# seobbro/TTA-depth-completion

Measured on AMD Instinct MI355X. Metric: TTA frames/sec (fwd+loss+bwd+Adam) at 352x1216, higher is better.
Workload: dtype mixed: real frames' forward (the scored depth) f32 storage + bf16x3 MFMA arithmetic; no_grad proxy pass and all data gradients bf16 storage + single bf16 MFMA; fp32 accumulate everywhere; loss / Adam / adapted parameters fp32 (include/ptta.h PTTA_DTYPE_MIXED)

## Files before the change

include/ptta.h:

```cpp
#ifndef PTTA_H
#define PTTA_H
#include <stdint.h>
#ifdef __cplusplus
extern "C" {
#endif

typedef struct ptta_ctx* ptta_handle;
typedef void* ptta_stream;

enum { PTTA_BACKBONE_MSG_CHN = 0, PTTA_BACKBONE_NLSPN = 1, PTTA_BACKBONE_COSTDCNET = 2 };
enum { PTTA_DTYPE_F32 = 0, PTTA_DTYPE_MIXED = 1,
       PTTA_MIXED_KEEP_PROXY = 0x100, PTTA_MIXED_KEEP_BACKWARD = 0x200, PTTA_MIXED_KEEP_HEADS = 0x400,
       PTTA_MIXED_BWD_ROUNDED_W = 0x800 };
enum { PTTA_META_1LAYER = 0, PTTA_META_2LAYERS = 1, PTTA_META_NONE = 2 };
enum { PTTA_NLSPN_LEGACY_OFFSET = 0x100,
       PTTA_NLSPN_SYNCBN_ADAPT = 0x200,
       PTTA_SYNCBN_ADAPT = 0x200,
       PTTA_ADAPT_META_ONLY = 0x400 };

typedef struct {
    float lr, beta1, beta2, eps, weight_decay;
    float w_sparse_depth, w_smoothness, w_cos;
    float max_input_depth;
    float max_predict_depth;
// ... 52 lines not shown
int ptta_eval_metrics(const float* depth, const float* ground_truth, int64_t numel, float min_evaluate_depth,
                      float max_evaluate_depth, void* scratch, float* metrics_out, ptta_stream s);

int ptta_mdconv_forward(const float* input, const float* weight, const float* bias, const float* offset, const float* mask,
                        float* output, int b, int c, int h, int w, int c_out, int kh, int kw, int sh, int sw, int ph, int pw,
                        int dh, int dw, int group, int deformable_group, ptta_stream s);
int ptta_mdconv_backward(const float* input, const float* weight, const float* bias, const float* offset, const float* mask,
                         const float* grad_output, float* grad_input, float* grad_offset, float* grad_mask, float* grad_weight,
                         float* grad_bias, int b, int c, int h, int w, int c_out, int kh, int kw, int sh, int sw, int ph, int pw,
                         int dh, int dw, int group, int deformable_group, ptta_stream s);

int ptta_set_image_norm(ptta_handle h, float divisor, const float* mean, const float* stdv);

int ptta_head_bind(ptta_handle h, const char* name, float* param, float* exp_avg, float* exp_avg_sq);
int ptta_head_set_hparams(ptta_handle h, float lr, float beta1, float beta2, float eps, float weight_decay, float tau,
                          int adam_step, ptta_stream s);
int ptta_head_reload(ptta_handle h, ptta_stream s);
int ptta_head_forward(ptta_handle h, const float* image, const float* sparse_depth, int reverse, float* emb_out, float* ref_out,
                      ptta_stream s);
int ptta_head_backward(ptta_handle h, float* loss_out, ptta_stream s);
int ptta_head_adam_step(ptta_handle h, ptta_stream s);
int ptta_head_step(ptta_handle h, const float* image, const float* sparse_depth, int reverse, float* loss_out, ptta_stream s);
int ptta_head_get_grad(ptta_handle h, const char* name, float* dst, int64_t capacity, int* has_grad_host, ptta_stream s);

enum { PTTA_HEAD_FORM_PLAIN = 0, PTTA_HEAD_FORM_SYNCBN = 1 };
int ptta_head_set_form(ptta_handle h, int form);

int ptta_crop_flip(const float* src, float* dst, int n, int channels, int height, int width, int crop_height, int crop_width,
                   const int32_t* start_y, const int32_t* start_x, const uint8_t* hflip, const uint8_t* vflip, ptta_stream s);

int ptta_rotate(const float* src, float* dst, int n, int channels, int height, int width, const uint8_t* do_rotate, const float* angle_deg,
                int bilinear, ptta_stream s);
int ptta_resize_crop(const float* src, float* dst, int n, int channels, int height, int width, const uint8_t* do_resize,
                     const int32_t* resize_height, const int32_t* resize_width, const int32_t* start_y, const int32_t* start_x,
                     int bilinear, int scale_depth, ptta_stream s);
int ptta_photometric(const float* src, float* dst, int n, int height, int width, const uint8_t* do_brightness, const float* f_brightness,
                     const uint8_t* do_contrast, const float* f_contrast, const uint8_t* do_saturation, const float* f_saturation,
                     double* scratch, ptta_stream s);

int ptta_photometric_full(const float* src, float* dst, int n, int height, int width, const uint8_t* do_brightness, const float* f_brightness,
                          const uint8_t* do_contrast, const float* f_contrast, const uint8_t* do_gamma, const float* f_gamma,
                          const uint8_t* do_hue, const float* f_hue, const uint8_t* do_saturation, const float* f_saturation,
                          double* scratch, ptta_stream s);
int ptta_add_noise(const float* src, const float* noise, float* dst, int n, int channels, int height, int width, const uint8_t* do_noise,
                   float spread, int uniform, ptta_stream s);
int ptta_remove_patches(const float* src, float* dst, int n, int channels, int height, int width, const uint8_t* do_remove,
                        const uint8_t* selected, const int32_t* patch_height, const int32_t* patch_width, ptta_stream s);
int ptta_crop_pad(const float* src, float* dst, int n, int channels, int height, int width, const uint8_t* do_crop_pad,
                  const int32_t* start_y, const int32_t* start_x, const int32_t* end_y, const int32_t* end_x,
                  const int32_t* pad_top, const int32_t* pad_left, int padding_mode, float fill, ptta_stream s);
int ptta_resize_pad(const float* src, float* dst, int n, int channels, int height, int width, const uint8_t* do_resize_pad,
                    const int32_t* resize_height, const int32_t* resize_width, const int32_t* pad_top, const int32_t* pad_left,
                    int bilinear, int padding_mode, float fill, ptta_stream s);

typedef int (*ptta_allreduce_fn)(void* user, double* exchange_buf, long long count, ptta_stream s);
int ptta_set_stat_sync(ptta_handle h, ptta_allreduce_fn fn, void* user, double* exchange_buf, int64_t capacity, int world_size);

int ptta_rccl_unique_id(void* id128_host);
int ptta_rccl_comm_create(const void* id128_host, int rank, int world_size, void** comm_out_host);
int ptta_rccl_comm_destroy(void* comm);
int ptta_rccl_allreduce_mean_f32(void* comm, float* buf, int64_t count, ptta_stream s);
const char* ptta_rccl_last_error(void);
int ptta_set_stat_sync_rccl(ptta_handle h, void* comm, double* exchange_buf, int64_t capacity, int world_size);
int ptta_set_grad_sync_rccl(ptta_handle h, void* comm);

int ptta_set_graph(ptta_handle h, int enable);

int ptta_set_option(ptta_handle h, const char* key, int value);
int ptta_get_option(ptta_handle h, const char* key, int* value_host);

int ptta_profile(ptta_handle h, int enable);
int ptta_profile_read(ptta_handle h, int klass, double* ms_total_host, double* alg_bytes_host, double* macs_host,
                      int64_t* launches_host, ptta_stream s);

int ptta_debug_tensor(ptta_handle h, const char* name, float* dst, int64_t capacity, int64_t* numel_host, ptta_stream s);
int ptta_op_conv32(const float* in_nhwc, const float* weight, const float* bias, float* out_nhwc,
                   int b, int hin, int win, int mode, int relu_in, int in_major, int flip, int dtype, int naive,
                   ptta_stream s);
int ptta_op_conv32_pair(const float* in_nhwc, const float* weight1, const float* bias1, const float* weight2, const float* bias2,
                        const float* up_nhwc, const float* add0_nhwc, const float* add1_nhwc, const float* add2_nhwc,
                        const uint32_t* mask1_bits, const uint32_t* mask2_bits, float* out_raw, float* out_sum, float* mid_raw,
                        float* mid_sum, uint32_t* mid_bits, int b, int in_nb, int hin, int win, int first_mode, int relu1, int relu2,
                        int in_major, int flip, int dtype, int w2, int fused, int* fused_host, ptta_stream s);
int ptta_op_gwgrad(const float* x_nhwc, const float* gy_nhwc, float* gw, float* gb, int b, int h, int w, int ci, int co, int impl,
                   int reps, float* us_per_call_host, ptta_stream s);
#define PTTA_GCONV_S1 0
#define PTTA_GCONV_S2 1
#define PTTA_GCONV_T2 2
#define PTTA_GCONV_VERT 1
#define PTTA_GCONV_X1_W2 2
#define PTTA_GCONV_DGRAD 4
#define PTTA_GCONV_AFF_ACT_FIRST 8
#define PTTA_GCONV_AFF_RES_PLAIN 16
int ptta_op_gconv(const float* x0, int c0, int ld0, const float* x1, int c1, int ld1, const float* weight, const float* bias, float* y,
                  int co, int ldy, int b, int hin, int win, int hout, int wout, int k, int geom, int act, int accumulate, int impl,
                  int flags, int six_b, int x1_from_b, int stat_npass, double* stat_host, int* form_host, ptta_stream s);
int ptta_op_gconv_affine(const float* x0, int c0, int ld0, const float* x1, int c1, int ld1, const float* weight, const float* bias, float* y,
                         int co, int ldy, int b, int hin, int win, int hout, int wout, int k, int geom, int act, int accumulate, int impl,
                         int flags, int six_b, int x1_from_b, int stat_npass, double* stat_host, int* form_host, const float* scale,
                         const float* shift, const float* res, int ld_res, ptta_stream s);
#define PTTA_GBN_TRAIN 0
#define PTTA_GBN_EVAL 1
#define PTTA_GBN_BACKWARD 2
typedef struct ptta_gbn_view { float* p; int c; int ld; } ptta_gbn_view;
typedef struct ptta_gbn_args {
    int mode, b, h, w, npass, act, act_first, res_relu, acc_gx, acc_gres, world, nblocks_in, repeats;
    float eps, momentum;
    ptta_gbn_view x, res, y, g, gx, gres;
    const float* gamma; const float* beta; const float* part_in;
    float* st; float* rm; float* rv; long long* nbt; float* st_eval; float* dgamma; float* dbeta;
} ptta_gbn_args;
int ptta_op_gbn(const ptta_gbn_args* a, ptta_stream s);
typedef struct ptta_cd_sparse ptta_cd_sparse;
int ptta_cd_sparse_create(ptta_cd_sparse** out, int n, int h, int w);
void ptta_cd_sparse_destroy(ptta_cd_sparse* q);
int ptta_cd_sparse_build(ptta_cd_sparse* q, const float* sparse, float z_step, ptta_stream s);
int ptta_cd_sparse_read(ptta_cd_sparse* q, int level, int* cnt_host, int* coords_host, long long coords_cap, int* vol_host, float* feat_in_host,
                        ptta_stream s);
int ptta_op_cd_sparse_conv(ptta_cd_sparse* q, const float* x, const float* wk, float* y, int lin, int lout, int ksize, int ci, int co, int backward,
                           int acc, ptta_stream s);
typedef struct ptta_cd_sbn_args {
    int mode, level, c, relu, repeats, world, acc_res;
    const float* f; const float* res; const float* y; const float* g; const float* gamma; const float* beta;
    float* rm; float* rv; long long* nbt; float* out; float* st; float* dgamma; float* dbeta; float* gx; float* gres;
} ptta_cd_sbn_args;
int ptta_op_cd_sbn(ptta_cd_sparse* q, const ptta_cd_sbn_args* a, ptta_stream s);
int ptta_op_cd_densify(ptta_cd_sparse* q, const float* in, float* out, int c, int backward, int ldv, int c0, ptta_stream s);
#define PTTA_CD_PAD_DUAL 0
#define PTTA_CD_CROP_AVG 1
#define PTTA_CD_SCATTER_DUAL_GRAD 2
#define PTTA_CD_STAGE 3
#define PTTA_CD_CLAMP 4
#define PTTA_CD_FUSION_FWD 5
#define PTTA_CD_FUSION_BWD 6
#define PTTA_CD_POOL_FWD 7
#define PTTA_CD_POOL_BWD 8
#define PTTA_CD_UP_FWD 9
#define PTTA_CD_UP_BWD 10
#define PTTA_CD_REGRESS_FWD 11
#define PTTA_CD_REGRESS_BWD 12
#define PTTA_CD_ROWS_FWD 13
#define PTTA_CD_ROWS_BWD 14
int ptta_op_cd_dense(int op, const float* a, const float* b, float* out, float* out2, const int* d, const float* f, ptta_stream s);
int ptta_op_conv32_chain(const float* in_nhwc, const float* weight, const float* bias, float* buf_a, float* buf_b, const float* aux,
                         int b, int h, int w, int relu_in, int epi_flags, int reps, int replays, float* us_per_launch_host, ptta_stream s);
#define PTTA_ABI_VERSION 2
int ptta_version(void);

#ifdef __cplusplus
}
#endif
#endif
```

tta-depth-completion_amd/csrc/msgchn_backward.hip:

```cpp
#include "msgchn_ctx.h"

using namespace msgchn;

namespace msgchn {

static int meta2_backward(ptta_ctx* c, hipStream_t s) {
    auto& m2 = c->m2;
    ptta_ctx::Adapted* A = c->adapted.data();
    const int H4 = c->H4, W4 = c->W4, Nn = c->Nn;
    const long P = (long)Nn * H4 * W4;
    if (m2.generic) {
        const int npass = 2;
        GView x; x.p = (float*)c->c2; x.B = Nn; x.H = H4; x.W = W4; x.C = 32; x.ld = 32;
        GView hv = x; hv.p = m2.gh; hv.C = 128; hv.ld = 128;
        GView av = hv; av.p = m2.ga1;
        GView tv = x; tv.p = m2.gt;
        GView gm = x; gm.p = c->nar_bwd ? c->dm_f32 : (float*)c->dm_total;
        GView dt = x; dt.p = m2.gdt;
        GView da1 = hv; da1.p = m2.gda1;
        GView dh = hv; dh.p = m2.gdh;
        RUN(ptta_launch_gbn_backward(tv, gm, tv, dt, GView(), npass, GACT_NONE, 0, 0, 0, A[5].p, m2.gst2, m2.gpart, m2.gbw, A[5].g, A[6].g, s, 0, &c->stat_sync));
        RUN(ptta_launch_gwgrad_mfma(av, dt, m2.wgp, A[3].g, A[4].g, s));
        GX3Args a;
        a.x0 = dt.p; a.C0 = 32; a.ld0 = 32; a.B = Nn; a.H = H4; a.W = W4;
// ... 30 lines not shown
                  (double)c->Rg * (16384.0 + 262144.0), 3);
    const Lin& l0 = c->fc["proj.0"]; const Lin& l3 = c->fc["proj.3"]; BNorm& bn = c->bn["proj.1"];
    const int R = (int)c->Rg;
    if (c->nar_heads && heads_v2_on(c)) {
        HnGemmArgs g; g.epi = 3; g.R = R; g.W = l3.Wtsl;
        if (c->cos_in_gemm) { g.pro = 4; g.A = c->emb_n; g.Bref = c->ref_n; g.rowstats = c->loss_ws + ptta_loss_ws_rows_off(c->N); g.coef = c->loss_ws; }
        else { g.pro = 5; g.Af = gref; }
        g.X = c->feat; g.x_bf16 = 0; g.W0 = l0.Whi; g.W0t = l0.Wthi; g.b0 = l0.bias;
        g.escale = bn.scale; g.eshift = bn.shift; g.emean = bn.mean; g.einv = bn.inv; g.part = c->bn_part; g.P = c->headP;
        RUN(ptta_launch_hn_gemm(g, s));
        const int nb = ptta_hn_row_blocks(R);
        RUN(ptta_stat_sync(&c->stat_sync, c->bn_part, nb, 512, 1, s));
        RUN(ptta_launch_bn_bwd_finalize(c->bn_part, nb, R * (c->stat_sync.world > 1 ? c->stat_sync.world : 1), 512, bn.gamma, bn.inv, c->bnb_gscale, c->bnb_c1, c->bnb_c2, s,
                                        nullptr, nullptr, c->head_k12, l0.bias, bn.mean));
        RUN(ptta_launch_head_bwd_finish(c->head_k12, l0.W, c->headP, (const float*)c->feat, R, c->g_feat, s, 1, c->nar_bwd ? 1 : 0));
        return 0;
    }
    if (heads_v2_on(c)) {
        GemmArgs g; g.A = gref; g.W = l3.Wt; g.R = R; g.K = 512; g.N = 512; g.epi = 3;
        if (c->cos_in_gemm) {
            g.A = c->emb; g.Bref = c->ref; g.rowstats = c->loss_ws + ptta_loss_ws_rows_off(c->N); g.coef = c->loss_ws; g.pro = 4;
        }
        g.escale = bn.scale; g.eshift = bn.shift; g.emean = bn.mean; g.einv = bn.inv; g.part = c->bn_part;
        g.x3 = 1; g.Whi = l3.Wthi; g.Wlo = l3.Wtlo; g.Wil = l3.Wtil;
        g.X = (const float*)c->feat; g.b0 = l0.bias; g.W0hi = l0.Whi; g.W0lo = l0.Wlo; g.W0thi = l0.Wthi; g.W0tlo = l0.Wtlo; g.P = c->headP;
        RUN(ptta_launch_gemm(g, s));
        RUN(ptta_stat_sync(&c->stat_sync, c->bn_part, ptta_gemm_part_blocks(g), 512, 1, s));
        RUN(ptta_launch_bn_bwd_finalize(c->bn_part, ptta_gemm_part_blocks(g), R * (c->stat_sync.world > 1 ? c->stat_sync.world : 1), 512, bn.gamma, bn.inv, c->bnb_gscale, c->bnb_c1, c->bnb_c2, s,
                                        nullptr, nullptr, c->head_k12, l0.bias, bn.mean));
        RUN(ptta_launch_head_bwd_finish(c->head_k12, l0.W, c->headP, (const float*)c->feat, R, c->nar_bwd ? c->g_feat_f32 : (float*)c->g_feat, s));
        if (c->nar_bwd) RUN(to_narrow(c, c->g_feat_f32, c->g_feat, c->Rg * 32, s));
        return 0;
    }
    GemmArgs g; g.A = gref; g.W = l3.Wt; g.C = c->gmask; g.R = R; g.K = 512; g.N = 512; g.epi = 2;
    g.eH = c->h1; g.escale = bn.scale; g.eshift = bn.shift; g.emean = bn.mean; g.einv = bn.inv; g.part = c->bn_part;
    g.x3 = c->x3; g.Whi = l3.Wthi; g.Wlo = l3.Wtlo; g.Wil = l3.Wtil;
    RUN(ptta_launch_gemm(g, s));
    RUN(ptta_stat_sync(&c->stat_sync, c->bn_part, ptta_gemm_part_blocks(g), 512, 1, s));
    RUN(ptta_launch_bn_bwd_finalize(c->bn_part, ptta_gemm_part_blocks(g), R * (c->stat_sync.world > 1 ? c->stat_sync.world : 1), 512, bn.gamma, bn.inv, c->bnb_gscale, c->bnb_c1, c->bnb_c2, s));
    GemmArgs g2; g2.A = c->gmask; g2.A2 = c->h1; g2.W = l0.Wt; g2.C = (c->bf16 || c->nar_bwd) ? c->g_feat_f32 : (float*)c->g_feat; g2.R = R; g2.K = 512; g2.N = 32; g2.pro = 2;
    g2.pscale = c->bnb_gscale; g2.pmean = bn.mean; g2.pinv = bn.inv; g2.pc1 = c->bnb_c1; g2.pc2 = c->bnb_c2;
    g2.x3 = c->x3; g2.Whi = l0.Wthi; g2.Wlo = l0.Wtlo;
    RUN(ptta_launch_gemm(g2, s));
    if (c->bf16 || c->nar_bwd) from_f32_launch(c->g_feat_f32, (bf16_t*)c->g_feat, c->Rg * 32, s);
    return 0;
}

int backbone_backward(ptta_ctx* c, const float* g_net, hipStream_t s, bool join_aux) {
    const int Nn = c->Nn, B2 = 2 * Nn;
    const int nbf = c->nar_bwd ? 1 : c->bf16;
    const int H1 = c->Hp, W1 = c->Wp, H2 = c->H2, W2 = c->W2, H4 = c->H4, W4 = c->W4, H8 = c->H8, W8 = c->W8;
    auto out1_args = [&](const std::string& layer, const float* g, const void* mask, void* out, int H, int W) {
        const LOut& lo = c->lout[layer];
        ConvInArgs a; a.cin = 1; a.pl[0].p = g; a.pl[0].nb = Nn; a.pl[0].bstride = (long)H * W;
        a.wfrag = lo.bfrag; a.wcanon = lo.bcanon; a.mask = mask; a.mask_nb = B2; a.out_raw = out;
        a.B = Nn; a.H = H; a.W = W; a.bf16 = c->nar_bwd ? 1 : c->bf16; a.naive = c->naive;
        return a;
    };
    auto dgrad_out1 = [&](const std::string& layer, const float* g, const void* mask, void* out, int H, int W) -> int {
        ConvInArgs a = out1_args(layer, g, mask, out, H, W);
        return conv_in_p(c, a, s);
    };
    auto head_bwd = [&](const std::string& l3, const std::string& l1, const float* g, const void* v, void* dv, int H, int W, const E& e) -> int {
        ConvInArgs a = out1_args(l3, g, v, dv, H, W);
        return conv32_first_bwd(c, s, l1, a, Nn, H, W, e);
    };
    auto dgrad_in_ch1 = [&](const std::string& layer, const void* g, const float* add, float* out, int H, int W) -> int {
        const LIn& li = c->lin_in[layer];
        ConvOut1Args a; a.in = g; a.in_nb = Nn; a.w = li.bw; a.add = add; a.add_nb = Nn; a.out = out;
        a.B = Nn; a.H = H; a.W = W; a.relu_in = 0; a.bf16 = c->nar_bwd ? 1 : c->bf16;
        return conv_out1_p(c, a, s);
    };
    auto em = [](void* raw, const void* mask, int mask_nb) { E e; e.raw = raw; e.mask = mask; e.mask_nb = mask_nb; return e; };
    RUN(head_bwd("depth_decoder3.prdct.3", "depth_decoder3.prdct.1", g_net, c->v3, c->dv3, H1, W1, em(c->ds0_3, c->s0_3, Nn)));
    CV("depth_decoder3.dec1.3", true, CONV_S1, c->ds0_3, Nn, Nn, H1, W1, false, em(c->du3, c->u3, Nn));
    CV("depth_decoder3.dec1.1", true, CONV_S2, c->du3, Nn, Nn, H1, W1, false, em(c->ds1_3, c->s1_3, Nn));
    CV("depth_decoder3.dec2.3", true, CONV_S1, c->ds1_3, Nn, Nn, H2, W2, false, em(c->dt3, c->t3, Nn));
    if (join_aux) HIPCHK(hipStreamWaitEvent(s, c->ev_join, 0));
    { E e; e.raw = c->dw2; e.mask = c->w2; e.mask_nb = B2; e.sum = c->dfeat_tot; e.add1 = c->g_feat; e.add1_nb = Nn;
      RUN(conv32_pair(c, s, true, "depth_decoder3.dec2.1", c->dt3, Nn, Nn, H2, W2, e, "depth_encoder3.enc2.3", Nn, em(c->de3_2a, c->e3_2a, B2))); }
    hipStream_t sd = join_aux ? c->aux(s) : nullptr;
    if (!sd) sd = s;
    { E e; e.sum = c->de3_1; e.mask = c->e3_1; e.mask_nb = B2; e.add1 = c->ds1_3; e.add1_nb = Nn;
      CV("depth_encoder3.enc2.1", true, CONV_T2, c->de3_2a, Nn, Nn, H4, W4, false, e); }
    CV("depth_encoder3.enc1.3", true, CONV_S1, c->de3_1, Nn, Nn, H2, W2, false, em(c->de3_1a, c->e3_1a, B2));
    { E e; e.sum = c->de3_0; e.mask = c->e3_0; e.mask_nb = B2; e.add1 = c->ds0_3; e.add1_nb = Nn;
      CV("depth_encoder3.enc1.1", true, CONV_T2, c->de3_1a, Nn, Nn, H2, W2, false, e); }
    if (sd != s) { HIPCHK(hipEventRecord(c->ev_side[0], s)); HIPCHK(hipStreamWaitEvent(sd, c->ev_side[0], 0)); }
    REST_(sd, ptta_launch_up2T_32(c->de3_0, nullptr, c->up4_t, Nn, H2, W2, nbf, sd));
    REST_(sd, ptta_launch_up2T_32(c->de3_1, nullptr, c->up3_t, Nn, H4, W4, nbf, sd));
    REST_(sd, ptta_launch_up2T_32(c->dfeat_tot, nullptr, c->dz2_up, Nn, H8, W8, nbf, sd));
    if (sd != s) HIPCHK(hipEventRecord(c->ev_side[3], sd));
    if (c->loss_report.on) {
        REST_(sd, ptta_launch_loss_depth_part(final_depth(c), c->loss_report.image, c->loss_report.sparse, c->loss_report.validity, c->hp.max_input_depth,
                                              c->N, c->H, c->W, c->loss_ws, sd));
        REST_(sd, ptta_launch_loss_finalize(c->loss_ws, c->N, c->H, c->W, c->Rg, 1, c->hyper + 5, c->loss_info_dst ? c->loss_info_dst : c->loss_info, sd));
        HIPCHK(hipEventRecord(c->ev_loss, sd));
    }
    CV("depth_encoder3.init.2", true, CONV_S1, c->de3_0, Nn, Nn, H1, W1, false, em(c->de3_0a, c->e3_0a, B2));
    RUN(dgrad_in_ch1("depth_encoder3.init.0", c->de3_0a, g_net, c->dp11, H1, W1));
    REST_(s, ptta_launch_up2T_1ch(c->dp11, c->dq, Nn, H2, W2, s));
    if (sd != s) HIPCHK(hipStreamWaitEvent(s, c->ev_side[3], 0));
    { E e = em(c->ds0_2, c->s0_2, B2); e.sum = c->dz4; e.add1 = c->up4_t; e.add1_nb = Nn;
      RUN(head_bwd("depth_decoder2.prdct.3", "depth_decoder2.prdct.1", c->dq, c->v2, c->dv2, H2, W2, e)); }
    CV("depth_decoder2.dec1.3", true, CONV_S1, c->dz4, Nn, Nn, H2, W2, false, em(c->du2, c->u2, B2));
    { E e = em(c->ds1_2, c->s1_2, B2); e.sum = c->dz3; e.add1 = c->up3_t; e.add1_nb = Nn;
      RUN(conv32_pair(c, s, true, "depth_decoder2.dec1.1", c->du2, Nn, Nn, H2, W2, e, "depth_decoder2.dec2.3", Nn, em(c->dt2, c->t2, B2))); }
    { E e; e.sum = c->dz2; e.mask = c->z2; e.mask_nb = B2; e.add1 = c->dz2_up; e.add1_nb = Nn;
      RUN(conv32_pair(c, s, true, "depth_decoder2.dec2.1", c->dt2, Nn, Nn, H4, W4, e, "depth_encoder2.enc2.3", Nn, em(c->de2_2a, c->e2_2a, B2))); }
    { E e; e.sum = c->de2_1; e.mask = c->e2_1; e.mask_nb = B2; e.add1 = c->ds1_2; e.add1_nb = Nn;
      CV("depth_encoder2.enc2.1", true, CONV_T2, c->de2_2a, Nn, Nn, H8, W8, false, e); }
    CV("depth_encoder2.enc1.3", true, CONV_S1, c->de2_1, Nn, Nn, H4, W4, false, em(c->de2_1a, c->e2_1a, B2));
    { E e; e.sum = c->de2_0; e.mask = c->e2_0; e.mask_nb = B2; e.add1 = c->ds0_2; e.add1_nb = Nn;
      CV("depth_encoder2.enc1.1", true, CONV_T2, c->de2_1a, Nn, Nn, H4, W4, false, e); }
    CV("depth_encoder2.init.2", true, CONV_S1, c->de2_0, Nn, Nn, H2, W2, false, em(c->de2_0a, c->e2_0a, B2));
    RUN(dgrad_in_ch1("depth_encoder2.init.0", c->de2_0a, c->dq, c->dp12, H2, W2));
    REST_(s, ptta_launch_up2T_1ch(c->dp12, c->dout1, Nn, H4, W4, s));
    RUN(dgrad_out1("depth_decoder1.prdct.3", c->dout1, c->v1, c->dv1, H4, W4));
    { E e; e.sum = c->dm_total; e.mask = c->s0_1; e.mask_nb = B2; e.add1 = c->dw2; e.add1_nb = Nn; e.add2 = c->ds1_2; e.add2_nb = Nn;
      CV("depth_decoder1.prdct.1", true, CONV_S1, c->dv1, Nn, Nn, H4, W4, false, e); }
    if (sd != s && c->loss_report.on) HIPCHK(hipStreamWaitEvent(s, c->ev_loss, 0));
    if (c->nar_bwd && c->meta_mode == PTTA_META_2LAYERS) RUN(to_wide(c, c->dm_total, c->dm_f32, (long)Nn * H4 * W4 * 32, s));
    if (c->meta_mode == PTTA_META_2LAYERS) return meta2_backward(c, s);
    if (!c->bf16 && c->x3 && !c->naive) {
        GView xv; xv.p = (float*)c->c2; xv.B = Nn; xv.H = H4; xv.W = W4; xv.C = 32; xv.ld = 32;
        GView gv; gv.p = (float*)c->dm_total; gv.B = Nn; gv.H = H4; gv.W = W4; gv.C = 32; gv.ld = 32;
        GwAdam ga;
        const bool fuse = c->adam_fuse_req && c->adam_in_wgrad && !c->grad_comm && c->adapted.size() == 2 && c->adapted[0].p && c->adapted[0].m && c->adapted[0].v &&
                          c->adapted[1].p && c->adapted[1].m && c->adapted[1].v && c->adapted[0].g == c->gW && c->adapted[1].g == c->gB;
        if (fuse) { ga.pw = c->adapted[0].p; ga.mw = c->adapted[0].m; ga.vw = c->adapted[0].v; ga.pb = c->adapted[1].p; ga.mb = c->adapted[1].m; ga.vb = c->adapted[1].v;
                    ga.hyper = c->hyper; ga.step = c->step_dev; ga.ticket = c->adam_ticket; }
        REST_(s, ptta_launch_gwgrad_mfma(xv, gv, c->wgrad_part, c->gW, c->gB, s, c->nar_bwd ? 1 : 0, fuse ? &ga : nullptr));
        c->adam_fused = fuse;
        return 0;
    }
    REST_(s, ptta_launch_wgrad32(c->c2, c->dm_total, c->bf16, Nn, H4, W4, c->wgrad_part, c->gW, c->gB, s));
    return 0;
}

}
```

tta-depth-completion_amd/csrc/msgchn_ctx.h:

```cpp
#pragma once
#include <cstdio>
#include <cstdlib>
#include <cstring>
#include <map>
#include <string>
#include <unordered_map>
#include <vector>

#include "../../include/ptta.h"
#include "ptta_common.h"
#include "ptta_kernels.h"
#include "nlspn.h"

#pragma GCC visibility push(hidden)

#define HIPCHK(x) do { hipError_t e_ = (x); if (e_ != hipSuccess) return c->fail(std::string(#x) + ": " + hipGetErrorString(e_), -100 - (int)e_); } while (0)
#define RUN(x) do { int r_ = (x); if (r_ != 0) return c->fail_chain(std::string(#x) + " failed", r_ < 0 ? r_ : -r_); } while (0)

#define NLFWD(call) do { if (c && c->nl) { c->err.clear(); return (call); } } while (0)

struct ImgNorm { int on; float div; float mean[3]; float stdv[3]; };

namespace msgchn {
hipError_t d2d_copy(void* dst, const void* src, size_t bytes, hipStream_t s);
void stamp_launch(float* out, unsigned long long* base, int i, hipStream_t s);
void transpose_launch(const float* src, float* dst, int rows, int cols, hipStream_t s);
void pad_dual_launch(const float* src, float* dst, int N, int C, int H, int W, int Hp, int Wp, int pt, int pr, hipStream_t s,
                     ImgNorm nm = ImgNorm{0, 1.f, {0.f, 0.f, 0.f}, {1.f, 1.f, 1.f}});
void crop_avg_launch(const float* net, float* out, int N, int H, int W, int Hp, int Wp, int pt, int pr, hipStream_t s);
void scatter_dual_grad_launch(const float* g, float* gnet, int N, int H, int W, int Hp, int Wp, int pt, int pr, hipStream_t s);
void to_f32_launch(const bf16_t* src, float* dst, long n, hipStream_t s);
void from_f32_launch(const float* src, bf16_t* dst, long n, hipStream_t s);
void fuse_linear_launch(const float* Wb, const float* bb, const float* Wa, const float* ba, float* W, float* bias, int N, int M, int K, hipStream_t s);
}

static constexpr unsigned kStepEvent = hipEventDisableTiming | hipEventDisableSystemFence;
struct L32 { ConvW f{}, b{}; float* bias = nullptr; int transposed = 0; };
struct LIn { float *wfrag = nullptr, *wcanon = nullptr, *bias = nullptr, *bw = nullptr; int cin = 1; };
struct LOut { float *w = nullptr, *bias = nullptr, *bfrag = nullptr, *bcanon = nullptr; };
struct Lin { float *W = nullptr, *Wt = nullptr, *bias = nullptr; bf16_t *Whi = nullptr, *Wlo = nullptr, *Wthi = nullptr, *Wtlo = nullptr, *Wil = nullptr, *Wtil = nullptr;
             bf16_t *Wsl = nullptr, *Wtsl = nullptr;
             int N = 0, K = 0; };
struct BNorm { float *gamma = nullptr, *beta = nullptr, *rm = nullptr, *rv = nullptr; long long* nbt = nullptr;
               float *mean = nullptr, *inv = nullptr, *scale = nullptr, *shift = nullptr; };
struct Dbg { const void* p; long numel; int is_act; };

struct PrefixBufs {
    void *c0 = nullptr, *c1 = nullptr, *c2 = nullptr, *c3 = nullptr, *c4 = nullptr, *e1_0a = nullptr, *e1_0 = nullptr, *e1_1a = nullptr;
    void *c0a = nullptr, *c1a = nullptr, *c2a = nullptr, *c3a = nullptr, *c4a = nullptr;
    void *e1_1 = nullptr, *y1 = nullptr, *e1_2a = nullptr, *y2 = nullptr, *t1 = nullptr, *y3 = nullptr, *s1_1 = nullptr, *u1 = nullptr;
    float *dclamp = nullptr, *d12 = nullptr, *d14 = nullptr, *in_image = nullptr, *in_loss_image = nullptr, *in_sparse = nullptr, *in_validity = nullptr;
    bool proxy_valid = false;
};

struct ptta_ctx : PrefixBufs {
    GNet* nl = nullptr;
    int N = 1, H = 0, W = 0, Hp = 0, Wp = 0, pt = 0, pr = 0, dual = 0, Nn = 1;
    int bf16 = 0, naive = 0, es = 4, x3 = 1;
    int mixed = 0;
    int nar_proxy = 0, nar_bwd = 0, nar_heads = 0;
    std::unordered_map<const void*, void*> ntwin;
    void* tw(const void* p) const { auto it = ntwin.find(p); return it == ntwin.end() ? nullptr : it->second; }
    void twin_alloc(const void* p, int nb, int h, int w) { if (nar_proxy && p) ntwin[p] = dalloc((size_t)nb * h * w * 32 * 2); }
    float *dm_f32 = nullptr;
    ptta_hparams hp{};
    std::string err;
    std::vector<void*> allocs;
    std::map<std::string, L32> l32;
    std::map<std::string, LIn> lin_in;
    std::map<std::string, LOut> lout;
    std::map<std::string, Lin> fc;
    std::map<std::string, BNorm> bn;
    std::map<std::string, Dbg> dbg;
    int meta_mode = 0;
    struct Adapted { std::string name; long n = 0; float *p = nullptr, *m = nullptr, *v = nullptr, *g = nullptr; };
    std::vector<Adapted> adapted;
    struct HeadT { bool ready = false; std::vector<Adapted> prm, tgt; bool has_grad[12] = {};
                   float *hyper = nullptr, *tau2 = nullptr, *loss = nullptr, *loss_part = nullptr, *wpart = nullptr, *bpart = nullptr, *dp = nullptr;
                   float *sv_mean = nullptr, *sv_inv = nullptr, *sv_scale = nullptr, *sv_shift = nullptr;
                   int* step = nullptr; unsigned* ticket = nullptr; PttaAdamEntry *tab = nullptr, *etab = nullptr;
                   std::vector<PttaAdamEntry> tab_host, etab_host; int tab_n = 0; long tab_total = 0, etab_total = 0; int tab_mode = -1; bool etab_dirty = true;
                   int reverse = 1; bool fwd_ok = false, bwd_ok = false;
                   float* garena = nullptr; long garena_n = 0;
                   int form = 0; bool stepped = false; } head;
    int skip_dec3 = 0;
    int head_swap = 0;
    float *meta_w = nullptr, *meta_b = nullptr;
    float *gW = nullptr, *gB = nullptr;
    struct Meta2 {
        ConvW w1f[4], w2f[4], w2b[4];
        void *h[4] = {}, *a1[4] = {}, *t = nullptr, *dt = nullptr, *da1 = nullptr, *dh = nullptr;
        float *st1 = nullptr, *st2 = nullptr;
        float *rm1 = nullptr, *rv1 = nullptr, *rm2 = nullptr, *rv2 = nullptr; long long *nbt1 = nullptr, *nbt2 = nullptr;
        float *cs_part = nullptr, *bw = nullptr;
        bool generic = false;
        float *gh = nullptr, *ga1 = nullptr, *gt = nullptr, *gdt = nullptr, *gda1 = nullptr, *gdh = nullptr;
        float *w1c = nullptr, *w2c = nullptr, *w2bc = nullptr;
        bf16_t *w1hi = nullptr, *w1lo = nullptr, *w2hi = nullptr, *w2lo = nullptr, *w2bhi = nullptr, *w2blo = nullptr;
        float *gst1 = nullptr, *gst2 = nullptr, *part1 = nullptr, *part2 = nullptr, *gbw = nullptr, *gpart = nullptr, *wgp = nullptr;
    } m2;
    float* hyper = nullptr;
    float* w3_tmp = nullptr;
    int* step_dev = nullptr; float* stamp_f = nullptr; unsigned long long* stamp_base = nullptr; int stamps = 0;
    void stamp(int i, hipStream_t s) { if (stamps) msgchn::stamp_launch(stamp_f, stamp_base, i, s); }
    PttaAdamEntry* adam_tab = nullptr; unsigned* adam_ticket = nullptr; bool adam_tab_dirty = true;
    std::vector<PttaAdamEntry> adam_host;
    bool fwd_valid = false;
    PttaStatSync stat_sync;
    Lin fused_pp; bool fused_pp_valid = false; int fuse_heads = 1;
    int heads_v2 = 1;
    int thru = 1; bool thru_active = false;
    int adam_in_wgrad = 1; bool adam_fuse_req = false, adam_fused = false;
    int bwd_w2 = 1;
    const float *cnt_sparse = nullptr, *cnt_validity = nullptr;
    struct { const float *image = nullptr, *sparse = nullptr, *validity = nullptr; bool on = false; } loss_report;
    hipEvent_t ev_loss = nullptr;
    hipEvent_t ev_dpart = nullptr;
    int fuse_first = 1, fuse_head_bwd = 1;
    int pair_fuse = 1;
    int pair_fuse_count = 0;
    int cos_grad_fused = 1;
    bool cos_in_gemm = false;
    void* w0frag = nullptr; float *hm_part = nullptr, *headP = nullptr; double* head_k12 = nullptr;
    struct ProfClass { std::vector<std::pair<hipEvent_t, hipEvent_t>> ev; size_t used = 0; double bytes = 0, macs = 0; long launches = 0; };
    bool prof_on = false;
    static constexpr int NPROF = 9;
    ProfClass prof[NPROF];
    std::vector<std::pair<int, size_t>> prof_seq;
    int use_graph = 0;
    void* grad_comm = nullptr;
    float* grad_arena = nullptr; long grad_arena_n = 0;
    int pre_sync_graph = -1, pre_sync_aux = -1;
    hipGraphExec_t gexec[4] = {nullptr, nullptr, nullptr, nullptr};
    hipGraph_t graph[4] = {nullptr, nullptr, nullptr, nullptr};
    hipStream_t cap_stream = nullptr;
    struct PreSet : PrefixBufs {
        bool prepared = false, rest_recorded = false;
        uint64_t prep_token = 0;
        uint64_t last_token = 0;
    };
    PreSet pset[2];
    int cur_set = 0, pipe_cur = 0, pipe_last = 0;
    bool pipe_ready = false, pipe_active = false, skip_prefix = false;
    const float *fb_image = nullptr, *fb_sparse = nullptr;
    hipStream_t pre_stream = nullptr;
    hipEvent_t ev_prefix[2] = {nullptr, nullptr}, ev_rest[2] = {nullptr, nullptr}, ev_entry = nullptr;
    hipStream_t pipe_stream = nullptr; bool pipe_stream_set = false;
    hipGraph_t pgraph[2] = {nullptr, nullptr}, rgraph[4][2] = {{nullptr, nullptr}, {nullptr, nullptr}, {nullptr, nullptr}, {nullptr, nullptr}};
    hipGraphExec_t pexec[2] = {nullptr, nullptr}, rexec[4][2] = {{nullptr, nullptr}, {nullptr, nullptr}, {nullptr, nullptr}, {nullptr, nullptr}};
    int use_aux = 1;
    hipStream_t aux_stream = nullptr;
    hipEvent_t ev_fork = nullptr, ev_join = nullptr, ev_real = nullptr;
    hipEvent_t ev_side[4] = {nullptr, nullptr, nullptr, nullptr};
    hipStream_t aux(hipStream_t caller) {
        if (!use_aux) return nullptr;
        if (!aux_stream) {
            if (hipStreamCreateWithFlags(&aux_stream, hipStreamNonBlocking) != hipSuccess) return nullptr;
            if (hipEventCreateWithFlags(&ev_fork, kStepEvent) != hipSuccess ||
                hipEventCreateWithFlags(&ev_join, kStepEvent) != hipSuccess ||
                hipEventCreateWithFlags(&ev_real, kStepEvent) != hipSuccess ||
                hipEventCreateWithFlags(&ev_side[0], kStepEvent) != hipSuccess || hipEventCreateWithFlags(&ev_side[1], kStepEvent) != hipSuccess ||
                hipEventCreateWithFlags(&ev_side[2], kStepEvent) != hipSuccess || hipEventCreateWithFlags(&ev_side[3], kStepEvent) != hipSuccess) { (void)hipStreamDestroy(aux_stream); aux_stream = nullptr; return nullptr; }
        }
        return prof_on ? caller : aux_stream;
    }
    hipEvent_t ev_replay = nullptr;
    void drop_graphs() {
        if (ev_replay) (void)hipEventSynchronize(ev_replay);
        if (pre_stream) (void)hipStreamSynchronize(pre_stream);
        for (int k = 0; k < 4; ++k) {
            if (gexec[k]) { (void)hipGraphExecDestroy(gexec[k]); gexec[k] = nullptr; }
            if (graph[k]) { (void)hipGraphDestroy(graph[k]); graph[k] = nullptr; }
            for (int p = 0; p < 2; ++p) {
                if (rexec[k][p]) { (void)hipGraphExecDestroy(rexec[k][p]); rexec[k][p] = nullptr; }
                if (rgraph[k][p]) { (void)hipGraphDestroy(rgraph[k][p]); rgraph[k][p] = nullptr; }
            }
        }
        for (int p = 0; p < 2; ++p) {
            if (pexec[p]) { (void)hipGraphExecDestroy(pexec[p]); pexec[p] = nullptr; }
            if (pgraph[p]) { (void)hipGraphDestroy(pgraph[p]); pgraph[p] = nullptr; }
            pset[p].prepared = false; pset[p].prep_token = pset[p].last_token = 0;
        }
        fb_image = fb_sparse = nullptr;
    }

    int err_code = 0;
    int fail(const std::string& m, int code) { err = m; err_code = code; return code; }
    int fail_chain(const std::string& m, int code) { err = (err_code == code && !err.empty() && err.size() < 600) ? m + " <- " + err : m; err_code = code; return code; }

    bool oom = false;
    void* dalloc(size_t bytes) {
        void* p = nullptr;
        if (hipMalloc(&p, bytes ? bytes : 16) != hipSuccess) { oom = true; return nullptr; }
        allocs.push_back(p);
        if (hipMemset(p, 0, bytes ? bytes : 16) != hipSuccess) { oom = true; return nullptr; }
        return p;
    }
    float* falloc(size_t n) { return (float*)dalloc(n * sizeof(float)); }
    void* act(const char* name, int nb, int h, int w) {
        void* p = dalloc((size_t)nb * h * w * 32 * es);
        dbg[name] = Dbg{p, (long)nb * h * w * 32, 1};
        if (nar_proxy && nb == 2 * Nn) twin_alloc(p, Nn, h, w);
        return p;
// ... 1 lines not shown
    void* gact(const char* name, int nb, int h, int w) {
        const int e = nar_bwd ? 2 : es;
        void* p = dalloc((size_t)nb * h * w * 32 * e);
        dbg[name] = Dbg{p, (long)nb * h * w * 32, nar_bwd ? 2 : 1};
        return p;
    }
    int mask_bits_on = 1;
    std::unordered_map<const void*, uint32_t*> mbits;
    void mask_plane(const void* map, int nb, int h, int w) {
        if (bf16 || naive) return;
        if (mbits.count(map)) return;
        mbits[map] = (uint32_t*)dalloc((size_t)nb * h * w * sizeof(uint32_t));
    }
    uint32_t* bits_of(const void* map) const {
        if (!map || !mask_bits_on) return nullptr;
        auto it = mbits.find(map);
        return it == mbits.end() ? nullptr : it->second;
    }
    float* map1(const char* name, int nb, int h, int w) {
        float* p = falloc((size_t)nb * h * w);
        dbg[name] = Dbg{p, (long)nb * h * w, 0};
        return p;
    }

    int H2, W2, H4, W4, H8, W8, H16, W16;
    long Rg = 0;
    float *img_pad = nullptr, *sp_pad = nullptr, *zero_plane = nullptr;
    ImgNorm img_norm = ImgNorm{0, 1.f, {0.f, 0.f, 0.f}, {1.f, 1.f, 1.f}};
    float *out1, *p12, *q, *p11, *depth_net, *depth_final, *validity_tmp;
    void *m, *y4, *s0_1, *v1;
    void *e2_0a, *e2_0, *e2_1a, *e2_1, *e2_2a, *z2, *t2, *z3, *s1_2, *u2, *z4, *s0_2, *v2;
    void *e3_0a, *e3_0, *e3_1a, *e3_1, *e3_2a, *feat, *w2, *t3, *s1_3, *u3, *s0_3, *v3;
    float *h1z, *pz, *h2, *emb, *h1, *ref, *gref_buf, *gmask, *bn_part;
    double* hn_msc = nullptr;
    float* hn_rs = nullptr;
    bool cos_rows_done = false;
    bf16_t *emb_n = nullptr, *ref_n = nullptr, *h2_n = nullptr;
    float *bnb_gscale, *bnb_c1, *bnb_c2;
    float *loss_ws, *loss_info, *g_final, *g_net;
    float* loss_info_dst = nullptr;
    void *dv3, *ds0_3, *du3, *ds1_3, *dt3, *dw2, *dfeat_tot, *dz2_up, *de3_2a, *de3_1, *de3_1a, *de3_0, *de3_0a;
    void *up4_t, *up3_t, *dv2, *ds0_2, *dz4, *du2, *ds1_2, *dz3, *dt2, *dz2, *de2_2a, *de2_1, *de2_1a, *de2_0, *de2_0a, *dv1, *dm_total, *g_feat;
    float *dp11, *dq, *dp12, *dout1, *g_feat_f32;
    float* wgrad_part;
};

struct ProfScope {
    ptta_ctx::ProfClass* pc = nullptr; hipStream_t s;
    ProfScope(ptta_ctx* c, int klass, hipStream_t s_, double bytes, double macs, int launches) : s(s_) {
        if (!c->prof_on) return;
        pc = &c->prof[klass];
        if (pc->used == pc->ev.size()) {
            hipEvent_t e0, e1;
            if (hipEventCreate(&e0) != hipSuccess || hipEventCreate(&e1) != hipSuccess) { pc = nullptr; return; }
            pc->ev.push_back({e0, e1});
        }
        pc->bytes += bytes; pc->macs += macs; pc->launches += launches;
        c->prof_seq.push_back({klass, pc->used});
        (void)hipEventRecord(pc->ev[pc->used].first, s);
    }
    ~ProfScope() { if (pc) { (void)hipEventRecord(pc->ev[pc->used].second, s); pc->used++; } }
};
#define REST_(s_, call) do { ProfScope ps_(c, 8, (s_), 0, 0, 1); RUN(call); } while (0)
#define CV(...) RUN(conv32(c, s, __VA_ARGS__))

struct E { const void* up = nullptr; int up_nb = 1; const void* mask = nullptr; int mask_nb = 1;
           const void* add1 = nullptr; int add1_nb = 1; const void* add2 = nullptr; int add2_nb = 1;
           void* raw = nullptr; void* sum = nullptr;
           bool nar = false; };

inline float* st_ptr(float* base, int C, int pass, int kind) { return base + ((size_t)pass * 4 + kind) * C; }

namespace msgchn {
int pad16(int n);
void build_registry(ptta_ctx* c);
void build_workspace(ptta_ctx* c);
int load_weight(ptta_ctx* c, const std::string& name, const void* tensor, const int64_t* shape, int ndim, hipStream_t s);
int conv_in_p(ptta_ctx* c, const ConvInArgs& a_, hipStream_t s);
int conv_out1_p(ptta_ctx* c, const ConvOut1Args& a, hipStream_t s);
int conv32(ptta_ctx* c, hipStream_t s, const std::string& layer, bool bwd, int mode, const void* in, int in_nb,
           int B, int Hin, int Win, bool relu, const E& e);
int conv32_pair(ptta_ctx* c, hipStream_t s, bool bwd, const std::string& first, const void* in, int in_nb, int B, int Hin, int Win, const E& fe,
                const std::string& second, int mid_nb, const E& se);
int conv32w(ptta_ctx* c, hipStream_t s, const ConvW* w, const float* bias, const void* in, int in_nb, int B, int H, int W, const E& e);
int conv32_first_bwd(ptta_ctx* c, hipStream_t s, const std::string& layer, ConvInArgs& f, int B, int H, int W, const E& e);
int to_narrow(ptta_ctx* c, const void* src_f32, void* dst, long n, hipStream_t s);
int to_wide(ptta_ctx* c, const void* src_nar, float* dst, long n, hipStream_t s);
int rgb_encoder(ptta_ctx* c, const float* image, int nb, int boff, int zero_from_b, hipStream_t s);
int ensure_fused_heads(ptta_ctx* c, hipStream_t s);
int ensure_proxy_rgb(ptta_ctx* c, const float* any_image, hipStream_t s);
int enc1_head_fn(ptta_ctx* c, hipStream_t st);
int stage1_independent(ptta_ctx* c, int B2, hipStream_t s);
bool heads_v2_on(const ptta_ctx* c);
int heads_forward(ptta_ctx* c, hipStream_t s, int part = 0);
int push_hparams(ptta_ctx* c, hipStream_t s);
int forward_common(ptta_ctx* c, const float* image, const float* sparse, bool train, hipStream_t s);
const float* final_depth(ptta_ctx* c);
int heads_backward(ptta_ctx* c, const float* gref, hipStream_t s);
int backbone_backward(ptta_ctx* c, const float* g_net, hipStream_t s, bool join_aux);
void pipe_use(ptta_ctx* c, int p);
void pipe_overwritten(ptta_ctx* c, int p);
int pipe_quiesce(ptta_ctx* c);
int ensure_adam_table(ptta_ctx* c, hipStream_t s);
}
#pragma GCC visibility pop
```

tta-depth-completion_amd/csrc/msgchn_forward.hip:

```cpp
#include "msgchn_ctx.h"

using namespace msgchn;

namespace msgchn {

int conv_in_p(ptta_ctx* c, const ConvInArgs& a_, hipStream_t s) {
    ConvInArgs a = a_;
    const double px = (double)a.B * a.H * a.W;
    ProfScope ps(c, 7, s, px * (a.cin * 4 + 32 * (a.bf16 ? 2 : c->es)) + 9.0 * a.cin * 32 * 4, px * 9.0 * a.cin * 32, 1);
    if (!c->mbits.empty()) {
        if (!a.mask_bits) a.mask_bits = c->bits_of(a.mask);
        if (!a.bf16 && !a.a_bits) { a.a_bits = c->bits_of(a.out_raw); a.a_bits_nb = c->Nn; }
    }
    return ptta_launch_conv_in(a, s);
}
int conv_out1_p(ptta_ctx* c, const ConvOut1Args& a, hipStream_t s) {
    const double px = (double)a.B * a.H * a.W;
    ProfScope ps(c, 7, s, px * (32 * (a.bf16 ? 2 : c->es) + 4) + 288 * 4, px * 288.0, 1);
    return ptta_launch_conv_out1(a, s);
}

static int conv32_args(ptta_ctx* c, Conv32Args& a, const std::string& layer, bool bwd, int mode, const void* in, int in_nb,
                       int B, int Hin, int Win, bool relu, const E& e) {
    auto it = c->l32.find(layer);
    if (it == c->l32.end()) return c->fail("unknown 32->32 layer " + layer, -2);
    a.in = in; a.in_nb = in_nb; a.w = bwd ? &it->second.b : &it->second.f;
    a.bias = bwd ? nullptr : (layer == "conv1_rgb_meta" ? c->meta_b : it->second.bias);
    a.up = e.up; a.up_nb = e.up_nb; a.mask = e.mask; a.mask_nb = e.mask_nb;
    a.add1 = e.add1; a.add1_nb = e.add1_nb; a.add2 = e.add2; a.add2_nb = e.add2_nb;
    a.out_raw = e.raw; a.out_sum = e.sum;
    const bool nar = e.nar || (bwd && c->nar_bwd);
    a.B = B; a.Hin = Hin; a.Win = Win; a.mode = mode; a.relu_in = relu ? 1 : 0; a.bf16 = nar ? 1 : c->bf16; a.naive = c->naive; a.x3 = c->x3;
    a.w2 = (bwd && c->nar_bwd && c->bwd_w2) ? 1 : 0;
    if (!c->mbits.empty()) {
        a.mask_bits = c->bits_of(e.mask);
        if (!bwd && !nar) {
            uint32_t* bs = c->bits_of(e.sum); uint32_t* br = c->bits_of(e.raw);
            if (bs && br) return c->fail("conv32: both outputs of " + layer + " are registered masks", -22);
            if (bs || br) { a.bits_out = bs ? bs : br; a.bits_sum = bs ? 1 : 0; a.bits_nb = c->Nn; }
        }
    }
    return 0;
}

static void conv32_cost(int mode, int B, int Hin, int Win, int es_l, double& bytes, double& macs) {
    const long pin = (long)B * Hin * Win;
    const long pout = mode == CONV_S1 ? pin : (mode == CONV_S2 ? pin / 4 : pin * 4);
    bytes = (double)((pin + pout) * 32 + 9216) * es_l;
    macs = (double)(mode == CONV_T2 ? pin : pout) * 9.0 * 32.0 * 32.0;
}

int conv32(ptta_ctx* c, hipStream_t s, const std::string& layer, bool bwd, int mode, const void* in, int in_nb,
           int B, int Hin, int Win, bool relu, const E& e) {
    Conv32Args a;
    { const int rc = conv32_args(c, a, layer, bwd, mode, in, in_nb, B, Hin, Win, relu, e); if (rc) return rc; }
    const bool nar = e.nar || (bwd && c->nar_bwd);
    const int es_l = nar ? 2 : c->es;
    const long pin = (long)B * Hin * Win;
    const long pout = mode == CONV_S1 ? pin : (mode == CONV_S2 ? pin / 4 : pin * 4);
    const bool small = (long)Hin * Win <= (long)c->H4 * c->W4 * (mode == CONV_S2 ? 4 : 1);
#ifdef PTTA_EXP_SKIP_PAIRED_S1
    if (mode == CONV_S1 && small && layer.size() > 2 && layer.compare(layer.size() - 2, 2, ".3") == 0 && layer.find("prdct") == std::string::npos) return 0;
#endif
    ProfScope ps(c, (mode == CONV_S1 ? (relu ? 0 : 2) : 4) + (small ? 1 : 0), s, (double)((pin + pout) * 32 + 9216) * es_l,
                 (double)(mode == CONV_T2 ? pin : pout) * 9.0 * 32.0 * 32.0, 1);
    return ptta_launch_conv32(a, s);
}

int conv32_pair(ptta_ctx* c, hipStream_t s, bool bwd, const std::string& first, const void* in, int in_nb, int B, int Hin, int Win, const E& fe,
                const std::string& second, int mid_nb, const E& se) {
    const int Hm = Hin / 2, Wm = Win / 2;
    const bool relu = !bwd;
    void* const mid = fe.sum ? fe.sum : fe.raw;
    const bool nar = fe.nar || (bwd && c->nar_bwd);
    if (c->pair_fuse && !c->naive && (c->x3 || c->bf16 || nar) && fe.nar == se.nar && mid) {
        Conv32Args f, g;
        { const int rc = conv32_args(c, f, first, bwd, CONV_S2, in, in_nb, B, Hin, Win, relu, fe); if (rc) return rc; }
        { const int rc = conv32_args(c, g, second, bwd, CONV_S1, mid, mid_nb, B, Hm, Wm, relu, se); if (rc) return rc; }
        if (mid_nb == B && ptta_conv32_pair_applies(f, g)) {
            const int es_l = nar ? 2 : c->es;
            double b1, m1, b2, m2;
            conv32_cost(CONV_S2, B, Hin, Win, es_l, b1, m1); conv32_cost(CONV_S1, B, Hm, Wm, es_l, b2, m2);
            ProfScope ps(c, 5, s, b1 + b2, m1 + m2, 1);
            const int rc = ptta_launch_conv32_pair(f, g, s);
            if (rc == 1) return c->fail("conv32_pair: fused form refused a case its own test accepted", -22);
            if (rc == 0) c->pair_fuse_count++;
            return rc;
        }
    }
    { const int rc = conv32(c, s, first, bwd, CONV_S2, in, in_nb, B, Hin, Win, relu, fe); if (rc) return rc; }
    return conv32(c, s, second, bwd, CONV_S1, mid, mid_nb, B, Hm, Wm, relu, se);
}

int conv32w(ptta_ctx* c, hipStream_t s, const ConvW* w, const float* bias, const void* in, int in_nb, int B, int H, int W, const E& e) {
    Conv32Args a;
    a.in = in; a.in_nb = in_nb; a.w = w; a.bias = bias;
    a.add1 = e.add1; a.add1_nb = e.add1_nb; a.out_raw = e.raw; a.out_sum = e.sum;
    a.B = B; a.Hin = H; a.Win = W; a.mode = CONV_S1; a.relu_in = 0; a.bf16 = c->bf16; a.naive = c->naive; a.x3 = c->x3;
    return ptta_launch_conv32(a, s);
}

static int conv32_first(ptta_ctx* c, hipStream_t s, const std::string& layer, ConvInArgs& f, int a_nb, int B, int H, int W, const E& e) {
    auto it = c->l32.find(layer);
    if (it == c->l32.end()) return c->fail("unknown 32->32 layer " + layer, -2);
    const long tiles = (long)B * ((W + 31) / 32) * ((H + 7) / 8);
    const bool nar = e.nar;
    f.bf16 = nar ? 1 : c->bf16;
    if (c->fuse_first >= (f.cin == 3 ? 2 : 1) && !c->bf16 && !c->naive && c->x3 && tiles > 256 && !e.mask && !e.add1 && !e.add2 && !e.sum) {
        Conv32Args a;
        a.in = nullptr; a.in_nb = B; a.w = &it->second.f; a.bias = it->second.bias;
        a.up = e.up; a.up_nb = e.up_nb; a.out_raw = e.raw;
        a.B = B; a.Hin = H; a.Win = W; a.mode = CONV_S1; a.relu_in = 1; a.bf16 = nar ? 1 : 0; a.naive = 0; a.x3 = 1;
        const double px = (double)B * H * W;
        const int es_l = nar ? 2 : c->es;
        ProfScope ps(c, 0, s, (px * f.cin + 9.0 * f.cin * 32) * 4 + (px * 96 + 9216) * es_l, px * 9.0 * (f.cin * 32 + 1024), 1);
        f.a_bits = (a_nb > 0 && !nar) ? c->bits_of(f.out_raw) : nullptr;
        if (!c->mbits.empty() && !nar) { uint32_t* br = c->bits_of(e.raw); if (br) { a.bits_out = br; a.bits_nb = c->Nn; } }
        const int rc = ptta_launch_conv32_first(a, f, (a_nb > 0 && !nar && !f.a_bits) ? f.out_raw : nullptr, a_nb, s);
        return rc == 1 ? c->fail("conv32_first: fused form refused a case its caller accepted", -22) : rc;
    }
    RUN(conv_in_p(c, f, s));
    return conv32(c, s, layer, false, CONV_S1, f.out_raw, B, B, H, W, true, e);
}

int conv32_first_bwd(ptta_ctx* c, hipStream_t s, const std::string& layer, ConvInArgs& f, int B, int H, int W, const E& e) {
    auto it = c->l32.find(layer);
    if (it == c->l32.end()) return c->fail("unknown 32->32 layer " + layer, -2);
    const long tiles = (long)B * ((W + 31) / 32) * ((H + 7) / 8);
    const bool nar = c->nar_bwd != 0;
    f.bf16 = nar ? 1 : c->bf16;
    if (c->fuse_head_bwd && c->bits_of(f.mask) && c->bits_of(e.mask) && c->fuse_first >= 1 && !c->bf16 && !c->naive && c->x3 && tiles > 256 && e.mask && e.raw && (e.add1 != nullptr) == (e.sum != nullptr) && !e.add2 && !e.up) {
        Conv32Args a;
        a.in = nullptr; a.in_nb = B; a.w = &it->second.b; a.bias = nullptr;
        a.mask = e.mask; a.mask_nb = e.mask_nb; a.out_raw = e.raw; a.add1 = e.add1; a.add1_nb = e.add1_nb; a.out_sum = e.sum;
        a.mask_bits = c->bits_of(e.mask); f.mask_bits = c->bits_of(f.mask);
        a.B = B; a.Hin = H; a.Win = W; a.mode = CONV_S1; a.relu_in = 0; a.bf16 = nar ? 1 : 0; a.naive = 0; a.x3 = 1;
        a.w2 = (nar && c->bwd_w2) ? 1 : 0;
        const double px = (double)B * H * W;
        const int es_l = nar ? 2 : c->es;
        ProfScope ps(c, 2, s, (px + 9.0 * 32) * 4 + (px * 96 + 9216) * es_l, px * 9.0 * (32 + 1024), 1);
        const int rc = ptta_launch_conv32_first(a, f, nullptr, 0, s);
        return rc == 1 ? c->fail("conv32_first_bwd: fused form refused a case its caller accepted", -22) : rc;
    }
    RUN(conv_in_p(c, f, s));
    return conv32(c, s, layer, true, CONV_S1, f.out_raw, B, B, H, W, false, e);
}


static int meta_forward(ptta_ctx* c, bool train, int B, hipStream_t s) {
    const int H4 = c->H4, W4 = c->W4, Nn = c->Nn;
    if (c->meta_mode == PTTA_META_1LAYER) {
        E e; e.raw = c->m;
        if (c->nar_proxy && train && B == 2 * Nn) {
            return conv32(c, s, "conv1_rgb_meta", false, CONV_S1, c->c2, Nn, Nn, H4, W4, false, e);
        }
        return conv32(c, s, "conv1_rgb_meta", false, CONV_S1, c->c2, B, B, H4, W4, false, e);
    }
    auto& m2 = c->m2;
    const ptta_ctx::Adapted* A = c->adapted.data();
    const long P = (long)Nn * H4 * W4;
    const int npass = train ? B / Nn : 1;
    if (m2.generic) {
        if (!train && (!m2.rm1 || !m2.rv1 || !m2.rm2 || !m2.rv2)) return c->fail("meta BatchNorm running statistics not loaded", -3);
        GView x; x.p = (float*)c->c2; x.B = B; x.H = H4; x.W = W4; x.C = 32; x.ld = 32;
        GView hv = x; hv.p = m2.gh; hv.C = 128; hv.ld = 128;
        GView av = hv; av.p = m2.ga1;
        GView tv = x; tv.p = m2.gt;
        GView mv = x; mv.p = (float*)c->m;
        const int tiles_pp = ptta_gconv_x3_tiles(B / npass, H4, W4);
        auto finalize = [&](float* part, int C, const float* gamma, const float* beta, float* rm, float* rv, long long* nbt, float* st) -> int {
            if (!train) return ptta_launch_bn_eval_affine(gamma, beta, rm, rv, 1e-5f, st + 2 * C, st + 3 * C, C, s);
            if (ptta_stat_sync(&c->stat_sync, part, tiles_pp, C, npass, s)) return -5;
            const int wmul = c->stat_sync.world > 1 ? c->stat_sync.world : 1;
// ... 135 lines not shown
    return 0;
}

int enc1_head_fn(ptta_ctx* c, hipStream_t st) {
    const int Nn = c->Nn, H4 = c->H4, W4 = c->W4;
    const LIn& li = c->lin_in["depth_encoder1.init.0"];
    ConvInArgs a; a.cin = 1; a.pl[0].p = c->d14; a.pl[0].nb = Nn; a.pl[0].bstride = (long)H4 * W4;
    a.wfrag = li.wfrag; a.wcanon = li.wcanon; a.bias = li.bias; a.out_raw = c->e1_0a;
    a.B = Nn; a.H = H4; a.W = W4; a.bf16 = c->bf16; a.naive = c->naive;
    RUN(conv_in_p(c, a, st));
    { E e; e.raw = c->e1_0; RUN(conv32(c, st, "depth_encoder1.init.2", false, CONV_S1, c->e1_0a, Nn, Nn, H4, W4, true, e)); }
    { E e; e.raw = c->e1_1a; RUN(conv32(c, st, "depth_encoder1.enc1.1", false, CONV_S2, c->e1_0, Nn, Nn, H4, W4, true, e)); }
    return 0;
}

int stage1_independent(ptta_ctx* c, int B2, hipStream_t s) {
    const int Nn = c->Nn, H4 = c->H4, W4 = c->W4, H8 = c->H8, W8 = c->W8, H16 = c->H16, W16 = c->W16;
    const bool two = c->nar_proxy && B2 == 2 * Nn;
    const int Bf = two ? Nn : B2;
    { E e; e.raw = c->e1_1; e.sum = c->y1; e.add1 = c->c3; e.add1_nb = B2;
      RUN(conv32(c, s, "depth_encoder1.enc1.3", false, CONV_S1, c->e1_1a, Nn, Bf, H8, W8, true, e)); }
    { E e; e.raw = c->e1_2a; RUN(conv32(c, s, "depth_encoder1.enc2.1", false, CONV_S2, c->e1_1, B2, Nn, H8, W8, true, e)); }
    { E e; e.sum = c->y2; e.add1 = c->c4; e.add1_nb = B2;
      RUN(conv32(c, s, "depth_encoder1.enc2.3", false, CONV_S1, c->e1_2a, Nn, Bf, H16, W16, true, e)); }
    { E e; e.raw = c->t1; RUN(conv32(c, s, "depth_decoder1.dec2.1", false, CONV_T2, c->y2, B2, Bf, H16, W16, true, e)); }
    { E e; e.raw = c->y3; e.sum = c->s1_1; e.add1 = c->y1; e.add1_nb = B2;
      RUN(conv32(c, s, "depth_decoder1.dec2.3", false, CONV_S1, c->t1, B2, Bf, H8, W8, true, e)); }
    { E e; e.raw = c->u1; RUN(conv32(c, s, "depth_decoder1.dec1.1", false, CONV_T2, c->s1_1, B2, Bf, H8, W8, true, e)); }
    if (!two) return 0;
    RUN(to_narrow(c, c->e1_0, c->tw(c->e1_0), (long)Nn * H4 * W4 * 32, s));
    RUN(to_narrow(c, c->e1_1a, c->tw(c->e1_1a), (long)Nn * H8 * W8 * 32, s));
    RUN(to_narrow(c, c->e1_2a, c->tw(c->e1_2a), (long)Nn * H16 * W16 * 32, s));
    { E e; e.nar = true; e.sum = c->tw(c->y1); e.add1 = c->tw(c->c3); e.add1_nb = Nn;
      RUN(conv32(c, s, "depth_encoder1.enc1.3", false, CONV_S1, c->tw(c->e1_1a), Nn, Nn, H8, W8, true, e)); }
    { E e; e.nar = true; e.sum = c->tw(c->y2); e.add1 = c->tw(c->c4); e.add1_nb = Nn;
      RUN(conv32(c, s, "depth_encoder1.enc2.3", false, CONV_S1, c->tw(c->e1_2a), Nn, Nn, H16, W16, true, e)); }
    { E e; e.nar = true; e.raw = c->tw(c->t1); RUN(conv32(c, s, "depth_decoder1.dec2.1", false, CONV_T2, c->tw(c->y2), Nn, Nn, H16, W16, true, e)); }
    { E e; e.nar = true; e.raw = c->tw(c->y3); e.sum = c->tw(c->s1_1); e.add1 = c->tw(c->y1); e.add1_nb = Nn;
      RUN(conv32(c, s, "depth_decoder1.dec2.3", false, CONV_S1, c->tw(c->t1), Nn, Nn, H8, W8, true, e)); }
    { E e; e.nar = true; e.raw = c->tw(c->u1); RUN(conv32(c, s, "depth_decoder1.dec1.1", false, CONV_T2, c->tw(c->s1_1), Nn, Nn, H8, W8, true, e)); }
    return 0;
}

static int backbone(ptta_ctx* c, const float* image, bool train, hipStream_t s) {
    hipStream_t s2 = train ? c->aux(s) : nullptr;
    const int Nn = c->Nn, B2 = train ? 2 * Nn : Nn;
    const bool two = train && c->nar_proxy;
    const int H1 = c->Hp, W1 = c->Wp, H2 = c->H2, W2 = c->W2, H4 = c->H4, W4 = c->W4, H8 = c->H8, W8 = c->W8, H16 = c->H16, W16 = c->W16;
    auto e_raw = [](void* raw) { E e; e.raw = raw; return e; };
    if (!c->skip_prefix) RUN(rgb_encoder(c, image, Nn, 0, Nn, s));
    RUN(meta_forward(c, train, B2, s));
    if (!c->skip_prefix) { RUN(enc1_head_fn(c, s)); RUN(stage1_independent(c, B2, s)); }

    auto region = [&](hipStream_t st, int b0, int Bl, bool nar) -> int {
        auto A = [&](void* p_, int h, int w) -> void* { return nar ? c->tw(p_) : (void*)((char*)p_ + (size_t)b0 * h * w * 32 * c->es); };
        auto P1 = [&](float* p_, int h, int w) { return p_ + (size_t)b0 * h * w; };
        auto raw = [&](void* r) { E e; e.raw = r; e.nar = nar; return e; };
        const void* e1_0 = nar ? c->tw(c->e1_0) : c->e1_0;
#define CR(...) RUN(conv32(c, st, __VA_ARGS__))
        { E e; e.nar = nar; e.raw = A(c->y4, H4, W4); e.sum = A(c->s0_1, H4, W4); e.add1 = e1_0; e.add1_nb = Nn; e.add2 = A(c->m, H4, W4); e.add2_nb = Bl;
          CR("depth_decoder1.dec1.3", false, CONV_S1, A(c->u1, H4, W4), Bl, Bl, H4, W4, true, e); }
        CR("depth_decoder1.prdct.1", false, CONV_S1, A(c->s0_1, H4, W4), Bl, Bl, H4, W4, true, raw(A(c->v1, H4, W4)));
        {
            const LOut& lo = c->lout["depth_decoder1.prdct.3"];
            ConvOut1Args a; a.in = A(c->v1, H4, W4); a.in_nb = Bl; a.w = lo.w; a.bias = lo.bias; a.out = P1(c->out1, H4, W4);
            a.B = Bl; a.H = H4; a.W = W4; a.relu_in = 1; a.bf16 = nar ? 1 : c->bf16;
            RUN(conv_out1_p(c, a, st));
        }
        REST_(st, ptta_launch_up2_1ch(P1(c->out1, H4, W4), P1(c->p12, H2, W2), Bl, H4, W4, st));
        {
            const LIn& li = c->lin_in["depth_encoder2.init.0"];
            ConvInArgs a; a.cin = 2;
            a.pl[0].p = c->d12; a.pl[0].nb = Nn; a.pl[0].bstride = (long)H2 * W2;
            a.pl[1].p = P1(c->p12, H2, W2); a.pl[1].nb = Bl; a.pl[1].bstride = (long)H2 * W2;
            a.wfrag = li.wfrag; a.wcanon = li.wcanon; a.bias = li.bias; a.out_raw = A(c->e2_0a, H2, W2);
            a.B = Bl; a.H = H2; a.W = W2; a.bf16 = c->bf16; a.naive = c->naive;
            E e; e.nar = nar; e.raw = A(c->e2_0, H2, W2); e.up = A(c->y4, H4, W4); e.up_nb = Bl;
            RUN(conv32_first(c, st, "depth_encoder2.init.2", a, (b0 == 0 && !nar) ? Nn : 0, Bl, H2, W2, e));
        }
        { E e; e.nar = nar; e.raw = A(c->e2_1, H4, W4); e.up = A(c->y3, H8, W8); e.up_nb = Bl;
          RUN(conv32_pair(c, st, false, "depth_encoder2.enc1.1", A(c->e2_0, H2, W2), Bl, Bl, H2, W2, raw(A(c->e2_1a, H4, W4)), "depth_encoder2.enc1.3", Bl, e)); }
        { E e; e.nar = nar; e.sum = A(c->z2, H8, W8); e.up = A(c->y2, H16, W16); e.up_nb = Bl; e.add1 = A(c->c3, H8, W8); e.add1_nb = Bl;
          RUN(conv32_pair(c, st, false, "depth_encoder2.enc2.1", A(c->e2_1, H4, W4), Bl, Bl, H4, W4, raw(A(c->e2_2a, H8, W8)), "depth_encoder2.enc2.3", Bl, e)); }
        CR("depth_decoder2.dec2.1", false, CONV_T2, A(c->z2, H8, W8), Bl, Bl, H8, W8, true, raw(A(c->t2, H4, W4)));
        { E e; e.nar = nar; e.raw = A(c->z3, H4, W4); e.sum = A(c->s1_2, H4, W4); e.add1 = A(c->e2_1, H4, W4); e.add1_nb = Bl; e.add2 = A(c->m, H4, W4); e.add2_nb = Bl;
          CR("depth_decoder2.dec2.3", false, CONV_S1, A(c->t2, H4, W4), Bl, Bl, H4, W4, true, e); }
        CR("depth_decoder2.dec1.1", false, CONV_T2, A(c->s1_2, H4, W4), Bl, Bl, H4, W4, true, raw(A(c->u2, H2, W2)));
        { E e; e.nar = nar; e.raw = A(c->z4, H2, W2); e.sum = A(c->s0_2, H2, W2); e.add1 = A(c->e2_0, H2, W2); e.add1_nb = Bl; e.add2 = A(c->c1, H2, W2); e.add2_nb = Bl;
          CR("depth_decoder2.dec1.3", false, CONV_S1, A(c->u2, H2, W2), Bl, Bl, H2, W2, true, e); }
        CR("depth_decoder2.prdct.1", false, CONV_S1, A(c->s0_2, H2, W2), Bl, Bl, H2, W2, true, raw(A(c->v2, H2, W2)));
        {
            const LOut& lo = c->lout["depth_decoder2.prdct.3"];
            ConvOut1Args a; a.in = A(c->v2, H2, W2); a.in_nb = Bl; a.w = lo.w; a.bias = lo.bias; a.add = P1(c->p12, H2, W2); a.add_nb = Bl; a.out = P1(c->q, H2, W2);
            a.B = Bl; a.H = H2; a.W = W2; a.relu_in = 1; a.bf16 = nar ? 1 : c->bf16;
            RUN(conv_out1_p(c, a, st));
        }
        REST_(st, ptta_launch_up2_1ch(P1(c->q, H2, W2), P1(c->p11, H1, W1), Bl, H2, W2, st));
        {
            const LIn& li = c->lin_in["depth_encoder3.init.0"];
            ConvInArgs a; a.cin = 2;
            a.pl[0].p = c->dclamp; a.pl[0].nb = Nn; a.pl[0].bstride = (long)H1 * W1;
            a.pl[1].p = P1(c->p11, H1, W1); a.pl[1].nb = Bl; a.pl[1].bstride = (long)H1 * W1;
            a.wfrag = li.wfrag; a.wcanon = li.wcanon; a.bias = li.bias; a.out_raw = A(c->e3_0a, H1, W1);
            a.B = Bl; a.H = H1; a.W = W1; a.bf16 = c->bf16; a.naive = c->naive;
            E e; e.nar = nar; e.raw = A(c->e3_0, H1, W1); e.up = A(c->z4, H2, W2); e.up_nb = Bl;
            RUN(conv32_first(c, st, "depth_encoder3.init.2", a, (b0 == 0 && !nar) ? Nn : 0, Bl, H1, W1, e));
        }
        CR("depth_encoder3.enc1.1", false, CONV_S2, A(c->e3_0, H1, W1), Bl, Bl, H1, W1, true, raw(A(c->e3_1a, H2, W2)));
        { E e; e.nar = nar; e.raw = A(c->e3_1, H2, W2); e.up = A(c->z3, H4, W4); e.up_nb = Bl; CR("depth_encoder3.enc1.3", false, CONV_S1, A(c->e3_1a, H2, W2), Bl, Bl, H2, W2, true, e); }
        { E e; e.nar = nar; e.raw = A(c->feat, H4, W4); e.up = A(c->z2, H8, W8); e.up_nb = Bl; e.add1 = A(c->m, H4, W4); e.add1_nb = Bl;
          if (!nar) e.sum = A(c->w2, H4, W4); else e.add1 = nullptr;
          RUN(conv32_pair(c, st, false, "depth_encoder3.enc2.1", A(c->e3_1, H2, W2), Bl, Bl, H2, W2, raw(A(c->e3_2a, H4, W4)), "depth_encoder3.enc2.3", Bl, e)); }
#undef CR
        return 0;
    };
    if (two) {
        hipStream_t sp = s2 ? s2 : s;
        if (s2) { HIPCHK(hipEventRecord(c->ev_fork, s)); HIPCHK(hipStreamWaitEvent(s2, c->ev_fork, 0)); }
        c->stamp(3, sp);
        if (s2 && c->thru_active && c->cnt_sparse) REST_(s2, ptta_launch_loss_valid_count(c->cnt_sparse, c->cnt_validity, c->N, c->H, c->W, c->loss_ws, s2));
        RUN(meta_forward_proxy(c, sp));
        c->stamp(1, s);
        RUN(region(s, 0, Nn, false));
        c->stamp(2, s);
        RUN(region(sp, Nn, Nn, true));
        c->stamp(4, sp);
        const bool hn = c->nar_heads && heads_v2_on(c);
        if (!hn) RUN(to_wide(c, c->tw(c->feat), (float*)c->feat + (size_t)c->Rg * 32, c->Rg * 32, sp));
        if (s2) {
            if (hn) RUN(heads_forward(c, s2, 1));
            c->stamp(5, s2);
            HIPCHK(hipEventRecord(c->ev_real, s)); HIPCHK(hipStreamWaitEvent(s2, c->ev_real, 0));
            RUN(heads_forward(c, s2, hn ? 2 : 0));
            c->stamp(6, s2);
            HIPCHK(hipEventRecord(c->ev_join, s2));
        }
    } else {
        RUN(region(s, 0, B2, false));
        if (train && s2) {
            HIPCHK(hipEventRecord(c->ev_fork, s)); HIPCHK(hipStreamWaitEvent(s2, c->ev_fork, 0));
            if (c->thru_active && c->cnt_sparse) REST_(s2, ptta_launch_loss_valid_count(c->cnt_sparse, c->cnt_validity, c->N, c->H, c->W, c->loss_ws, s2));
            RUN(heads_forward(c, s2));
            HIPCHK(hipEventRecord(c->ev_join, s2));
        }
    }
    if (!c->skip_dec3) {
    CV("depth_decoder3.dec2.1", false, CONV_T2, c->w2, B2, Nn, H4, W4, true, e_raw(c->t3));
    { E e; e.sum = c->s1_3; e.add1 = c->e3_1; e.add1_nb = B2; e.add2 = c->c1; e.add2_nb = B2;
      CV("depth_decoder3.dec2.3", false, CONV_S1, c->t3, Nn, Nn, H2, W2, true, e); }
    CV("depth_decoder3.dec1.1", false, CONV_T2, c->s1_3, Nn, Nn, H2, W2, true, e_raw(c->u3));
    { E e; e.sum = c->s0_3; e.add1 = c->e3_0; e.add1_nb = B2; e.add2 = c->c0; e.add2_nb = B2;
      CV("depth_decoder3.dec1.3", false, CONV_S1, c->u3, Nn, Nn, H1, W1, true, e); }
    CV("depth_decoder3.prdct.1", false, CONV_S1, c->s0_3, Nn, Nn, H1, W1, true, e_raw(c->v3));
    {
        const LOut& lo = c->lout["depth_decoder3.prdct.3"];
        ConvOut1Args a; a.in = c->v3; a.in_nb = Nn; a.w = lo.w; a.bias = lo.bias; a.add = c->p11; a.add_nb = B2; a.out = c->depth_net;
        a.B = Nn; a.H = H1; a.W = W1; a.relu_in = 1; a.bf16 = c->bf16;
        RUN(conv_out1_p(c, a, s));
    }
    }
    c->stamp(7, s);
    if (train) {
        if (s2) { if (!c->thru_active) HIPCHK(hipStreamWaitEvent(s, c->ev_join, 0)); }
        else RUN(heads_forward(c, s));
    }
    return 0;
}

bool heads_v2_on(const ptta_ctx* c) {
    return c->heads_v2 && c->fuse_heads && c->fused_pp_valid && c->x3 && !c->bf16 && !c->naive && !c->skip_dec3 && !c->head_swap;
}

static int mlp_forward(ptta_ctx* c, const std::string& name, const void* A, int a_bf16, int K, float* hidden, float* out, hipStream_t s) {
    const Lin& l0 = c->fc[name + ".0"]; const Lin& l3 = c->fc[name + ".3"]; BNorm& bn = c->bn[name + ".1"];
    const int R = (int)c->Rg;
    GemmArgs g; g.A = A; g.a_bf16 = a_bf16; g.W = l0.W; g.bias = l0.bias; g.C = hidden; g.R = R; g.K = K; g.N = 512; g.epi = 1; g.part = c->bn_part;
    g.x3 = c->x3; g.Whi = l0.Whi; g.Wlo = l0.Wlo; g.Wil = l0.Wil;
    RUN(ptta_launch_gemm(g, s));
    RUN(ptta_stat_sync(&c->stat_sync, c->bn_part, ptta_gemm_part_blocks(g), 512, 1, s));
    RUN(ptta_launch_bn_finalize(c->bn_part, ptta_gemm_part_blocks(g), R * (c->stat_sync.world > 1 ? c->stat_sync.world : 1), 512, bn.gamma, bn.beta, 1e-5f, 0.1f, bn.rm, bn.rv, bn.nbt,
                                bn.mean, bn.inv, bn.scale, bn.shift, s));
    GemmArgs g2; g2.A = hidden; g2.W = l3.W; g2.bias = l3.bias; g2.C = out; g2.R = R; g2.K = 512; g2.N = 512; g2.pro = 1;
    g2.pscale = bn.scale; g2.pshift = bn.shift;
    g2.x3 = c->x3; g2.Whi = l3.Whi; g2.Wlo = l3.Wlo; g2.Wil = l3.Wil;
    RUN(ptta_launch_gemm(g2, s));
    return 0;
}

int heads_forward(ptta_ctx* c, hipStream_t s, int part) {
    if (part != 1) c->cos_rows_done = false;
    const double esh = (c->nar_heads && heads_v2_on(c)) ? 2.0 : 4.0;
    ProfScope ps_(c, 6, s, (double)c->Rg * 2 * 32 * 4 + ((double)c->Rg * (2 * 512 + 4 * 1024) + 2 * 16384.0 + 4 * 262144.0) * esh,
                  (double)c->Rg * (2 * 16384.0 + 4 * 262144.0), heads_v2_on(c) ? 7 : 8);
    const size_t half = (size_t)c->Rg * 32 * c->es;
    const void* feat_zero = (const char*)c->feat + half;
    if (c->nar_heads && heads_v2_on(c)) {
        const Lin& l0 = c->fc["proj.0"]; const Lin& lf = c->fused_pp; const Lin& lp3 = c->fc["pred.3"]; const Lin& l3 = c->fc["proj.3"];
        BNorm& b1 = c->bn["proj.1"]; BNorm& b2 = c->bn["pred.1"];
        const long R = c->Rg; const int Rw = (int)R * (c->stat_sync.world > 1 ? c->stat_sync.world : 1);
        const int nbh = 2, nb = ptta_hn_row_blocks(R);
        float* part_real = c->hm_part; float* part_zero = c->hm_part + (size_t)nbh * 2 * 512;
        double* msc_real = c->hn_msc; double* msc_zero = c->hn_msc + (size_t)ptta_hn_moment_scratch(R);
        HnBnOut bo1; bo1.gamma = b1.gamma; bo1.beta = b1.beta; bo1.rm = b1.rm; bo1.rv = b1.rv; bo1.nbt = b1.nbt;
        bo1.mean = b1.mean; bo1.inv = b1.inv; bo1.scale = b1.scale; bo1.shift = b1.shift;
        auto gemm_h = [&](const void* x, int x_bf16, const Lin& w, bf16_t* out, int epi) {
            HnGemmArgs g; g.pro = 3; g.epi = epi; g.X = x; g.x_bf16 = x_bf16; g.W0 = l0.Whi; g.b0 = l0.bias; g.pscale = b1.scale; g.pshift = b1.shift;
            g.W = w.Wsl; g.bias = w.bias; g.C = out; g.part = c->bn_part; g.R = R;
            return g;
        };
        if (part != 2) {
            const void* xz = c->nar_proxy ? (const void*)c->tw(c->feat) : (const void*)((const float*)c->feat + (size_t)R * 32);
            if (!c->stat_sync.on()) RUN(ptta_launch_hn_moments(xz, c->nar_proxy ? 1 : 0, R, 1, l0.W, l0.bias, msc_zero, nullptr, &bo1, s));
            else {
            RUN(ptta_launch_hn_moments(xz, c->nar_proxy ? 1 : 0, R, 1, l0.W, l0.bias, msc_zero, part_zero, nullptr, s));
            RUN(ptta_stat_sync(&c->stat_sync, part_zero, nbh, 512, 1, s));
            RUN(ptta_launch_bn_finalize(part_zero, nbh, Rw, 512, b1.gamma, b1.beta, 1e-5f, 0.1f, b1.rm, b1.rv, b1.nbt, b1.mean, b1.inv, b1.scale, b1.shift, s));
            }
            if (c->nar_proxy) RUN(ptta_launch_hn_gemm(gemm_h(c->tw(c->feat), 1, lf, c->h2_n, 1), s));
            else RUN(ptta_launch_hn_gemm(gemm_h((const float*)c->feat + (size_t)R * 32, 0, lf, c->h2_n, 1), s));
            RUN(ptta_stat_sync(&c->stat_sync, c->bn_part, nb, 512, 1, s));
            RUN(ptta_launch_bn_finalize(c->bn_part, nb, Rw, 512, b2.gamma, b2.beta, 1e-5f, 0.1f, b2.rm, b2.rv, b2.nbt, b2.mean, b2.inv, b2.scale, b2.shift, s));
            HnGemmArgs g3; g3.pro = 1; g3.epi = 2; g3.A = c->h2_n; g3.pscale = b2.scale; g3.pshift = b2.shift; g3.W = lp3.Wsl; g3.bias = lp3.bias; g3.C = c->emb_n; g3.R = R;
            g3.rs = c->hn_rs;
            RUN(ptta_launch_hn_gemm(g3, s));
        }
        if (part != 1) {
            if (!c->stat_sync.on()) RUN(ptta_launch_hn_moments(c->feat, 0, R, 1, l0.W, l0.bias, msc_real, nullptr, &bo1, s));
            else {
            RUN(ptta_launch_hn_moments(c->feat, 0, R, 1, l0.W, l0.bias, msc_real, part_real, nullptr, s));
            RUN(ptta_stat_sync(&c->stat_sync, part_real, nbh, 512, 1, s));
            RUN(ptta_launch_bn_finalize(part_real, nbh, Rw, 512, b1.gamma, b1.beta, 1e-5f, 0.1f, b1.rm, b1.rv, b1.nbt, b1.mean, b1.inv, b1.scale, b1.shift, s));
            }
            HnGemmArgs gr = gemm_h(c->feat, 0, l3, c->ref_n, 5);
            gr.E = c->emb_n; gr.rs = c->hn_rs; gr.rowstats_out = c->loss_ws + ptta_loss_ws_rows_off(c->N);
            gr.cpart = c->loss_ws + ptta_loss_ws_cos_off(c->N, c->Rg); gr.cpart_n = ptta_loss_cos_blocks(c->Rg);
// ... 131 lines not shown
```

tta-depth-completion_amd/csrc/msgchn_step.hip:

```cpp
#include "msgchn_ctx.h"

using namespace msgchn;

namespace msgchn {

void pipe_overwritten(ptta_ctx* c, int p) {
    ptta_ctx::PreSet& P = c->pset[p];
    if (c->pipe_cur == p) { P.prepared = false; P.prep_token = 0; }
    P.last_token = 0;
}

static void pipe_save(ptta_ctx* c, ptta_ctx::PreSet& P) { static_cast<PrefixBufs&>(P) = *c; }
void pipe_use(ptta_ctx* c, int p) {
    if (p == c->cur_set) return;
    pipe_save(c, c->pset[c->cur_set]);
    static_cast<PrefixBufs&>(*c) = c->pset[p];
    c->cur_set = p;
}
static int pipe_init(ptta_ctx* c) {
    if (c->pipe_ready) return 0;
    const int Nn = c->Nn, B2 = 2 * Nn, H1 = c->Hp, W1 = c->Wp;
    const size_t es = c->es;
    auto A = [&](int nb, int h, int w) { return c->dalloc((size_t)nb * h * w * 32 * es); };
    pipe_save(c, c->pset[c->cur_set]);
// ... 43 lines not shown
    RUN(enc1_head_fn(c, s));
    RUN(stage1_independent(c, 2 * c->Nn, s));
    c->stamp(13, s);
    return 0;
}
template <class F>
static int pipe_capture(ptta_ctx* c, hipGraph_t* g_out, hipGraphExec_t* e_out, F body) {
    if (!c->cap_stream) HIPCHK(hipStreamCreateWithFlags(&c->cap_stream, hipStreamNonBlocking));
    HIPCHK(hipStreamBeginCapture(c->cap_stream, hipStreamCaptureModeThreadLocal));
    const int rc = body(c->cap_stream);
    hipGraph_t g = nullptr;
    const hipError_t e = hipStreamEndCapture(c->cap_stream, &g);
    if (rc != 0) { if (g) (void)hipGraphDestroy(g); return rc; }
    if (e != hipSuccess || !g) return c->fail(std::string("hipStreamEndCapture: ") + hipGetErrorString(e), -100 - (int)e);
    *g_out = g;
    HIPCHK(hipGraphInstantiate(e_out, g, nullptr, nullptr, 0));
    return 0;
}

}

static int step_tail(ptta_handle c, const float* loss_image, const float* sparse, const float* validity, ptta_stream s_) {
    hipStream_t s = (hipStream_t)s_;
    auto sync_and_adam = [&](bool stamp9) -> int {
        if (c->grad_comm && ptta_rccl_allreduce_mean_f32(c->grad_comm, c->grad_arena, c->grad_arena_n, s_)) return c->fail(std::string("gradient all-reduce: ") + ptta_rccl_last_error(), -5);
        if (stamp9) c->stamp(9, s);
        if (!c->adam_fused) RUN(ptta_adam_step(c, nullptr, nullptr, s_));
        return 0;
    };
    if (c->thru_active) {
        hipStream_t s2 = c->aux(s);
        if (!c->ev_dpart) HIPCHK(hipEventCreateWithFlags(&c->ev_dpart, kStepEvent));
        if (!(c->nar_heads && heads_v2_on(c) && c->cos_rows_done)) REST_(s2, ptta_launch_loss_cos_part(c->emb, c->ref, c->Rg, 512, c->N, c->loss_ws, s2));
        HIPCHK(hipEventRecord(c->ev_dpart, s2));
        REST_(s2, ptta_launch_loss_cos_coef(c->loss_ws, c->N, c->Rg, c->hyper + 5, s2));
        HIPCHK(hipStreamWaitEvent(s, c->ev_dpart, 0));
        if (!c->ev_loss) HIPCHK(hipEventCreateWithFlags(&c->ev_loss, kStepEvent));
        c->loss_report.image = loss_image; c->loss_report.sparse = sparse; c->loss_report.validity = validity; c->loss_report.on = true;
        REST_(s, ptta_launch_loss_backward(final_depth(c), loss_image, sparse, validity, c->hp.max_input_depth, nullptr, nullptr, c->Rg, 512,
                                           c->N, c->H, c->W, c->loss_ws, c->g_final, nullptr, s, c->hyper + 5, nullptr, 1, 1));
        c->cos_in_gemm = true;
        const int rc_h = heads_backward(c, c->gref_buf, s2);
        c->cos_in_gemm = false;
        if (rc_h) return rc_h;
        c->stamp(8, s2);
        HIPCHK(hipEventRecord(c->ev_join, s2));
        const float* g_net = c->g_final;
        if (c->dual) {
            scatter_dual_grad_launch(c->g_final, c->g_net, c->N, c->H, c->W, c->Hp, c->Wp, c->pt, c->pr, s);
            g_net = c->g_net;
        }
        c->adam_fuse_req = true; c->adam_fused = false;
        const int rc_bb = backbone_backward(c, g_net, s, true);
        c->adam_fuse_req = false;
        if (rc_bb) return rc_bb;
        const int rc_a = sync_and_adam(true);
        if (rc_a) return rc_a;
        c->stamp(10, s);
        return 0;
    }
    if (c->nar_heads && heads_v2_on(c)) {
        RUN(ptta_launch_hn_untile(c->emb_n, c->emb, c->Rg, s));
        RUN(ptta_launch_hn_untile(c->ref_n, c->ref, c->Rg, s));
    }
    REST_(s, ptta_launch_loss_forward(final_depth(c), loss_image, sparse, validity, c->hp.max_input_depth, c->emb, c->ref, c->Rg, 512,
                                      c->hyper + 5, c->N, c->H, c->W, c->loss_ws, c->loss_info_dst ? c->loss_info_dst : c->loss_info, s, 1));
    const bool cig = c->cos_grad_fused && heads_v2_on(c) && c->N <= 16;
    REST_(s, ptta_launch_loss_backward(final_depth(c), loss_image, sparse, validity, c->hp.max_input_depth, c->emb, c->ref, c->Rg, 512,
                                       c->N, c->H, c->W, c->loss_ws, c->g_final, cig ? nullptr : c->gref_buf, s, c->hyper + 5, c->loss_info_dst ? c->loss_info_dst : c->loss_info));
    c->cos_in_gemm = cig;
    c->adam_fuse_req = true; c->adam_fused = false;
    const int rc_b = ptta_backward(c, c->g_final, c->gref_buf, nullptr, nullptr, s_);
    c->cos_in_gemm = false; c->adam_fuse_req = false;
    if (rc_b) return rc_b;
    return sync_and_adam(false);
}

static bool thru_ok(ptta_ctx* c, hipStream_t s) {
    return c->thru && c->cos_grad_fused && heads_v2_on(c) && c->N <= 16 && c->aux(s) != nullptr;
}
static int step_body(ptta_handle c, const float* image, const float* loss_image, const float* sparse, const float* validity,
                     ptta_stream s_) {
    c->pair_fuse_count = 0;
    RUN(ensure_fused_heads(c, (hipStream_t)s_));
    c->thru_active = thru_ok(c, (hipStream_t)s_);
    c->cnt_sparse = c->thru_active ? sparse : nullptr; c->cnt_validity = validity;
    const int rc = ptta_forward_train(c, image, sparse, nullptr, nullptr, nullptr, s_);
    if (rc) { c->thru_active = false; c->cnt_sparse = nullptr; return rc; }
    const int rc2 = step_tail(c, loss_image, sparse, validity, s_);
    c->thru_active = false; c->cnt_sparse = nullptr; c->loss_report.on = false;
    return rc2;
}

extern "C" {

int ptta_step(ptta_handle c, const float* image, const float* loss_image, const float* sparse, const float* validity,
              float* depth_out, float* loss_info_out, ptta_stream s_) {
    if (c) c->err_code = 0;
    if (!c || !image || !sparse) return -1;
    if (c->nl) return c->nl->step(image, loss_image, sparse, validity, depth_out, loss_info_out, (hipStream_t)s_);
    RUN(pipe_quiesce(c));
    hipStream_t s = (hipStream_t)s_;
    if (!loss_image) loss_image = image;
    const size_t ibytes = (size_t)c->N * 3 * c->H * c->W * 4, pbytes = (size_t)c->N * c->H * c->W * 4;
    if (c->use_graph && !c->prof_on) {
        const int key = (validity ? 2 : 0) | (loss_image != image ? 1 : 0);
        HIPCHK(d2d_copy(c->in_image, image, ibytes, s));
        HIPCHK(d2d_copy(c->in_sparse, sparse, pbytes, s));
        if (key & 1) HIPCHK(d2d_copy(c->in_loss_image, loss_image, ibytes, s));
        if (key & 2) HIPCHK(d2d_copy(c->in_validity, validity, pbytes, s));
        RUN(ensure_fused_heads(c, s));
        if (!c->gexec[key]) {
            RUN(ensure_proxy_rgb(c, c->in_image, s));
            RUN(ensure_adam_table(c, s));
            const int rc = pipe_capture(c, &c->graph[key], &c->gexec[key], [&](hipStream_t cs) {
                return step_body(c, c->in_image, (key & 1) ? c->in_loss_image : c->in_image, c->in_sparse, (key & 2) ? c->in_validity : nullptr, (ptta_stream)cs);
            });
            if (rc) return rc;
        }
        HIPCHK(hipGraphLaunch(c->gexec[key], s));
        if (!c->ev_replay) HIPCHK(hipEventCreateWithFlags(&c->ev_replay, hipEventDisableTiming));
        HIPCHK(hipEventRecord(c->ev_replay, s));
        c->fwd_valid = true;
    } else {
        c->loss_info_dst = loss_info_out;
        const int rc = step_body(c, image, loss_image, sparse, validity, s_);
        c->loss_info_dst = nullptr;
        if (rc) return rc;
        if (depth_out) HIPCHK(d2d_copy(depth_out, final_depth(c), pbytes, s));
        return 0;
    }
    if (depth_out) HIPCHK(d2d_copy(depth_out, final_depth(c), pbytes, s));
    if (loss_info_out) HIPCHK(d2d_copy(loss_info_out, c->loss_info, 16, s));
    return 0;
}

int ptta_pipeline_stream(ptta_handle c, ptta_stream* out) {
    if (!c || !out) return -1;
    if (c->nl) return c->fail("frame pipelining is built for MSG_CHN handles", -38);
    RUN(pipe_init(c));
    *out = (ptta_stream)c->pre_stream;
    return 0;
}

int ptta_step_pipelined(ptta_handle c, const float* image, const float* loss_image, const float* sparse, const float* validity, uint64_t frame_token,
                        const float* next_image, const float* next_sparse, uint64_t next_token, float* depth_out, float* loss_info_out, ptta_stream s_) {
    if (c) c->err_code = 0;
    if (!c || !image || !sparse) return -1;
    if (c->nl || c->prof_on || c->dual || c->stat_sync.on() || c->grad_comm || c->naive || c->bf16) {
        const int rc = ptta_step(c, image, loss_image, sparse, validity, depth_out, loss_info_out, s_);
        if (!c->nl) { c->fb_image = rc ? nullptr : image; c->fb_sparse = rc ? nullptr : sparse; }
        return rc;
    }
    hipStream_t s = (hipStream_t)s_;
    if (!loss_image) loss_image = image;
    RUN(pipe_init(c));
    c->pipe_active = true;
    const size_t ibytes = (size_t)c->N * 3 * c->H * c->W * 4, pbytes = (size_t)c->N * c->H * c->W * 4;
    const int p = c->pipe_cur, q = 1 - p;
    const int key = (validity ? 2 : 0) | (loss_image != image ? 1 : 0);
    if (c->pipe_stream_set && c->pipe_stream != s) { HIPCHK(hipEventRecord(c->ev_rest[0], c->pipe_stream)); HIPCHK(hipStreamWaitEvent(s, c->ev_rest[0], 0)); }
    c->pipe_stream = s; c->pipe_stream_set = true;
    HIPCHK(hipEventRecord(c->ev_entry, s));
    pipe_use(c, p);
    RUN(ensure_fused_heads(c, s));
    if (!c->proxy_valid) RUN(ensure_proxy_rgb(c, c->in_image, s));
// ... 67 lines not shown
```

tta-depth-completion_amd/csrc/ptta_api.hip:

```cpp
#include "msgchn_ctx.h"

using namespace msgchn;

int msgchn::ensure_adam_table(ptta_ctx* c, hipStream_t s) {
    if (!c->adam_tab_dirty) return 0;
    for (auto& ad : c->adapted) if (!ad.p || !ad.m || !ad.v) return 0;
    c->adam_host.resize(c->adapted.size());
    long off = 0;
    for (size_t k = 0; k < c->adapted.size(); ++k) { auto& ad = c->adapted[k]; c->adam_host[k] = PttaAdamEntry{ad.p, ad.m, ad.v, ad.g, ad.n, off}; off += ad.n; }
    HIPCHK(hipMemcpyAsync(c->adam_tab, c->adam_host.data(), c->adam_host.size() * sizeof(PttaAdamEntry), hipMemcpyHostToDevice, s));
    c->adam_tab_dirty = false;
    return 0;
}

extern "C" {

int ptta_version(void) { return PTTA_ABI_VERSION; }

static thread_local std::string g_create_err;
static int create_refused(const std::string& why) { g_create_err = why; return -38; }

const char* ptta_last_error(ptta_handle h) {
    if (!h) return g_create_err.empty() ? "null handle" : g_create_err.c_str();
    return h->nl && h->err.empty() ? h->nl->err.c_str() : h->err.c_str();
// ... 303 lines not shown
    if ((gw || gb) && c->meta_mode != PTTA_META_1LAYER) return c->fail("explicit gradients are a 1layer convenience; use the internal ones", -22);
    hipStream_t s = (hipStream_t)s_;
    if (!gw && !gb) {
        RUN(ensure_adam_table(c, s));
        long total = 0; for (auto& ad : c->adapted) total += ad.n;
        REST_(s, ptta_launch_adam_multi(c->adam_tab, (int)c->adapted.size(), total, c->hyper, c->step_dev, c->adam_ticket, s));
        return 0;
    }
    RUN(ptta_launch_step_inc(c->step_dev, s));
    for (size_t k = 0; k < c->adapted.size(); ++k) {
        auto& ad = c->adapted[k];
        const float* g = ad.g;
        if (c->meta_mode == PTTA_META_1LAYER) { if (k == 0 && gw) g = gw; if (k == 1 && gb) g = gb; }
        RUN(ptta_launch_adam(ad.p, ad.m, ad.v, g, ad.n, c->hyper, c->step_dev, s));
    }
    return 0;
}

int ptta_set_image_norm(ptta_handle c, float divisor, const float* mean, const float* stdv) {
    NLFWD(c->nl->set_image_norm(divisor, mean, stdv));

    if (!c) return -1;
    if (!(divisor > 0.f)) return c->fail("ptta_set_image_norm: divisor must be positive", -22);
    ImgNorm nm = ImgNorm{0, divisor, {0.f, 0.f, 0.f}, {1.f, 1.f, 1.f}};
    for (int k = 0; k < 3; ++k) {
        if (mean) nm.mean[k] = mean[k];
        if (stdv) { if (!(stdv[k] > 0.f)) return c->fail("ptta_set_image_norm: std must be positive", -22); nm.stdv[k] = stdv[k]; }
    }
    nm.on = !(divisor == 1.f && nm.mean[0] == 0.f && nm.mean[1] == 0.f && nm.mean[2] == 0.f && nm.stdv[0] == 1.f &&
              nm.stdv[1] == 1.f && nm.stdv[2] == 1.f);
    c->img_norm = nm;
    c->drop_graphs();
    return 0;
}

static int set_stat_sync(ptta_ctx* c, const PttaStatSync& sy, bool on, bool keeps_graph) {
    if (c->nl && !c->nl->one_rank_why.empty()) { c->err.clear(); return c->nl->fail(c->nl->one_rank_why, -38); }
    if (c->nl && c->nl->meta_only) { c->err.clear(); return c->nl->fail("the SyncBatchNorm form of the meta-only adaptation mode is not offered (PTTA_ADAPT_META_ONLY)", -38); }
    if (c->nl) { c->err.clear(); c->nl->drop_graphs(); c->nl->stat_sync = sy; return 0; }
    if (on && c->meta_mode == PTTA_META_2LAYERS && !c->m2.generic) return c->fail("SyncBatchNorm needs the default arithmetic for the 2layers meta layer", -38);
    c->stat_sync = sy;
    c->drop_graphs();
    if (on) {
        if (c->pre_sync_graph < 0) { c->pre_sync_graph = c->use_graph; c->pre_sync_aux = c->use_aux; }
        else if (keeps_graph) c->use_graph = c->pre_sync_graph;
        if (!keeps_graph) c->use_graph = 0;
        c->use_aux = 0;
    } else if (c->pre_sync_graph >= 0) {
        c->use_graph = c->pre_sync_graph; c->use_aux = c->pre_sync_aux; c->pre_sync_graph = c->pre_sync_aux = -1;
    }
    return 0;
}

int ptta_set_stat_sync(ptta_handle c, ptta_allreduce_fn fn, void* user, double* exchange_buf, int64_t capacity, int world_size) {
    if (!c || world_size < 1 || (world_size > 1 && (!fn || !exchange_buf || capacity < 2 * 1024))) return -22;
    PttaStatSync sy; sy.fn = (ptta_allreduce_cb)fn; sy.user = user; sy.buf = exchange_buf; sy.cap = (long)capacity; sy.world = world_size;
    return set_stat_sync(c, sy, world_size > 1, false);
}

int ptta_set_stat_sync_rccl(ptta_handle c, void* comm, double* exchange_buf, int64_t capacity, int world_size) {
    if (!c || world_size < 1 || (comm && (!exchange_buf || capacity < 2 * 1024))) return -22;
    PttaStatSync sy; sy.comm = comm; sy.buf = exchange_buf; sy.cap = (long)capacity; sy.world = world_size;
    return set_stat_sync(c, sy, comm != nullptr, true);
}

int ptta_set_grad_sync_rccl(ptta_handle c, void* comm) {
    if (!c) return -1;
    if (c->nl && !c->nl->one_rank_why.empty()) { c->err.clear(); return c->nl->fail(c->nl->one_rank_why, -38); }
    if (c->nl && c->nl->meta_only) { c->err.clear(); return c->nl->fail("no gradient exchange in the meta-only adaptation mode: more than one rank is not offered (PTTA_ADAPT_META_ONLY)", -38); }
    if (c->nl) { c->nl->drop_graphs(); c->nl->grad_comm = comm; return 0; }
    c->grad_comm = comm;
    c->drop_graphs();
    return 0;
}

struct Option { const char* key; int ptta_ctx::*member; int hi; bool mixed_free; };
static const Option kOptions[] = {
    {"aux_stream", &ptta_ctx::use_aux, 1, true},        {"thru", &ptta_ctx::thru, 1, true},
    {"adam_in_wgrad", &ptta_ctx::adam_in_wgrad, 1, true}, {"bwd_w2", &ptta_ctx::bwd_w2, 1, true},
    {"fuse_first", &ptta_ctx::fuse_first, 2, false},    {"fuse_head_bwd", &ptta_ctx::fuse_head_bwd, 1, false},
    {"fuse_heads", &ptta_ctx::fuse_heads, 1, false},    {"heads_v2", &ptta_ctx::heads_v2, 1, false},
    {"cos_in_gemm", &ptta_ctx::cos_grad_fused, 1, false}, {"mask_bits", &ptta_ctx::mask_bits_on, 1, false},
    {"stamps", &ptta_ctx::stamps, 1, true},             {"pair_fuse", &ptta_ctx::pair_fuse, 1, true},
};
static const Option* find_option(const std::string& k) {
    for (const Option& o : kOptions) if (k == o.key) return &o;
    return nullptr;
}
int ptta_set_option(ptta_handle c, const char* key, int value) {
    if (!c || !key) return -1;
    const std::string k(key);
    if (k == "graph") return ptta_set_graph(c, value);
    if (k == "eval_bn_fused") {
        if (!c->nl || !c->nl->meta_only) return c->nl ? (c->err.clear(), c->nl->fail("ptta_set_option: 'eval_bn_fused' belongs to PTTA_ADAPT_META_ONLY handles", -38))
                                                      : c->fail("ptta_set_option: 'eval_bn_fused' belongs to PTTA_ADAPT_META_ONLY handles", -38);
        c->err.clear();
        if (value < 0 || value > 1) return c->nl->fail("ptta_set_option: value out of range for 'eval_bn_fused'", -22);
        if (c->nl->eval_bn_fused != value) { c->nl->drop_graphs(); c->nl->eval_bn_fused = value; }
        return 0;
    }
    if (k == "head_bn_fused" || k == "head_bn_fused_count") {
        if (!c->nl) return c->fail("ptta_set_option: '" + k + "' belongs to the generic engine's handles (MSG_CHN has no BatchNorm2d)", -38);
        c->err.clear();
        if (k == "head_bn_fused_count") return c->nl->fail("ptta_set_option: 'head_bn_fused_count' is read-only", -22);
        if (value < 0 || value > 1) return c->nl->fail("ptta_set_option: value out of range for 'head_bn_fused'", -22);
        if (c->nl->head_bn_fused != value) { c->nl->drop_graphs(); c->nl->head_bn_fused = value; }
        return 0;
    }
    if (c->nl) return -38;
    if (k == "pair_fuse_count") return c->fail("ptta_set_option: 'pair_fuse_count' is read-only", -22);
    const Option* o = find_option(k);
    if (!o) return c->fail("ptta_set_option: unknown key '" + k + "'", -22);
    int* f = &(c->*(o->member));
    if (value < 0 || value > o->hi) return c->fail("ptta_set_option: value out of range for '" + k + "'", -22);
    if (c->mixed && !o->mixed_free && value != 1)
        return c->fail("ptta_set_option: the mixed mode is defined on the default kernels ('" + k + "' stays 1)", -38);
    if (k == "aux_stream" && c->pre_sync_graph >= 0) { c->pre_sync_aux = value; return 0; }
    if (*f == value) return 0;
    RUN(pipe_quiesce(c));
    c->drop_graphs();
    *f = value;
    return 0;
}

int ptta_get_option(ptta_handle c, const char* key, int* value) {
    if (!c || !key || !value) return -1;
    const std::string k(key);
    if (k == "pipelined_active") { *value = !(c->nl || c->prof_on || c->dual || c->stat_sync.on() || c->grad_comm || c->naive || c->bf16); return 0; }
    if (k == "thru_active") { *value = c->nl ? 0 : (c->thru && c->cos_grad_fused && heads_v2_on(c) && c->use_aux); return 0; }
    if (k == "eval_bn_fused") { if (!c->nl || !c->nl->meta_only) return -38; *value = c->nl->eval_bn_fused; return 0; }
    if (k == "head_bn_fused" || k == "head_bn_fused_count") {
        if (!c->nl) return -38;
        *value = k == "head_bn_fused" ? c->nl->head_bn_fused : c->nl->head_bn_fused_count();
        return 0;
    }
    if (c->nl) { if (k != "graph") return -38; *value = c->nl->use_graph; return 0; }
    if (k == "graph") { *value = c->use_graph; return 0; }
    if (k == "pair_fuse_count") { *value = c->pair_fuse_count; return 0; }
    const Option* o = find_option(k);
    if (!o) return -22;
    *value = c->*(o->member);
    return 0;
}

int ptta_set_graph(ptta_handle c, int enable) {
    if (c && c->nl) { c->nl->use_graph = enable ? 1 : 0; if (!enable) c->nl->drop_graphs(); return 0; }

    if (!c) return -1;
    if (enable && c->stat_sync.on() && !c->stat_sync.comm) return c->fail("graph replay is not available with SyncBatchNorm exchange (ptta_set_stat_sync)", -38);
    c->use_graph = enable ? 1 : 0;
    if (!enable) c->drop_graphs();
    return 0;
}

int ptta_profile(ptta_handle c, int enable) {
    if (c && c->nl) return c->fail("not available for the NLSPN / CostDCNet backbones: use ptta_step / ptta_forward_*", -38);

    if (!c) return -1;
    c->prof_on = enable != 0;
    for (auto& pc : c->prof) { pc.used = 0; pc.bytes = 0; pc.macs = 0; pc.launches = 0; }
    c->prof_seq.clear();
    return 0;
}

int ptta_profile_read(ptta_handle c, int klass, double* ms_total, double* alg_bytes, double* macs, int64_t* launches, ptta_stream s_) {
    if (c && c->nl) return c->fail("not available for the NLSPN / CostDCNet backbones: use ptta_step / ptta_forward_*", -38);

    if (!c || klass < 0 || klass >= ptta_ctx::NPROF) return -1;
    HIPCHK(hipStreamSynchronize((hipStream_t)s_));
    ptta_ctx::ProfClass& pc = c->prof[klass];
    double ms = 0;
    for (size_t k = 0; k < pc.used; ++k) {
        float t = 0.f;
        HIPCHK(hipEventElapsedTime(&t, pc.ev[k].first, pc.ev[k].second));
        ms += t;
    }
    if (ms_total) *ms_total = ms;
    if (alg_bytes) *alg_bytes = pc.bytes;
    if (macs) *macs = pc.macs;
    if (launches) *launches = (int64_t)pc.launches;
    return 0;
}

int ptta_debug_tensor(ptta_handle c, const char* name, float* dst, int64_t capacity, int64_t* numel_host, ptta_stream s_) {
    NLFWD(c->nl->debug_tensor(name, dst, capacity, numel_host, (hipStream_t)s_));

    if (!c || !name) return -1;
    if (std::string(name) == "prof_seq") {
        HIPCHK(hipStreamSynchronize((hipStream_t)s_));
        const int64_t n = 2 * (int64_t)c->prof_seq.size();
        if (numel_host) *numel_host = n;
        if (!dst) return 0;
        if (capacity < n) return c->fail("capacity too small", -22);
        std::vector<float> h((size_t)n);
        for (size_t k = 0; k < c->prof_seq.size(); ++k) {
            const auto& q = c->prof_seq[k];
            float t = 0.f;
            HIPCHK(hipEventElapsedTime(&t, c->prof[q.first].ev[q.second].first, c->prof[q.first].ev[q.second].second));
            h[2 * k] = (float)q.first; h[2 * k + 1] = 1e3f * t;
        }
        HIPCHK(hipMemcpy(dst, h.data(), (size_t)n * 4, hipMemcpyHostToDevice));
        return 0;
    }
    auto it = c->dbg.find(name);
    if (it == c->dbg.end()) return c->fail(std::string("no debug tensor ") + name, -2);
    if (numel_host) *numel_host = it->second.numel;
    if (!dst) return 0;
    if (capacity < it->second.numel) return c->fail("capacity too small", -22);
    hipStream_t s = (hipStream_t)s_;
    const long n = it->second.numel;
    if (it->second.is_act == 3) RUN(ptta_launch_hn_untile(it->second.p, dst, n / 512, s));
    else if ((it->second.is_act == 1 && c->bf16) || it->second.is_act == 2) to_f32_launch((const bf16_t*)it->second.p, dst, n, s);
    else HIPCHK(hipMemcpyAsync(dst, it->second.p, (size_t)n * 4, hipMemcpyDeviceToDevice, s));
    return 0;
}

}
```

tta-depth-completion_amd/csrc/ptta_kernels.h:

```cpp
#pragma once
#include <hip/hip_runtime.h>
#include <cstdlib>
#include <cstring>
#include "ptta_common.h"

struct PttaCreateEnv { int naive = 0, exact = 0, graph = -1; };
inline PttaCreateEnv ptta_create_env() {
    PttaCreateEnv e;
    const char* v = getenv("PTTA_CONV_IMPL"); e.naive = (v && strcmp(v, "naive") == 0) ? 1 : 0;
    v = getenv("PTTA_ARITH"); e.exact = (v && strcmp(v, "exact") == 0) ? 1 : 0;
    v = getenv("PTTA_GRAPH"); e.graph = (v && (strcmp(v, "0") == 0 || strcmp(v, "1") == 0)) ? (v[0] - '0') : -1;
    return e;
}

struct ConvW {
    float* mf32;
    bf16_t* mbf16;
    bf16_t* mlo;
    float* canon;
};
struct Conv32Args {
    const void* in = nullptr; int in_nb = 1;
    const ConvW* w = nullptr;
    const float* bias = nullptr;
    const void* up = nullptr; int up_nb = 1;
    const void* mask = nullptr; int mask_nb = 1;
    const void* add1 = nullptr; int add1_nb = 1;
    const void* add2 = nullptr; int add2_nb = 1;
    void* out_raw = nullptr; void* out_sum = nullptr;
    int B = 1, Hin = 0, Win = 0;
    int mode = CONV_S1; int relu_in = 0; int bf16 = 0; int naive = 0;
    int x3 = 0;
    int w2 = 0;
    const uint32_t* mask_bits = nullptr;
    uint32_t* bits_out = nullptr; int bits_nb = 0; int bits_sum = 0;
};
void ptta_pack_conv32(const float* src, const ConvW& w, int in_major, int flip, hipStream_t s, int row_stride = 32, int col_off = 0);
int ptta_launch_conv32(const Conv32Args& a, hipStream_t s);
bool ptta_conv32_pair_applies(const Conv32Args& first, const Conv32Args& second);
int ptta_launch_conv32_pair(const Conv32Args& first, const Conv32Args& second, hipStream_t s);
int ptta_launch_conv32_loop(const Conv32Args& a, void* buf_a, void* buf_b, int reps, unsigned* ctr, unsigned* base_io, int* err, int variant, hipStream_t s);

struct Plane { const float* p = nullptr; int nb = 1; long bstride = 0;
               int norm = 0; float div = 1.f, mean = 0.f, stdv = 1.f; };
struct ConvInArgs {
    Plane pl[3]; int cin = 1; int zero_from_b = 1 << 30;
    const float* wfrag = nullptr;
    const float* wcanon = nullptr;
    const float* bias = nullptr;
    const void* up = nullptr; int up_nb = 1;
    const void* mask = nullptr; int mask_nb = 1;
    const void* add1 = nullptr; int add1_nb = 1;
    void* out_raw = nullptr; void* out_sum = nullptr;
    int B = 1, H = 0, W = 0; int bf16 = 0; int naive = 0;
    const uint32_t* mask_bits = nullptr; uint32_t* a_bits = nullptr;
    int a_bits_nb = 0;
};
void ptta_pack_conv_in(const float* src, int cin_total, int cin_first, int cin, int transpose_flip,
                       float* wfrag, float* wcanon, hipStream_t s);
int ptta_launch_conv_in(const ConvInArgs& a, hipStream_t s);
int ptta_launch_conv32_first(const Conv32Args& a, const ConvInArgs& f, void* a_out, int a_nb, hipStream_t s);

struct ConvOut1Args {
    const void* in = nullptr; int in_nb = 1;
    const float* w = nullptr;
    const float* bias = nullptr;
    const float* add = nullptr; int add_nb = 1;
    float* out = nullptr;
    int B = 1, H = 0, W = 0; int relu_in = 0; int bf16 = 0;
};
void ptta_pack_conv_out1(const float* src, int src_cin_total, int src_cin_index, int from_conv_in, float* w, hipStream_t s);
int ptta_launch_conv_out1(const ConvOut1Args& a, hipStream_t s);

int ptta_launch_prep(const float* sparse, float max_input_depth, float* dclamp, float* d12, float* d14,
                     int N, int H, int W, hipStream_t s);
int ptta_launch_up2_1ch(const float* in, float* out, int B, int Hin, int Win, hipStream_t s);
int ptta_launch_up2T_1ch(const float* gout, float* gin, int B, int Hin, int Win, hipStream_t s);
int ptta_launch_up2T_32(const void* gout, const void* add, void* gin, int B, int Hin, int Win, int bf16, hipStream_t s);

int ptta_launch_outlier_removal(const float* sparse, const float* validity, float* sparse_out, float* validity_out,
                                int N, int H, int W, int ksize, float threshold, float* scratch, hipStream_t s);

typedef int (*ptta_allreduce_cb)(void* user, double* dev_buf, long long count, void* stream);
int ptta_rccl_sum_f64(void* comm, double* buf, long long count, hipStream_t s);
struct PttaStatSync {
    ptta_allreduce_cb fn = nullptr; void* user = nullptr;
    void* comm = nullptr;
    double* buf = nullptr; long cap = 0; int world = 1;
    bool on() const { return (fn || comm) && (world > 1 || comm); }
    int exchange(long long count, hipStream_t s) const {
        if (comm) return ptta_rccl_sum_f64(comm, buf, count, s);
        const int rc = fn(user, buf, count, (void*)s);
        return rc ? (rc < 0 ? rc : -rc) : 0;
    }
};
int ptta_stat_sync(const PttaStatSync* sy, float* part, int nblocks, int C, int npass, hipStream_t s);
int ptta_grad_mean_sync(const PttaStatSync* sy, float* g, long n, hipStream_t s);

struct GemmArgs {
    const void* A = nullptr; int a_bf16 = 0;
    const float* A2 = nullptr;
    const float* W = nullptr;
    const float* bias = nullptr;
    float* C = nullptr;
    int R = 0, K = 0, N = 0;
    int pro = 0;
    const float* pscale = nullptr; const float* pshift = nullptr;
    const float* pmean = nullptr; const float* pinv = nullptr;
    const float* pc1 = nullptr; const float* pc2 = nullptr;
    int epi = 0;
    const float* eH = nullptr;
    const float* escale = nullptr; const float* eshift = nullptr; const float* emean = nullptr; const float* einv = nullptr;
    float* part = nullptr;
    int x3 = 0; const bf16_t* Whi = nullptr; const bf16_t* Wlo = nullptr;
    const bf16_t* Wil = nullptr;
    const float* X = nullptr;
    const void* W0frag = nullptr;
    const float* b0 = nullptr;
    const bf16_t* W0hi = nullptr; const bf16_t* W0lo = nullptr;
    const bf16_t* W0thi = nullptr; const bf16_t* W0tlo = nullptr;
    float* P = nullptr;
    const float* Bref = nullptr; const float* rowstats = nullptr; const float* coef = nullptr;
};
// ... 206 lines not shown
```

tta-depth-completion_amd/csrc/ptta_ops.hip:

```cpp
#include "msgchn_ctx.h"
#include "gnet.h"
#include "costdc.h"

using namespace msgchn;

namespace {
struct ScratchConvW {
    ConvW w{};
    bool ok;
    ScratchConvW() {
        ok = hipMalloc((void**)&w.mf32, 9 * 4 * 64 * 4 * 4) == hipSuccess && hipMalloc((void**)&w.mbf16, 9 * 2 * 64 * 8 * 2) == hipSuccess &&
             hipMalloc((void**)&w.canon, 9216 * 4) == hipSuccess && hipMalloc((void**)&w.mlo, 9 * 2 * 64 * 8 * 2) == hipSuccess;
    }
    ~ScratchConvW() { (void)hipFree(w.mf32); (void)hipFree(w.mbf16); (void)hipFree(w.mlo); (void)hipFree(w.canon); }
    ScratchConvW(const ScratchConvW&) = delete;
    ScratchConvW& operator=(const ScratchConvW&) = delete;
};

__global__ void op_scale_f64_kernel(double* buf, long long n, double f) {
    for (long long i = (long long)blockIdx.x * blockDim.x + threadIdx.x; i < n; i += (long long)gridDim.x * blockDim.x) buf[i] *= f;
}
int op_gbn_exchange(void* user, double* buf, long long count, void* stream) {
    long long blocks = (count + 255) / 256; if (blocks > 1024) blocks = 1024; if (blocks < 1) blocks = 1;
    hipLaunchKernelGGL(op_scale_f64_kernel, dim3((int)blocks), dim3(256), 0, (hipStream_t)stream, buf, count, (double)*(const int*)user);
    return hipGetLastError() == hipSuccess ? 0 : -5;
}
}

extern "C" {

int ptta_outlier_removal(const float* sparse, const float* validity, float* sparse_out, float* validity_out, int n, int height,
                         int width, int kernel_size, float threshold, float* scratch, ptta_stream s) {
    if (!sparse || !validity || !sparse_out || !validity_out || !scratch || n < 1 || height < 1 || width < 1 || kernel_size < 1 ||
        (kernel_size & 1) == 0) return -22;
    return ptta_launch_outlier_removal(sparse, validity, sparse_out, validity_out, n, height, width, kernel_size, threshold, scratch,
                                       (hipStream_t)s);
}

int ptta_eval_metrics(const float* depth, const float* ground_truth, int64_t numel, float min_evaluate_depth, float max_evaluate_depth,
                      void* scratch, float* metrics_out, ptta_stream s) {
    if (!depth || !ground_truth || !scratch || !metrics_out || numel < 1) return -22;
    return ptta_launch_eval_metrics(depth, ground_truth, numel, min_evaluate_depth, max_evaluate_depth, (double*)scratch, metrics_out,
                                    (hipStream_t)s);
}

static void dcn_args(DcnArgs& a, const float* input, const float* weight, const float* bias, const float* offset, const float* mask,
                     int b, int c, int h, int w, int c_out, int kh, int kw, int sh, int sw, int ph, int pw, int dh, int dw, int group, int dg) {
    a.in = input; a.weight = weight; a.bias = bias; a.offset = offset; a.mask = mask;
    a.B = b; a.C = c; a.H = h; a.W = w; a.Co = c_out; a.kh = kh; a.kw = kw; a.sh = sh; a.sw = sw; a.ph = ph; a.pw = pw;
    a.dh = dh; a.dw = dw; a.group = group; a.dg = dg;
}

int ptta_mdconv_forward(const float* input, const float* weight, const float* bias, const float* offset, const float* mask, float* output,
                        int b, int c, int h, int w, int c_out, int kh, int kw, int sh, int sw, int ph, int pw, int dh, int dw,
                        int group, int deformable_group, ptta_stream s) {
    if (!input || !weight || !offset || !mask || !output) return -22;
    DcnArgs a; dcn_args(a, input, weight, bias, offset, mask, b, c, h, w, c_out, kh, kw, sh, sw, ph, pw, dh, dw, group, deformable_group);
    a.out = output;
    return ptta_launch_dcn_forward(a, (hipStream_t)s);
}

int ptta_mdconv_backward(const float* input, const float* weight, const float* bias, const float* offset, const float* mask,
                         const float* grad_output, float* grad_input, float* grad_offset, float* grad_mask, float* grad_weight,
                         float* grad_bias, int b, int c, int h, int w, int c_out, int kh, int kw, int sh, int sw, int ph, int pw,
                         int dh, int dw, int group, int deformable_group, ptta_stream s) {
    if (!input || !weight || !offset || !mask || !grad_output) return -22;
    DcnArgs a; dcn_args(a, input, weight, bias, offset, mask, b, c, h, w, c_out, kh, kw, sh, sw, ph, pw, dh, dw, group, deformable_group);
    a.gout = grad_output; a.gin = grad_input; a.goff = grad_offset; a.gmask = grad_mask; a.gweight = grad_weight; a.gbias = grad_bias;
    return ptta_launch_dcn_backward(a, (hipStream_t)s);
}

int ptta_op_conv32(const float* in, const float* weight, const float* bias, float* out, int b, int hin, int win, int mode,
                   int relu_in, int in_major, int flip, int dtype, int naive, ptta_stream s_) {
    hipStream_t s = (hipStream_t)s_;
    ScratchConvW sw; ConvW& w = sw.w;
    void *tin = nullptr, *tout = nullptr;
    const int ho = mode == CONV_S1 ? hin : (mode == CONV_S2 ? hin / 2 : hin * 2), wo = mode == CONV_S1 ? win : (mode == CONV_S2 ? win / 2 : win * 2);
    const long nin = (long)b * hin * win * 32, nout = (long)b * ho * wo * 32;
    int rc = 0;
    if (!sw.ok || hipMalloc(&tin, nin * 2) != hipSuccess || hipMalloc(&tout, nout * 2) != hipSuccess) rc = -12;
    if (rc == 0) {
        ptta_pack_conv32(weight, w, in_major, flip, s);
        Conv32Args a; a.w = &w; a.bias = bias; a.B = b; a.Hin = hin; a.Win = win; a.mode = mode; a.relu_in = relu_in; a.naive = naive & 1; a.x3 = (naive >> 1) & 1;
        if (dtype != PTTA_DTYPE_F32) {
            from_f32_launch(in, (bf16_t*)tin, nin, s);
            a.in = tin; a.in_nb = b; a.out_raw = tout; a.bf16 = 1;
            rc = ptta_launch_conv32(a, s);
            to_f32_launch((const bf16_t*)tout, out, nout, s);
        } else {
            a.in = in; a.in_nb = b; a.out_raw = out; a.bf16 = 0;
            rc = ptta_launch_conv32(a, s);
        }
        (void)hipStreamSynchronize(s);
    }
    (void)hipFree(tin); (void)hipFree(tout);
    return rc;
}

int ptta_op_conv32_pair(const float* in, const float* weight1, const float* bias1, const float* weight2, const float* bias2, const float* up,
                        const float* add0, const float* add1, const float* add2, const uint32_t* mask1_bits, const uint32_t* mask2_bits,
                        float* out_raw, float* out_sum, float* mid_raw, float* mid_sum, uint32_t* mid_bits, int b, int in_nb,
                        int hin, int win, int first_mode, int relu1, int relu2, int in_major, int flip, int dtype, int w2, int fused,
                        int* fused_host, ptta_stream s_) {
    hipStream_t s = (hipStream_t)s_;
    if (!in || !weight1 || !weight2 || (!out_raw && !out_sum) || b < 1 || in_nb < 1 || in_nb > b || hin < 1 || win < 1 ||
        (first_mode != CONV_S2 && first_mode != CONV_T2) || (add2 && !add1) || (add1 && !out_sum)) return -22;
    const bool nar = dtype != PTTA_DTYPE_F32;
    if (w2 && (!nar || relu1 || relu2 || up)) return -22;
    const int hm = first_mode == CONV_S2 ? hin / 2 : hin * 2, wm = first_mode == CONV_S2 ? win / 2 : win * 2;
    if (hm < 1 || wm < 1) return -22;
    const long nin = (long)in_nb * hin * win * 32, nm = (long)b * hm * wm * 32, nu = (long)b * (hm / 2) * (wm / 2) * 32;
    ScratchConvW sw1, sw2;
    void* t[9] = {nullptr, nullptr, nullptr, nullptr, nullptr, nullptr, nullptr, nullptr, nullptr};
    const long cnt[9] = {nin, up ? nu : 0, add0 ? nm : 0, add1 ? nm : 0, add2 ? nm : 0, nm, add0 ? nm : 0, out_raw ? nm : 0, out_sum ? nm : 0};
    const float* src[5] = {in, up, add0, add1, add2};
    const int es = nar ? 2 : 4;
    int rc = (sw1.ok && sw2.ok) ? 0 : -12;
    for (int k = 0; k < 9 && !rc; ++k) if (cnt[k] > 0 && hipMalloc(&t[k], (size_t)cnt[k] * es) != hipSuccess) rc = -12;
    if (!rc) {
        ptta_pack_conv32(weight1, sw1.w, in_major, flip, s);
        ptta_pack_conv32(weight2, sw2.w, 0, 0, s);
        for (int k = 0; k < 5; ++k) {
            if (cnt[k] <= 0) continue;
            if (nar) from_f32_launch(src[k], (bf16_t*)t[k], cnt[k], s);
            else if (hipMemcpyAsync(t[k], src[k], (size_t)cnt[k] * 4, hipMemcpyDeviceToDevice, s) != hipSuccess) rc = -5;
        }
        (void)hipMemsetAsync(t[5], 0xff, (size_t)nm * es, s);
        if (t[6]) (void)hipMemsetAsync(t[6], 0xff, (size_t)nm * es, s);
    }
    if (!rc) {
        Conv32Args f, g;
        f.in = t[0]; f.in_nb = in_nb; f.w = &sw1.w; f.bias = bias1; f.out_raw = t[5]; f.B = b; f.Hin = hin; f.Win = win; f.mode = first_mode;
        f.relu_in = relu1; f.bf16 = nar ? 1 : 0; f.x3 = 1; f.w2 = w2;
        if (add0) { f.add1 = t[2]; f.add1_nb = b; f.out_sum = t[6]; }
        if (mask1_bits) { f.mask = mask1_bits; f.mask_nb = b; f.mask_bits = mask1_bits; }
        if (!nar && mid_bits) { f.bits_out = mid_bits; f.bits_nb = b; }
        g.in = add0 ? t[6] : t[5]; g.in_nb = b; g.w = &sw2.w; g.bias = bias2; g.up = t[1]; g.up_nb = b;
        g.add1 = t[3]; g.add1_nb = b; g.add2 = t[4]; g.add2_nb = b;
        if (mask2_bits) { g.mask = mask2_bits; g.mask_nb = b; g.mask_bits = mask2_bits; }
        g.out_raw = t[7]; g.out_sum = t[8]; g.B = b; g.Hin = hm; g.Win = wm; g.mode = CONV_S1; g.relu_in = relu2; g.bf16 = nar ? 1 : 0; g.x3 = 1; g.w2 = w2;
        int did = 0;
        rc = fused ? ptta_launch_conv32_pair(f, g, s) : 1;
        if (rc == 0) did = 1;
        if (rc == 1) { rc = ptta_launch_conv32(f, s); if (!rc) rc = ptta_launch_conv32(g, s); }
        if (fused_host) *fused_host = did;
    }
    if (!rc) {
        float* dst[4] = {mid_raw, mid_sum, out_raw, out_sum};
        for (int k = 0; k < 4; ++k) {
            if (!dst[k] || !t[5 + k]) continue;
            if (nar) to_f32_launch((const bf16_t*)t[5 + k], dst[k], nm, s);
            else if (hipMemcpyAsync(dst[k], t[5 + k], (size_t)nm * 4, hipMemcpyDeviceToDevice, s) != hipSuccess) rc = -5;
        }
    }
    if (hipStreamSynchronize(s) != hipSuccess && !rc) rc = -5;
    for (int k = 0; k < 9; ++k) (void)hipFree(t[k]);
    return rc;
}

int ptta_op_gwgrad(const float* x, const float* gy, float* gw, float* gb, int b, int h, int w, int ci, int co, int impl, int reps,
                   float* us_per_call_host, ptta_stream s_) {
    hipStream_t s = (hipStream_t)s_;
    if (!x || !gy || !gw || b < 1 || h < 1 || w < 1 || ci < 1 || co < 1 || ci > 256 || co > 256 || impl < 0 || impl > 2 || reps < 0 ||
        (reps > 0 && !us_per_call_host)) return -22;
    GView xv, gv;
    xv.p = (float*)x; xv.B = b; xv.H = h; xv.W = w; xv.C = ci; xv.ld = ci;
    gv.p = (float*)gy; gv.B = b; gv.H = h; gv.W = w; gv.C = co; gv.ld = co;
    const long P = (long)b * h * w;
    const size_t nm = (size_t)ptta_gwgrad_mfma_part_floats(P, ci, co), nn = (size_t)ptta_gwgrad_slabs(P) * (9 * ci * co + co);
    float* part = nullptr;
    if (hipMalloc((void**)&part, (impl == 2 ? nn : nm) * 4) != hipSuccess) return -12;
    auto run = [&]() {
        return impl == 0 ? ptta_launch_gwgrad_mfma(xv, gv, part, gw, gb, s)
                         : (impl == 1 ? ptta_launch_gwgrad_f32mfma(xv, gv, part, gw, gb, s) : ptta_launch_gwgrad(xv, gv, part, gw, gb, s));
    };
    int rc = run();
    if (!rc && reps > 0) {
        hipEvent_t e0 = nullptr, e1 = nullptr;
        if (hipEventCreate(&e0) != hipSuccess || hipEventCreate(&e1) != hipSuccess) rc = -5;
        if (!rc) {
            (void)hipEventRecord(e0, s);
            for (int r = 0; r < reps && !rc; ++r) rc = run();
            (void)hipEventRecord(e1, s);
            (void)hipEventSynchronize(e1);
            float ms = 0.f; (void)hipEventElapsedTime(&ms, e0, e1);
            *us_per_call_host = 1e3f * ms / (float)reps;
        }
        if (e0) (void)hipEventDestroy(e0);
        if (e1) (void)hipEventDestroy(e1);
    }
    if (hipStreamSynchronize(s) != hipSuccess && !rc) rc = -5;
    (void)hipFree(part);
    return rc;
}

static int op_gconv(const float* x0, int c0, int ld0, const float* x1, int c1, int ld1, const float* weight, const float* bias, float* y, int co,
                    int ldy, int b, int hin, int win, int hout, int wout, int k, int geom, int act, int accumulate, int impl, int flags,
                    int six_b, int x1_from_b, int stat_npass, double* stat_host, int* form_host, bool affine, const float* scale, const float* shift,
                    const float* res, int ld_res, ptta_stream s_) {
    hipStream_t s = (hipStream_t)s_;
    if (affine) {
        const int cm = geom == PTTA_GCONV_S1 ? 7 : 15;
        if (!scale || !shift || (((size_t)scale | (size_t)shift) & 15) || (res != nullptr) != (ld_res != 0) || (res && ld_res < co) ||
            impl != 0 || accumulate || stat_npass || six_b < 0 || six_b > b || (flags & PTTA_GCONV_DGRAD) || (act != GACT_NONE && act != GACT_RELU && act != GACT_LRELU) ||
            c0 < 1 || c1 < 0 || (c0 & cm) || (c1 & cm)) return -22;
        const bool af = flags & PTTA_GCONV_AFF_ACT_FIRST, rp = flags & PTTA_GCONV_AFF_RES_PLAIN;
        if ((af && rp) || (af && (!res || act != GACT_RELU || (flags & PTTA_GCONV_VERT))) || (rp && (!res || act != GACT_NONE))) return -22;
        if (geom == PTTA_GCONV_T2 && (af || six_b > 0)) return -22;
    } else if (flags & (PTTA_GCONV_AFF_ACT_FIRST | PTTA_GCONV_AFF_RES_PLAIN)) return -22;
    const bool vert = flags & PTTA_GCONV_VERT, dgrad = flags & PTTA_GCONV_DGRAD;
    if (!x0 || !weight || !y || b < 1 || hin < 1 || win < 1 || hout < 1 || wout < 1 || c0 < 1 || c1 < 0 || co < 1 || ld0 < c0 || ldy < co ||
        (c1 > 0) != (x1 != nullptr) || (c1 > 0 && ld1 < c1) || (k != 1 && k != 3) || geom < PTTA_GCONV_S1 || geom > PTTA_GCONV_T2 ||
        act < GACT_NONE || act > GACT_SIGMOID || impl < 0 || impl > 1 || (flags & ~31) || six_b < 0 || six_b > b || x1_from_b < 0 ||
        stat_npass < 0 || stat_npass > 2 || (accumulate & ~1)) return -22;
    if (vert && (k != 3 || geom != PTTA_GCONV_S1)) return -22;
    if (dgrad && (c1 > 0 || six_b > 0)) return -22;
    if (stat_npass > 0 && (!stat_host || geom != PTTA_GCONV_S1 || impl != 0 || dgrad || (b % stat_npass))) return -22;
    const int run = !dgrad ? geom : (geom == PTTA_GCONV_S2 ? PTTA_GCONV_T2 : (geom == PTTA_GCONV_T2 ? PTTA_GCONV_S2 : PTTA_GCONV_S1));
    const bool size_ok = run == PTTA_GCONV_S1 ? (hout == hin && wout == win)
                       : run == PTTA_GCONV_S2 ? (hout == (hin + 1) / 2 && wout == (win + 1) / 2)
                       : ((hout == 2 * hin || (dgrad && hout == 2 * hin - 1)) && (wout == 2 * win || (dgrad && wout == 2 * win - 1)));
    if (!size_ok) return -22;
    if (impl == 0 && ((((size_t)x0 | (size_t)x1) & 15) || (ld0 & 3) || (ld1 & 3))) return -22;
    if (form_host) *form_host = -1;

    gnet::GConvW cw;
    cw.k = k; cw.stride = geom == PTTA_GCONV_S1 ? 1 : 2; cw.transposed = geom == PTTA_GCONV_T2 ? 1 : 0; cw.vcol = vert ? 1 : 0;
    if (!dgrad) { cw.Ci = c0 + c1; cw.Co = co; cw.C0 = c0; cw.C1 = c1; }
    else { cw.Ci = co; cw.Co = c0; cw.C0 = co; cw.C1 = 0; }
    cw.mf = impl == 0 && !dgrad; cw.mb = impl == 0 && dgrad;
    const int KK = k * k;
    const size_t nw = (size_t)KK * cw.Ci * cw.Co;
    const size_t nfrag = cw.mf ? (size_t)ptta_gfrag_elems(KK, cw.C0, cw.C1, cw.Co) : (cw.mb ? (size_t)ptta_gfrag_elems(KK, cw.Co, 0, cw.Ci) : 0);
    const int tiles_pp = stat_npass ? ptta_gconv_x3_tiles(b / stat_npass, hout, wout) : 0;
    const size_t nstat = (size_t)stat_npass * tiles_pp * 2 * co;
    float* wbuf = nullptr; bf16_t* fbuf = nullptr; float* stat = nullptr;
    int rc = 0;
    if (hipMalloc((void**)&wbuf, 2 * nw * sizeof(float)) != hipSuccess || (nfrag && hipMalloc((void**)&fbuf, 3 * nfrag * sizeof(bf16_t)) != hipSuccess) ||
        (nstat && hipMalloc((void**)&stat, nstat * sizeof(float)) != hipSuccess)) rc = -12;
    if (!rc && (hipMemsetAsync(wbuf, 0, 2 * nw * sizeof(float), s) != hipSuccess || (nstat && hipMemsetAsync(stat, 0, nstat * sizeof(float), s) != hipSuccess))) rc = -5;
// ... 389 lines not shown
```

tta-depth-completion_amd/proxytta/_lib.py:

```python
import ctypes
import os
from ctypes import POINTER, byref, c_char_p, c_float, c_int, c_int64, c_uint64, c_void_p


_HERE = os.path.dirname(os.path.abspath(__file__))
LIB_PATH = os.path.join(_HERE, 'libptta_hip.so')

PTTA_BACKBONE_MSG_CHN = 0
PTTA_BACKBONE_NLSPN = 1
PTTA_BACKBONE_COSTDCNET = 2
PTTA_NLSPN_LEGACY_OFFSET = 0x100
PTTA_NLSPN_SYNCBN_ADAPT = 0x200
PTTA_SYNCBN_ADAPT = 0x200
PTTA_ADAPT_META_ONLY = 0x400
PTTA_META_1LAYER = 0
PTTA_META_2LAYERS = 1
PTTA_META_NONE = 2
PTTA_DTYPE_F32 = 0
PTTA_DTYPE_MIXED = 1
PTTA_HEAD_FORM_PLAIN = 0
PTTA_HEAD_FORM_SYNCBN = 1
PTTA_GCONV_VERT = 1
PTTA_GCONV_X1_W2 = 2
PTTA_GCONV_DGRAD = 4
# ... 15 lines not shown

class GbnArgs(ctypes.Structure):
    _fields_ = ([(n, c_int) for n in ('mode', 'b', 'h', 'w', 'npass', 'act', 'act_first', 'res_relu', 'acc_gx', 'acc_gres', 'world',
                                      'nblocks_in', 'repeats')] + [('eps', c_float), ('momentum', c_float)] +
                [(n, GbnView) for n in ('x', 'res', 'y', 'g', 'gx', 'gres')] +
                [(n, c_void_p) for n in ('gamma', 'beta', 'part_in', 'st', 'rm', 'rv', 'nbt', 'st_eval', 'dgamma', 'dbeta')])


class CdSbnArgs(ctypes.Structure):
    _fields_ = ([(n, c_int) for n in ('mode', 'level', 'c', 'relu', 'repeats', 'world', 'acc_res')] +
                [(n, c_void_p) for n in ('f', 'res', 'y', 'g', 'gamma', 'beta', 'rm', 'rv', 'nbt', 'out', 'st', 'dgamma', 'dbeta', 'gx', 'gres')])


CD_OPS = {'pad_dual': 0, 'crop_avg': 1, 'scatter_dual_grad': 2, 'stage': 3, 'clamp': 4, 'fusion_fwd': 5, 'fusion_bwd': 6, 'pool_fwd': 7,
          'pool_bwd': 8, 'up_fwd': 9, 'up_bwd': 10, 'regress_fwd': 11, 'regress_bwd': 12, 'rows_fwd': 13, 'rows_bwd': 14}

_P = c_void_p
SIGNATURES = [
    ('ptta_create', c_int, [POINTER(c_void_p), c_int, c_int, c_int, c_int, c_int, c_int, POINTER(Hparams)]),
    ('ptta_destroy', None, [_P]),
    ('ptta_last_error', c_char_p, [_P]),
    ('ptta_set_hparams', c_int, [_P, POINTER(Hparams), _P]),
    ('ptta_load_weights', c_int, [_P, c_char_p, _P, POINTER(c_int64), c_int, _P]),
    ('ptta_bind_adapted', c_int, [_P, c_char_p, _P, _P, _P]),
    ('ptta_set_adam_step', c_int, [_P, c_int, _P]),
    ('ptta_get_adam_step', c_int, [_P, POINTER(c_int), _P]),
    ('ptta_forward_train', c_int, [_P, _P, _P, _P, _P, _P, _P]),
    ('ptta_embedding_rows', c_int64, [_P]),
    ('ptta_forward_eval', c_int, [_P, _P, _P, _P, _P]),
    ('ptta_loss_forward', c_int, [_P, _P, _P, _P, _P, _P, _P, c_int64, c_float, c_float, c_float, _P, _P]),
    ('ptta_loss_backward', c_int, [_P, _P, _P, _P, _P, _P, _P, c_int64, _P, _P, _P]),
    ('ptta_backward', c_int, [_P, _P, _P, _P, _P, _P]),
    ('ptta_set_grad', c_int, [_P, c_char_p, _P, c_int64, _P]),
    ('ptta_get_grad', c_int, [_P, c_char_p, _P, c_int64, _P]),
    ('ptta_adapted_count', c_int, [_P]),
    ('ptta_adapted_name', c_char_p, [_P, c_int, POINTER(c_int64)]),
    ('ptta_adapted_repeat', c_int, [_P, c_int]),
    ('ptta_adam_step', c_int, [_P, _P, _P, _P]),
    ('ptta_step', c_int, [_P, _P, _P, _P, _P, _P, _P, _P]),
    ('ptta_step_pipelined', c_int, [_P] * 5 + [c_uint64] + [_P] * 2 + [c_uint64] + [_P] * 3),
    ('ptta_pipeline_stream', c_int, [_P, POINTER(c_void_p)]),
    ('ptta_forward_eval_last', c_int, [_P, _P, _P]),
    ('ptta_outlier_removal', c_int, [_P, _P, _P, _P, c_int, c_int, c_int, c_int, c_float, _P, _P]),
    ('ptta_eval_metrics', c_int, [_P, _P, c_int64, c_float, c_float, _P, _P, _P]),
    ('ptta_mdconv_forward', c_int, [_P] * 6 + [c_int] * 15 + [_P]),
    ('ptta_mdconv_backward', c_int, [_P] * 11 + [c_int] * 15 + [_P]),
    ('ptta_set_image_norm', c_int, [_P, c_float, POINTER(c_float), POINTER(c_float)]),
    ('ptta_head_bind', c_int, [_P, c_char_p, _P, _P, _P]),
    ('ptta_head_set_hparams', c_int, [_P, c_float, c_float, c_float, c_float, c_float, c_float, c_int, _P]),
    ('ptta_head_reload', c_int, [_P, _P]),
    ('ptta_head_forward', c_int, [_P, _P, _P, c_int, _P, _P, _P]),
    ('ptta_head_backward', c_int, [_P, _P, _P]),
    ('ptta_head_adam_step', c_int, [_P, _P]),
    ('ptta_head_step', c_int, [_P, _P, _P, c_int, _P, _P]),
    ('ptta_head_get_grad', c_int, [_P, c_char_p, _P, c_int64, POINTER(c_int), _P]),
    ('ptta_head_set_form', c_int, [_P, c_int]),
    ('ptta_crop_flip', c_int, [_P, _P] + [c_int] * 6 + [_P] * 5),
    ('ptta_rotate', c_int, [_P, _P, c_int, c_int, c_int, c_int, _P, _P, c_int, _P]),
    ('ptta_resize_crop', c_int, [_P, _P, c_int, c_int, c_int, c_int, _P, _P, _P, _P, _P, c_int, c_int, _P]),
    ('ptta_photometric', c_int, [_P, _P, c_int, c_int, c_int, _P, _P, _P, _P, _P, _P, _P, _P]),
    ('ptta_photometric_full', c_int, [_P, _P, c_int, c_int, c_int] + [_P] * 12),
    ('ptta_add_noise', c_int, [_P, _P, _P, c_int, c_int, c_int, c_int, _P, c_float, c_int, _P]),
    ('ptta_remove_patches', c_int, [_P, _P, c_int, c_int, c_int, c_int, _P, _P, _P, _P, _P]),
    ('ptta_crop_pad', c_int, [_P, _P, c_int, c_int, c_int, c_int] + [_P] * 7 + [c_int, c_float, _P]),
    ('ptta_resize_pad', c_int, [_P, _P, c_int, c_int, c_int, c_int] + [_P] * 5 + [c_int, c_int, c_float, _P]),
    ('ptta_set_stat_sync', c_int, [_P, _P, _P, _P, c_int64, c_int]),
    ('ptta_rccl_unique_id', c_int, [_P]),
    ('ptta_rccl_comm_create', c_int, [_P, c_int, c_int, POINTER(c_void_p)]),
    ('ptta_rccl_comm_destroy', c_int, [_P]),
    ('ptta_rccl_allreduce_mean_f32', c_int, [_P, _P, c_int64, _P]),
    ('ptta_rccl_last_error', c_char_p, []),
    ('ptta_set_stat_sync_rccl', c_int, [_P, _P, _P, c_int64, c_int]),
    ('ptta_set_grad_sync_rccl', c_int, [_P, _P]),
    ('ptta_set_graph', c_int, [_P, c_int]),
    ('ptta_set_option', c_int, [_P, c_char_p, c_int]),
    ('ptta_get_option', c_int, [_P, c_char_p, POINTER(c_int)]),
    ('ptta_profile', c_int, [_P, c_int]),
    ('ptta_profile_read', c_int, [_P, c_int, POINTER(ctypes.c_double), POINTER(ctypes.c_double), POINTER(ctypes.c_double),
                                  POINTER(c_int64), _P]),
    ('ptta_debug_tensor', c_int, [_P, c_char_p, _P, c_int64, POINTER(c_int64), _P]),
    ('ptta_op_conv32', c_int, [_P, _P, _P, _P, c_int, c_int, c_int, c_int, c_int, c_int, c_int, c_int, c_int, _P]),
    ('ptta_op_conv32_chain', c_int, [_P] * 6 + [c_int] * 7 + [POINTER(c_float), _P]),
    ('ptta_op_conv32_pair', c_int, [_P] * 16 + [c_int] * 12 + [POINTER(c_int), _P]),
    ('ptta_op_gwgrad', c_int, [_P, _P, _P, _P] + [c_int] * 7 + [POINTER(c_float), _P]),
    ('ptta_op_gconv', c_int, [_P, c_int, c_int, _P, c_int, c_int, _P, _P, _P] + [c_int] * 16 + [POINTER(ctypes.c_double), POINTER(c_int), _P]),
    ('ptta_op_gconv_affine', c_int, [_P, c_int, c_int, _P, c_int, c_int, _P, _P, _P] + [c_int] * 16 + [POINTER(ctypes.c_double), POINTER(c_int),
                                     _P, _P, _P, c_int, _P]),
    ('ptta_op_gbn', c_int, [POINTER(GbnArgs), _P]),
    ('ptta_cd_sparse_create', c_int, [POINTER(c_void_p), c_int, c_int, c_int]),
    ('ptta_cd_sparse_destroy', None, [_P]),
    ('ptta_cd_sparse_build', c_int, [_P, _P, c_float, _P]),
    ('ptta_cd_sparse_read', c_int, [_P, c_int, POINTER(c_int), _P, ctypes.c_longlong, _P, _P, _P]),
    ('ptta_op_cd_sparse_conv', c_int, [_P, _P, _P, _P] + [c_int] * 7 + [_P]),
    ('ptta_op_cd_sbn', c_int, [_P, POINTER(CdSbnArgs), _P]),
    ('ptta_op_cd_densify', c_int, [_P, _P, _P, c_int, c_int, c_int, c_int, _P]),
    ('ptta_op_cd_dense', c_int, [c_int, _P, _P, _P, _P, POINTER(c_int), POINTER(c_float), _P]),
    ('ptta_version', c_int, []),
]

_lib = None


def load():
    global _lib
    if _lib is not None:
        return _lib
    import torch
    if not os.path.exists(LIB_PATH):
        raise RuntimeError('libptta_hip.so not found at %s: build it with `python -c "import '
                           '__graft_entry__ as g; g.build()"` — there is no CPU fallback' % LIB_PATH)
    lib = ctypes.CDLL(LIB_PATH)
    for name, res, args in SIGNATURES:
        fn = getattr(lib, name)
        fn.restype = res
        fn.argtypes = args
    have = lib.ptta_version()
    if have != PTTA_ABI_VERSION:
        raise RuntimeError('%s has ABI version %d, this binding is written against %d (include/ptta.h PTTA_ABI_VERSION): rebuild it with '
                           '`make -C tta-depth-completion_amd/csrc`' % (LIB_PATH, have, PTTA_ABI_VERSION))
    _lib = lib
    return lib


def check(lib, handle, rc, what):
    if rc != 0:
        msg = lib.ptta_last_error(handle).decode() if handle else ''
        raise RuntimeError('%s failed (%d): %s' % (what, rc, msg))


def ptr(t):
    if t is None:
        return None
    assert t.is_contiguous()
    return c_void_p(t.data_ptr())


__all__ = ['load', 'check', 'ptr', 'Hparams', 'GbnArgs', 'GbnView', 'CdSbnArgs', 'CD_OPS', 'SIGNATURES', 'LIB_PATH', 'byref']
```

Measured before the change: 857.9.

## Fuse transposed-conv and following stride-1 conv into one tiled kernel

Adds a conv32_tpair kernel that computes a stride-2 transposed 3x3 conv into LDS per tile, including its halo, and immediately feeds it to the following stride-1 3x3 conv. The intermediate activation then stays on chip instead of being written to and reread from global memory, and one launch replaces two. The cost is recomputing the halo rows, higher LDS and register use per block, and intermediates that are no longer materialized, so debug reads of them are blocked. An option toggle, a 'pays' heuristic and a test entry point are added.

```diff
diff --git a/include/ptta.h b/include/ptta.h
--- a/include/ptta.h
+++ b/include/ptta.h
@@ -158,6 +158,11 @@
                         const uint32_t* mask1_bits, const uint32_t* mask2_bits, float* out_raw, float* out_sum, float* mid_raw,
                         float* mid_sum, uint32_t* mid_bits, int b, int in_nb, int hin, int win, int first_mode, int relu1, int relu2,
                         int in_major, int flip, int dtype, int w2, int fused, int* fused_host, ptta_stream s);
+int ptta_op_conv32_tpair(const float* in_nhwc, const float* weight1, const float* bias1, const float* weight2, const float* bias2,
+                         const float* up_nhwc, const float* add0_nhwc, const float* add1_nhwc, const float* add2_nhwc,
+                         const uint32_t* mask1_bits, const uint32_t* mask2_bits, float* out_raw, float* out_sum, float* mid_raw,
+                         float* mid_sum, uint32_t* mid_bits, int b, int in_nb, int hin, int win, int first_mode, int relu1, int relu2,
+                         int in_major, int flip, int dtype, int w2, int fused, int form, int max_blocks, int* fused_host, ptta_stream s);
 int ptta_op_gwgrad(const float* x_nhwc, const float* gy_nhwc, float* gw, float* gb, int b, int h, int w, int ci, int co, int impl,
                    int reps, float* us_per_call_host, ptta_stream s);
 #define PTTA_GCONV_S1 0
diff --git a/tta-depth-completion_amd/csrc/conv_tpair.hip b/tta-depth-completion_amd/csrc/conv_tpair.hip
--- /dev/null
+++ b/tta-depth-completion_amd/csrc/conv_tpair.hip
@@ -0,0 +1,354 @@
+#include <type_traits>
+#include "ptta_common.h"
+#include "ptta_kernels.h"
+
+template <typename T, int TH, bool ADD, bool DG = false>
+__global__ __launch_bounds__(256, 2) void conv32_tpair_kernel(Conv32P<T> p1, Conv32P<T> p2) {
+    static_assert(TH == 4 || TH == 8, "tile heights of the two stride-1 kernels");
+    constexpr bool F32 = sizeof(T) == 4, LO = F32 || DG, RELU = !DG;
+    static_assert(!DG || (!F32 && !ADD), "the masked / summed first half exists for the narrow data gradients");
+    constexpr int STR = Geo<T>::STR, WL = LO ? 18 * 64 * 16 : 0;
+    constexpr int PH = TH + 2;
+    constexpr int NR = TH / 2 + 1, NC = X3_PW / 2;
+    constexpr int NQ = NR * NC, NGC = (NQ + 31) / 32;
+    constexpr int WH = TH / 2 + 2, WW = X3_PW / 2 + 1, NWP = WH * WW;
+    constexpr int NIT = (((NWP + 7) / 8) * 32 + 255) / 256;
+    constexpr int WFR = 18 * 64;
+    constexpr int NPC = (LO ? 2 : 1) * 18;
+    constexpr int HALO_B = PH * X3_PW * STR, WIN_B = NWP * STR, W1_B = NPC * 1024;
+    constexpr bool W1T = LO;
+    constexpr int R_B = W1T ? (HALO_B > WIN_B + W1_B ? HALO_B : WIN_B + W1_B) : (HALO_B > WIN_B ? HALO_B : WIN_B);
+    static_assert(WIN_B % 16 == 0 && R_B % 16 == 0, "16-byte LDS pieces");
+    __shared__ __attribute__((aligned(16))) unsigned char lds[R_B + WL + (W1T ? 0 : W1_B)];
+    unsigned char* const win = lds;
+    unsigned char* const w1_lds = W1T ? lds + WIN_B : lds + R_B;
+    unsigned char* const wl_lds = lds + R_B;
+    const int tid = threadIdx.x, lane = tid & 63;
+    const int i = lane & 31, h = lane >> 5;
+    const float bias1 = epi_bias(p1.epi, i), bias2 = epi_bias(p2.epi, i);
+    const int wave = __builtin_amdgcn_readfirstlane(tid >> 6);
+    const int Hin = p1.Hin, Win = p1.Win, H = p2.Hout, W = p2.Wout;
+    const int ntx = (W + 31) >> 5, nty = (H + TH - 1) / TH;
+    const long ntiles = (long)p2.B * ntx * nty;
+    const float sy = up_scale(H >> 1, H), sx = up_scale(W >> 1, W);
+    const unsigned sched = TH == 8 ? (wave == 0 ? 0x04Cu : wave == 1 ? 0x18Du : wave == 2 ? 0x25Eu : 0x6A9u)
+                                   : (wave == 0 ? 0x0Cu : wave == 1 ? 0x1Du : wave == 2 ? 0x54u : 0x98u);
+
+    auto tile_coords = [&](long tile, int& b, int& y0, int& x0) {
+        long t_ = tile;
+        const int ty = (int)(t_ % nty); t_ /= nty;
+        const int tx = (int)(t_ % ntx);
+        b = (int)(t_ / ntx); y0 = ty * TH; x0 = tx << 5;
+    };
+    Px<T> v[NIT];
+    unsigned vok = 0;
+    auto issue_loads = [&](long tile) {
+        int b, y0, x0;
+        tile_coords(tile, b, y0, x0);
+        const T* inb = p1.in + (size_t)(b % p1.in_nb) * Hin * Win * 32;
+        vok = 0;
+#pragma unroll
+        for (int it = 0; it < NIT; ++it) {
+            const int idx = tid + 256 * it;
+            const int g = idx & 3, pix = x3_stage_pix(idx);
+            const int py = pix / WW, px = pix - py * WW;
+            const int gy = (y0 >> 1) - 1 + py, gx = (x0 >> 1) - 1 + px;
+            if (pix < NWP && gy >= 0 && gy < Hin && gx >= 0 && gx < Win) vok |= 1u << it;
+            v[it] = px_load(inb + ((size_t)min(max(gy, 0), Hin - 1) * Win + min(max(gx, 0), Win - 1)) * 32 + 8 * g);
+        }
+    };
+    if (blockIdx.x < ntiles) issue_loads(blockIdx.x);
+    uint4 wh[9][2];
+    {
+        const uint4* ph = (const uint4*)p2.wpack;
+#pragma unroll
+        for (int t = 0; t < 9; ++t)
+#pragma unroll
+            for (int k = 0; k < 2; ++k) wh[t][k] = ph[(t * 2 + k) * 64 + lane];
+        if constexpr (LO) {
+            const uint4* pl = (const uint4*)p2.wpack2;
+            for (int idx = tid; idx < WFR; idx += 256) *(uint4*)(wl_lds + idx * 16) = pl[idx];
+        } else {
+            const uint4* p1h = (const uint4*)p1.wpack;
+            for (int idx = tid; idx < WFR; idx += 256) *(uint4*)(w1_lds + idx * 16) = p1h[idx];
+        }
+    }
+
+    for (long tile = blockIdx.x; tile < ntiles; tile += gridDim.x) {
+        int b, y0, x0;
+        tile_coords(tile, b, y0, x0);
+        if constexpr (W1T) {
+#pragma unroll
+            for (int k = 0; k < (NPC + 3) / 4; ++k) {
+                const int piece = wave + 4 * k;
+                if (piece < NPC) {
+                    const unsigned char* src = (const unsigned char*)(piece < 18 ? p1.wpack : p1.wpack2) + ((size_t)(piece < 18 ? piece : piece - 18) * 64 + lane) * 16;
+                    __builtin_amdgcn_global_load_lds((const __attribute__((address_space(1))) void*)src,
+                                                     (__attribute__((address_space(3))) void*)(w1_lds + piece * 1024), 16, 0, 0);
+                }
+            }
+        }
+#pragma unroll
+        for (int it = 0; it < NIT; ++it) {
+            const int idx = tid + 256 * it;
+            const int pix = x3_stage_pix(idx);
+            Px<T> x = v[it];
+            if (!((vok >> it) & 1u)) x = px_zero<T>();
+            if (pix < NWP) px_stage<RELU>(x, win + pix * STR + 16 * (idx & 3), Geo<T>::LO);
+        }
+        uint32_t mw1[DG ? NGC : 1][4];
+        uint2 a1v[DG ? NGC : 1][4];
+        if constexpr (DG) {
+            const int tq_ = (i & 3) + 4 * h;
+#pragma unroll
+            for (int s_ = 0; s_ < NGC; ++s_) {
+                const int code = (int)((sched >> (4 * s_)) & 15u);
+#pragma unroll
+                for (int j = 0; j < 4; ++j) {
+                    const int qc = min(32 * (code & 3) + 8 * j + tq_, NQ - 1);
+                    const int rr = qc / NC, jj = qc - rr * NC;
+                    const int row = 2 * rr + ((code & 8) ? 0 : 1), col = 2 * jj + ((code & 4) ? 0 : 1);
+                    const size_t cpix = (size_t)min(max(y0 - 1 + row, 0), H - 1) * W + min(max(x0 - 1 + col, 0), W - 1);
+                    mw1[s_][j] = p1.epi.mask_bits[(size_t)(b % p1.epi.mask_nb) * H * W + cpix];
+                    a1v[s_][j] = *(const uint2*)((const bf16_t*)p1.epi.add1 + ((size_t)(b % p1.epi.add1_nb) * H * W + cpix) * 32 + 4 * (i >> 2));
+                }
+            }
+        }
+        if constexpr (W1T) asm volatile("s_waitcnt vmcnt(0)" ::: "memory");
+        lds_barrier();
+
+        const bool wbits = F32 && p1.epi.bits_out != nullptr && b < p1.epi.bits_nb;
+        const bool wmap = p1.epi.out_raw != nullptr;
+        uint2 keep_hi[NGC][4], keep_lo[F32 ? NGC : 1][4];
+#pragma unroll
+        for (int s_ = 0; s_ < NGC; ++s_) {
+            const int code = (int)((sched >> (4 * s_)) & 15u);
+            const bool yo = code & 8, xo = code & 4;
+            const int gi = code & 3;
+            f32x16 acc;
+#pragma unroll
+            for (int r = 0; r < 16; ++r) acc[r] = 0.f;
+            {
+                const int q = min(32 * gi + i, NQ - 1);
+                const int rr = q / NC, j = q - rr * NC;
+                const unsigned char* const abase = win + (rr * WW + j) * STR + 16 * h;
+                const unsigned char* const wbase = w1_lds + lane * 16;
+                auto mma_class = [&](auto yo_c, auto xo_c) __attribute__((always_inline)) {
+                    constexpr bool YO = decltype(yo_c)::value, XO = decltype(xo_c)::value;
+                    constexpr int NS = (YO ? 2 : 1) * (XO ? 2 : 1) * 2;
+                    constexpr int AHEAD = F32 ? 1 : 2, RING = AHEAD + 1;
+                    uint4 fah[RING], fbh[RING], fal[F32 ? RING : 1], fbl[LO ? RING : 1];
+                    auto frag_load = [&](const int n_) __attribute__((always_inline)) {
+                        const int t_ = n_ >> 1, k = n_ & 1;
+                        const int ky = YO ? 2 * (t_ / (XO ? 2 : 1)) : 1, kx = XO ? 2 * (t_ % 2) : 1;
+                        const int tap = ky * 3 + kx;
+                        const unsigned char* a = abase + ((ky == 2 ? 0 : 1) * WW + (kx == 2 ? 0 : 1)) * STR + 32 * k;
+                        fah[n_ % RING] = *(const uint4*)a;
+                        fbh[n_ % RING] = *(const uint4*)(wbase + (tap * 2 + k) * 1024);
+                        if constexpr (F32) fal[n_ % RING] = *(const uint4*)(a + Geo<T>::LO);
+                        if constexpr (LO) fbl[n_ % RING] = *(const uint4*)(wbase + (WFR * 16 + (tap * 2 + k) * 1024));
+                    };
+#pragma unroll
+                    for (int n_ = 0; n_ < AHEAD; ++n_) frag_load(n_);
+#pragma unroll
+                    for (int n_ = 0; n_ < NS; ++n_) {
+                        if (n_ + AHEAD < NS) frag_load(n_ + AHEAD);
+                        __builtin_amdgcn_sched_barrier(0);
+                        const bf16x8 ah = __builtin_bit_cast(bf16x8, fah[n_ % RING]), bh = __builtin_bit_cast(bf16x8, fbh[n_ % RING]);
+                        if constexpr (F32) {
+                            acc = __builtin_amdgcn_mfma_f32_32x32x16_bf16(__builtin_bit_cast(bf16x8, fal[n_ % RING]), bh, acc, 0, 0, 0);
+                            acc = __builtin_amdgcn_mfma_f32_32x32x16_bf16(ah, __builtin_bit_cast(bf16x8, fbl[n_ % RING]), acc, 0, 0, 0);
+                        } else if constexpr (DG) {
+                            acc = __builtin_amdgcn_mfma_f32_32x32x16_bf16(ah, __builtin_bit_cast(bf16x8, fbl[n_ % RING]), acc, 0, 0, 0);
+                        }
+                        acc = __builtin_amdgcn_mfma_f32_32x32x16_bf16(ah, bh, acc, 0, 0, 0);
+                        __builtin_amdgcn_sched_barrier(0);
+                    }
+                };
+                typedef std::integral_constant<bool, true> Y_; typedef std::integral_constant<bool, false> N_;
+                if (yo) { if (xo) mma_class(Y_{}, Y_{}); else mma_class(Y_{}, N_{}); }
+                else { if (xo) mma_class(N_{}, Y_{}); else mma_class(N_{}, N_{}); }
+            }
+            f32x16 t;
+#pragma unroll
+            for (int r = 0; r < 16; ++r) t[r] = acc[r] + bias1;
+            quad_transpose(t, lane);
+            const int tq = (i & 3) + 4 * h, c4 = 4 * (i >> 2);
+#pragma unroll
+            for (int j = 0; j < 4; ++j) {
+                const int qq = 32 * gi + 8 * j + tq, qc = min(qq, NQ - 1);
+                const int rr = qc / NC, jj = qc - rr * NC;
+                const int row = 2 * rr + (yo ? 0 : 1), col = 2 * jj + (xo ? 0 : 1);
+                const int my = y0 - 1 + row, mx = x0 - 1 + col;
+                const bool inimg = qq < NQ && my >= 0 && my < H && mx >= 0 && mx < W;
+                const bool own = inimg && row >= 1 && row <= TH && col >= 1 && col <= 32;
+                const size_t opix = inimg ? ((size_t)b * H + my) * W + mx : 0;
+                const float4 val = make_float4(t[4 * j], t[4 * j + 1], t[4 * j + 2], t[4 * j + 3]);
+                if constexpr (F32) {
+                    if (wmap && own) *(float4*)((float*)p1.epi.out_raw + opix * 32 + c4) = val;
+                    if (wbits) {
+                        const uint32_t word = mask_word_from_quads(val.x, val.y, val.z, val.w, i, h);
+                        if (i < 4 && own) p1.epi.bits_out[opix] = word;
+                    }
+                    float4 r = RELU ? relu4(val) : val;
+                    if (!inimg) r = make_float4(0.f, 0.f, 0.f, 0.f);
+                    split2(r.x, r.y, keep_hi[s_][j].x, keep_lo[s_][j].x); split2(r.z, r.w, keep_hi[s_][j].y, keep_lo[s_][j].y);
+                } else {
+                    float4 mv = val;
+                    if constexpr (DG) {
+                        const uint32_t nib = mw1[s_][j] >> c4;
+                        mv.x = (nib & 1u) ? mv.x : 0.0f; mv.y = (nib & 2u) ? mv.y : 0.0f; mv.z = (nib & 4u) ? mv.z : 0.0f; mv.w = (nib & 8u) ? mv.w : 0.0f;
+                    }
+                    uint2 pk = f4_to_bf4(mv);
+                    if (wmap && own) *(uint2*)((bf16_t*)p1.epi.out_raw + opix * 32 + c4) = pk;
+                    if constexpr (DG) {
+                        const float4 a = bf4_to_f4(a1v[s_][j]);
+                        mv.x += a.x; mv.y += a.y; mv.z += a.z; mv.w += a.w;
+                        pk = f4_to_bf4(mv);
+                        if (p1.epi.out_sum && own) *(uint2*)((bf16_t*)p1.epi.out_sum + opix * 32 + c4) = pk;
+                    }
+                    if constexpr (RELU) { pk.x = relu_pk(pk.x); pk.y = relu_pk(pk.y); }
+                    if (!inimg) pk = make_uint2(0u, 0u);
+                    keep_hi[s_][j] = pk;
+                }
+            }
+        }
+        lds_barrier();
+#pragma unroll
+        for (int s_ = 0; s_ < NGC; ++s_) {
+            const int code = (int)((sched >> (4 * s_)) & 15u);
+            const bool yo = code & 8, xo = code & 4;
+            const int gi = code & 3;
+            const int tq = (i & 3) + 4 * h, c4 = 4 * (i >> 2);
+#pragma unroll
+            for (int j = 0; j < 4; ++j) {
+                const int qq = 32 * gi + 8 * j + tq, qc = min(qq, NQ - 1);
+                const int rr = qc / NC, jj = qc - rr * NC;
+                const int row = 2 * rr + (yo ? 0 : 1), col = 2 * jj + (xo ? 0 : 1);
+                unsigned char* dst = lds + (row * X3_PW + col) * STR + 2 * c4;
+                if (qq < NQ) {
+                    *(uint2*)dst = keep_hi[s_][j];
+                    if constexpr (F32) *(uint2*)(dst + Geo<T>::LO) = keep_lo[s_][j];
+                }
+            }
+        }
+        if (tile + gridDim.x < ntiles) issue_loads(tile + gridDim.x);
+        lds_barrier();
+
+        auto do_row = [&](const int row) __attribute__((always_inline)) {
+            const int y = y0 + row;
+            if (y >= H) return;
+            f32x16 acc;
+#pragma unroll
+            for (int r = 0; r < 16; ++r) acc[r] = 0.f;
+            {
+                constexpr int AHEAD = F32 ? 1 : (DG ? 2 : 4), RING = AHEAD + 1;
+                const unsigned char* const arow = lds + (row * X3_PW + i) * STR + 16 * h;
+                const unsigned char* const wrow = wl_lds + lane * 16;
+                uint4 fah[RING], fal[F32 ? RING : 1], fbl[LO ? RING : 1];
+                auto frag_load = [&](const int n_) __attribute__((always_inline)) {
+                    const unsigned char* a = arow + ((n_ / 6) * X3_PW + (n_ / 2) % 3) * STR + 32 * (n_ & 1);
+                    fah[n_ % RING] = *(const uint4*)a;
+                    if constexpr (F32) fal[n_ % RING] = *(const uint4*)(a + Geo<T>::LO);
+                    if constexpr (LO) fbl[n_ % RING] = *(const uint4*)(wrow + n_ * 1024);
+                };
+#pragma unroll
+                for (int s_ = 0; s_ < AHEAD; ++s_) frag_load(s_);
+#pragma unroll
+                for (int s_ = 0; s_ < 18; ++s_) {
+                    if (s_ + AHEAD < 18) frag_load(s_ + AHEAD);
+                    __builtin_amdgcn_sched_barrier(0);
+                    const bf16x8 ah = __builtin_bit_cast(bf16x8, fah[s_ % RING]), bh = __builtin_bit_cast(bf16x8, wh[s_ >> 1][s_ & 1]);
+                    if constexpr (F32) {
+                        acc = __builtin_amdgcn_mfma_f32_32x32x16_bf16(__builtin_bit_cast(bf16x8, fal[s_ % RING]), bh, acc, 0, 0, 0);
+                        acc = __builtin_amdgcn_mfma_f32_32x32x16_bf16(ah, __builtin_bit_cast(bf16x8, fbl[s_ % RING]), acc, 0, 0, 0);
+                    } else if constexpr (DG) {
+                        acc = __builtin_amdgcn_mfma_f32_32x32x16_bf16(ah, __builtin_bit_cast(bf16x8, fbl[s_ % RING]), acc, 0, 0, 0);
+                    }
+                    acc = __builtin_amdgcn_mfma_f32_32x32x16_bf16(ah, bh, acc, 0, 0, 0);
+                    __builtin_amdgcn_sched_barrier(0);
+                }
+            }
+            epi_tile<T, false, DG, ADD>(p2.epi, b, y, H, W, i, acc, x0, h, W, 1, 0, sy, sx, nullptr, 0, 0, &bias2);
+        };
+        if constexpr (TH == 8) {
+#pragma unroll 1
+            for (int rr = 0; rr < 2; ++rr) do_row(2 * wave + rr);
+        } else {
+            do_row(wave);
+        }
+        lds_barrier();
+    }
+}
+
+template <typename T>
+static Conv32P<T> tpair_params(const Conv32Args& a, int Hout, int Wout) {
+    Conv32P<T> p;
+    p.in = (const T*)a.in; p.in_nb = a.in_nb > 0 ? a.in_nb : 1;
+    p.wpack = a.w->mbf16; p.wpack2 = (sizeof(T) == 4 || a.w2) ? a.w->mlo : nullptr;
+    p.epi.bias = a.bias;
+    p.epi.up = nullptr; p.epi.up_nb = 1;
+    p.epi.mask = (const T*)a.mask; p.epi.mask_nb = a.mask_nb > 0 ? a.mask_nb : 1;
+    p.epi.add1 = (const T*)a.add1; p.epi.add1_nb = a.add1_nb > 0 ? a.add1_nb : 1;
+    p.epi.add2 = (const T*)a.add2; p.epi.add2_nb = a.add2_nb > 0 ? a.add2_nb : 1;
+    p.epi.out_raw = (T*)a.out_raw; p.epi.out_sum = (T*)a.out_sum;
+    p.epi.mask_bits = a.mask_bits; p.epi.bits_out = a.bits_out; p.epi.bits_nb = a.bits_nb; p.epi.bits_sum = a.bits_sum;
+    p.B = a.B; p.Hin = a.Hin; p.Win = a.Win; p.Hout = Hout; p.Wout = Wout;
+    return p;
+}
+
+static constexpr int kTpairBlocks = 480;
+
+template <typename T>
+static int launch_tpair_t(const Conv32Args& f, const Conv32Args& g, int form, int max_blocks, hipStream_t s) {
+    const int Hm = f.Hin * 2, Wm = f.Win * 2;
+    const Conv32P<T> p1 = tpair_params<T>(f, Hm, Wm), p2 = tpair_params<T>(g, Hm, Wm);
+    const long tiles8 = (long)g.B * ((Wm + 31) / 32) * ((Hm + 7) / 8), tiles4 = (long)g.B * ((Wm + 31) / 32) * ((Hm + 3) / 4);
+    if (form == 0) form = tiles8 > 256 ? 2 : 1;
+    long blocks = form == 2 ? (tiles8 > kTpairBlocks ? kTpairBlocks : tiles8) : (tiles4 > 1024 ? 1024 : tiles4);
+    if (max_blocks > 0 && blocks > max_blocks) blocks = max_blocks;
+    if constexpr (sizeof(T) == 2) {
+        if (f.w2) {
+            if (form == 2) hipLaunchKernelGGL((conv32_tpair_kernel<T, 8, false, true>), dim3((unsigned)blocks), dim3(256), 0, s, p1, p2);
+            else hipLaunchKernelGGL((conv32_tpair_kernel<T, 4, false, true>), dim3((unsigned)blocks), dim3(256), 0, s, p1, p2);
+            PTTA_CHECK_LAUNCH();
+            return 0;
+        }
+    }
+#define KT_(TH_, A_) hipLaunchKernelGGL((conv32_tpair_kernel<T, TH_, A_>), dim3((unsigned)blocks), dim3(256), 0, s, p1, p2)
+    if (form == 2) { if (g.add1) KT_(8, true); else KT_(8, false); }
+    else { if (g.add1) KT_(4, true); else KT_(4, false); }
+#undef KT_
+    PTTA_CHECK_LAUNCH();
+    return 0;
+}
+
+bool ptta_conv32_tpair_applies(const Conv32Args& first, const Conv32Args& second) {
+    const Conv32Args &f = first, &g = second;
+    if (!f.w || !g.w || !f.in) return false;
+    if (f.mode != CONV_T2 || g.mode != CONV_S1 || f.bf16 != g.bf16 || f.naive || g.naive || (!f.bf16 && (!f.x3 || !g.x3))) return false;
+    if (f.w2 != g.w2) return false;
+    if (f.bits_out && (f.bits_sum || f.bf16)) return false;
+    if (g.bits_out && g.bf16) return false;
+    if (f.w2) {
+        if (!f.bf16 || f.relu_in || g.relu_in || f.up || g.up || f.bits_out || g.bits_out) return false;
+        if (!f.mask || !f.mask_bits || !f.add1 || f.add2 || !f.out_sum) return false;
+        if (!g.mask || !g.mask_bits || g.add1 || g.add2 || g.out_sum || !g.out_raw) return false;
+    } else {
+        if (!f.relu_in || f.up || f.mask || f.add1 || f.add2 || f.out_sum || f.mask_bits) return false;
+        if (!g.relu_in || g.up || g.mask || g.mask_bits || (g.add2 && !g.add1) || (g.add1 && !g.out_sum) || (!g.out_raw && !g.out_sum)) return false;
+    }
+    const int Hm = f.Hin * 2, Wm = f.Win * 2;
+    return f.Hin >= 1 && f.Win >= 1 && g.Hin == Hm && g.Win == Wm && g.B == f.B && f.B >= 1;
+}
+bool ptta_conv32_tpair_pays(const Conv32Args& first, const Conv32Args& second) {
+    if (!first.w2) return true;
+    const int Hm = first.Hin * 2, Wm = first.Win * 2;
+    const long tiles8 = (long)second.B * ((Wm + 31) / 32) * ((Hm + 7) / 8);
+    return tiles8 <= kTpairBlocks;
+}
+int ptta_launch_conv32_tpair(const Conv32Args& first, const Conv32Args& second, int form, int max_blocks, hipStream_t s) {
+    if (form < 0 || form > 2 || !ptta_conv32_tpair_applies(first, second)) return 1;
+    if (form == 0 && !ptta_conv32_tpair_pays(first, second)) return 1;
+    return first.bf16 ? launch_tpair_t<bf16_t>(first, second, form, max_blocks, s) : launch_tpair_t<float>(first, second, form, max_blocks, s);
+}
diff --git a/tta-depth-completion_amd/csrc/msgchn_backward.hip b/tta-depth-completion_amd/csrc/msgchn_backward.hip
--- a/tta-depth-completion_amd/csrc/msgchn_backward.hip
+++ b/tta-depth-completion_amd/csrc/msgchn_backward.hip
@@ -136,10 +136,13 @@
     hipStream_t sd = join_aux ? c->aux(s) : nullptr;
     if (!sd) sd = s;
     { E e; e.sum = c->de3_1; e.mask = c->e3_1; e.mask_nb = B2; e.add1 = c->ds1_3; e.add1_nb = Nn;
-      CV("depth_encoder3.enc2.1", true, CONV_T2, c->de3_2a, Nn, Nn, H4, W4, false, e); }
-    CV("depth_encoder3.enc1.3", true, CONV_S1, c->de3_1, Nn, Nn, H2, W2, false, em(c->de3_1a, c->e3_1a, B2));
+      RUN(conv32_tpair(c, s, true, "depth_encoder3.enc2.1", c->de3_2a, Nn, Nn, H4, W4, e, "depth_encoder3.enc1.3", Nn, em(c->de3_1a, c->e3_1a, B2))); }
+    bool init2_done = false;
     { E e; e.sum = c->de3_0; e.mask = c->e3_0; e.mask_nb = B2; e.add1 = c->ds0_3; e.add1_nb = Nn;
-      CV("depth_encoder3.enc1.1", true, CONV_T2, c->de3_1a, Nn, Nn, H2, W2, false, e); }
+      const E se = em(c->de3_0a, c->e3_0a, B2);
+      init2_done = conv32_tpair_takes(c, true, "depth_encoder3.enc1.1", c->de3_1a, Nn, Nn, H2, W2, e, "depth_encoder3.init.2", Nn, se);
+      if (init2_done) RUN(conv32_tpair(c, s, true, "depth_encoder3.enc1.1", c->de3_1a, Nn, Nn, H2, W2, e, "depth_encoder3.init.2", Nn, se));
+      else CV("depth_encoder3.enc1.1", true, CONV_T2, c->de3_1a, Nn, Nn, H2, W2, false, e); }
     if (sd != s) { HIPCHK(hipEventRecord(c->ev_side[0], s)); HIPCHK(hipStreamWaitEvent(sd, c->ev_side[0], 0)); }
     REST_(sd, ptta_launch_up2T_32(c->de3_0, nullptr, c->up4_t, Nn, H2, W2, nbf, sd));
     REST_(sd, ptta_launch_up2T_32(c->de3_1, nullptr, c->up3_t, Nn, H4, W4, nbf, sd));
@@ -151,7 +154,7 @@
         REST_(sd, ptta_launch_loss_finalize(c->loss_ws, c->N, c->H, c->W, c->Rg, 1, c->hyper + 5, c->loss_info_dst ? c->loss_info_dst : c->loss_info, sd));
         HIPCHK(hipEventRecord(c->ev_loss, sd));
     }
-    CV("depth_encoder3.init.2", true, CONV_S1, c->de3_0, Nn, Nn, H1, W1, false, em(c->de3_0a, c->e3_0a, B2));
+    if (!init2_done) CV("depth_encoder3.init.2", true, CONV_S1, c->de3_0, Nn, Nn, H1, W1, false, em(c->de3_0a, c->e3_0a, B2));
     RUN(dgrad_in_ch1("depth_encoder3.init.0", c->de3_0a, g_net, c->dp11, H1, W1));
     REST_(s, ptta_launch_up2T_1ch(c->dp11, c->dq, Nn, H2, W2, s));
     if (sd != s) HIPCHK(hipStreamWaitEvent(s, c->ev_side[3], 0));
@@ -163,11 +166,9 @@
     { E e; e.sum = c->dz2; e.mask = c->z2; e.mask_nb = B2; e.add1 = c->dz2_up; e.add1_nb = Nn;
       RUN(conv32_pair(c, s, true, "depth_decoder2.dec2.1", c->dt2, Nn, Nn, H4, W4, e, "depth_encoder2.enc2.3", Nn, em(c->de2_2a, c->e2_2a, B2))); }
     { E e; e.sum = c->de2_1; e.mask = c->e2_1; e.mask_nb = B2; e.add1 = c->ds1_2; e.add1_nb = Nn;
-      CV("depth_encoder2.enc2.1", true, CONV_T2, c->de2_2a, Nn, Nn, H8, W8, false, e); }
-    CV("depth_encoder2.enc1.3", true, CONV_S1, c->de2_1, Nn, Nn, H4, W4, false, em(c->de2_1a, c->e2_1a, B2));
+      RUN(conv32_tpair(c, s, true, "depth_encoder2.enc2.1", c->de2_2a, Nn, Nn, H8, W8, e, "depth_encoder2.enc1.3", Nn, em(c->de2_1a, c->e2_1a, B2))); }
     { E e; e.sum = c->de2_0; e.mask = c->e2_0; e.mask_nb = B2; e.add1 = c->ds0_2; e.add1_nb = Nn;
-      CV("depth_encoder2.enc1.1", true, CONV_T2, c->de2_1a, Nn, Nn, H4, W4, false, e); }
-    CV("depth_encoder2.init.2", true, CONV_S1, c->de2_0, Nn, Nn, H2, W2, false, em(c->de2_0a, c->e2_0a, B2));
+      RUN(conv32_tpair(c, s, true, "depth_encoder2.enc1.1", c->de2_1a, Nn, Nn, H4, W4, e, "depth_encoder2.init.2", Nn, em(c->de2_0a, c->e2_0a, B2))); }
     RUN(dgrad_in_ch1("depth_encoder2.init.0", c->de2_0a, c->dq, c->dp12, H2, W2));
     REST_(s, ptta_launch_up2T_1ch(c->dp12, c->dout1, Nn, H4, W4, s));
     RUN(dgrad_out1("depth_decoder1.prdct.3", c->dout1, c->v1, c->dv1, H4, W4));
diff --git a/tta-depth-completion_amd/csrc/msgchn_ctx.h b/tta-depth-completion_amd/csrc/msgchn_ctx.h
--- a/tta-depth-completion_amd/csrc/msgchn_ctx.h
+++ b/tta-depth-completion_amd/csrc/msgchn_ctx.h
@@ -5,6 +5,7 @@
 #include <map>
 #include <string>
 #include <unordered_map>
+#include <unordered_set>
 #include <vector>
 
 #include "../../include/ptta.h"
@@ -119,6 +120,9 @@
     int fuse_first = 1, fuse_head_bwd = 1;
     int pair_fuse = 1;
     int pair_fuse_count = 0;
+    int tpair_fuse = 1;
+    int tpair_fuse_count = 0;
+    std::unordered_set<const void*> tpair_unwritten;
     int cos_grad_fused = 1;
     bool cos_in_gemm = false;
     void* w0frag = nullptr; float *hm_part = nullptr, *headP = nullptr; double* head_k12 = nullptr;
@@ -286,6 +290,10 @@
            int B, int Hin, int Win, bool relu, const E& e);
 int conv32_pair(ptta_ctx* c, hipStream_t s, bool bwd, const std::string& first, const void* in, int in_nb, int B, int Hin, int Win, const E& fe,
                 const std::string& second, int mid_nb, const E& se);
+int conv32_tpair(ptta_ctx* c, hipStream_t s, bool bwd, const std::string& first, const void* in, int in_nb, int B, int Hin, int Win, const E& fe,
+                 const std::string& second, int mid_nb, const E& se);
+bool conv32_tpair_takes(ptta_ctx* c, bool bwd, const std::string& first, const void* in, int in_nb, int B, int Hin, int Win, const E& fe,
+                        const std::string& second, int mid_nb, const E& se);
 int conv32w(ptta_ctx* c, hipStream_t s, const ConvW* w, const float* bias, const void* in, int in_nb, int B, int H, int W, const E& e);
 int conv32_first_bwd(ptta_ctx* c, hipStream_t s, const std::string& layer, ConvInArgs& f, int B, int H, int W, const E& e);
 int to_narrow(ptta_ctx* c, const void* src_f32, void* dst, long n, hipStream_t s);
diff --git a/tta-depth-completion_amd/csrc/msgchn_forward.hip b/tta-depth-completion_amd/csrc/msgchn_forward.hip
--- a/tta-depth-completion_amd/csrc/msgchn_forward.hip
+++ b/tta-depth-completion_amd/csrc/msgchn_forward.hip
@@ -89,6 +89,47 @@
         }
     }
     { const int rc = conv32(c, s, first, bwd, CONV_S2, in, in_nb, B, Hin, Win, relu, fe); if (rc) return rc; }
+    return conv32(c, s, second, bwd, CONV_S1, mid, mid_nb, B, Hm, Wm, relu, se);
+}
+
+static bool tpair_takes(ptta_ctx* c, Conv32Args& f, Conv32Args& g, bool bwd, const std::string& first, const void* in, int in_nb, int B, int Hin, int Win,
+                        const E& fe, const std::string& second, int mid_nb, const E& se) {
+    void* const mid = fe.sum ? fe.sum : fe.raw;
+    const bool nar = fe.nar || (bwd && c->nar_bwd);
+    if (!(c->tpair_fuse && !c->naive && (c->x3 || c->bf16 || nar) && fe.nar == se.nar && mid)) return false;
+    if (conv32_args(c, f, first, bwd, CONV_T2, in, in_nb, B, Hin, Win, !bwd, fe)) return false;
+    if (conv32_args(c, g, second, bwd, CONV_S1, mid, mid_nb, B, Hin * 2, Win * 2, !bwd, se)) return false;
+    return mid_nb == B && ptta_conv32_tpair_applies(f, g) && ptta_conv32_tpair_pays(f, g);
+}
+bool conv32_tpair_takes(ptta_ctx* c, bool bwd, const std::string& first, const void* in, int in_nb, int B, int Hin, int Win, const E& fe,
+                        const std::string& second, int mid_nb, const E& se) {
+    Conv32Args f, g;
+    return tpair_takes(c, f, g, bwd, first, in, in_nb, B, Hin, Win, fe, second, mid_nb, se);
+}
+int conv32_tpair(ptta_ctx* c, hipStream_t s, bool bwd, const std::string& first, const void* in, int in_nb, int B, int Hin, int Win, const E& fe,
+                 const std::string& second, int mid_nb, const E& se) {
+    const int Hm = Hin * 2, Wm = Win * 2;
+    const bool relu = !bwd;
+    void* const mid = fe.sum ? fe.sum : fe.raw;
+    const bool nar = fe.nar || (bwd && c->nar_bwd);
+    {
+        Conv32Args f, g;
+        if (tpair_takes(c, f, g, bwd, first, in, in_nb, B, Hin, Win, fe, second, mid_nb, se)) {
+            if (!bwd && (nar || f.bits_out != nullptr)) { f.out_raw = nullptr; c->tpair_unwritten.insert(fe.raw); }
+            else if (!bwd) c->tpair_unwritten.erase(fe.raw);
+            const int es_l = nar ? 2 : c->es;
+            double b1, m1, b2, m2;
+            conv32_cost(CONV_T2, B, Hin, Win, es_l, b1, m1); conv32_cost(CONV_S1, B, Hm, Wm, es_l, b2, m2);
+            const bool small = (long)Hin * Win <= (long)c->H4 * c->W4;
+            ProfScope ps(c, 4 + (small ? 1 : 0), s, b1 + b2, m1 + m2, 1);
+            const int rc = ptta_launch_conv32_tpair(f, g, 0, 0, s);
+            if (rc == 1) return c->fail("conv32_tpair: fused form refused a case its own test accepted", -22);
+            if (rc == 0) c->tpair_fuse_count++;
+            return rc;
+        }
+    }
+    if (!bwd) c->tpair_unwritten.erase(fe.raw);
+    { const int rc = conv32(c, s, first, bwd, CONV_T2, in, in_nb, B, Hin, Win, relu, fe); if (rc) return rc; }
     return conv32(c, s, second, bwd, CONV_S1, mid, mid_nb, B, Hm, Wm, relu, se);
 }
 
@@ -390,12 +431,10 @@
           RUN(conv32_pair(c, st, false, "depth_encoder2.enc1.1", A(c->e2_0, H2, W2), Bl, Bl, H2, W2, raw(A(c->e2_1a, H4, W4)), "depth_encoder2.enc1.3", Bl, e)); }
         { E e; e.nar = nar; e.sum = A(c->z2, H8, W8); e.up = A(c->y2, H16, W16); e.up_nb = Bl; e.add1 = A(c->c3, H8, W8); e.add1_nb = Bl;
           RUN(conv32_pair(c, st, false, "depth_encoder2.enc2.1", A(c->e2_1, H4, W4), Bl, Bl, H4, W4, raw(A(c->e2_2a, H8, W8)), "depth_encoder2.enc2.3", Bl, e)); }
-        CR("depth_decoder2.dec2.1", false, CONV_T2, A(c->z2, H8, W8), Bl, Bl, H8, W8, true, raw(A(c->t2, H4, W4)));
         { E e; e.nar = nar; e.raw = A(c->z3, H4, W4); e.sum = A(c->s1_2, H4, W4); e.add1 = A(c->e2_1, H4, W4); e.add1_nb = Bl; e.add2 = A(c->m, H4, W4); e.add2_nb = Bl;
-          CR("depth_decoder2.dec2.3", false, CONV_S1, A(c->t2, H4, W4), Bl, Bl, H4, W4, true, e); }
-        CR("depth_decoder2.dec1.1", false, CONV_T2, A(c->s1_2, H4, W4), Bl, Bl, H4, W4, true, raw(A(c->u2, H2, W2)));
+          RUN(conv32_tpair(c, st, false, "depth_decoder2.dec2.1", A(c->z2, H8, W8), Bl, Bl, H8, W8, raw(A(c->t2, H4, W4)), "depth_decoder2.dec2.3", Bl, e)); }
         { E e; e.nar = nar; e.raw = A(c->z4, H2, W2); e.sum = A(c->s0_2, H2, W2); e.add1 = A(c->e2_0, H2, W2); e.add1_nb = Bl; e.add2 = A(c->c1, H2, W2); e.add2_nb = Bl;
-          CR("depth_decoder2.dec1.3", false, CONV_S1, A(c->u2, H2, W2), Bl, Bl, H2, W2, true, e); }
+          RUN(conv32_tpair(c, st, false, "depth_decoder2.dec1.1", A(c->s1_2, H4, W4), Bl, Bl, H4, W4, raw(A(c->u2, H2, W2)), "depth_decoder2.dec1.3", Bl, e)); }
         CR("depth_decoder2.prdct.1", false, CONV_S1, A(c->s0_2, H2, W2), Bl, Bl, H2, W2, true, raw(A(c->v2, H2, W2)));
         {
             const LOut& lo = c->lout["depth_decoder2.prdct.3"];
@@ -453,12 +492,10 @@
         }
     }
     if (!c->skip_dec3) {
-    CV("depth_decoder3.dec2.1", false, CONV_T2, c->w2, B2, Nn, H4, W4, true, e_raw(c->t3));
     { E e; e.sum = c->s1_3; e.add1 = c->e3_1; e.add1_nb = B2; e.add2 = c->c1; e.add2_nb = B2;
-      CV("depth_decoder3.dec2.3", false, CONV_S1, c->t3, Nn, Nn, H2, W2, true, e); }
-    CV("depth_decoder3.dec1.1", false, CONV_T2, c->s1_3, Nn, Nn, H2, W2, true, e_raw(c->u3));
+      RUN(conv32_tpair(c, s, false, "depth_decoder3.dec2.1", c->w2, B2, Nn, H4, W4, e_raw(c->t3), "depth_decoder3.dec2.3", Nn, e)); }
     { E e; e.sum = c->s0_3; e.add1 = c->e3_0; e.add1_nb = B2; e.add2 = c->c0; e.add2_nb = B2;
-      CV("depth_decoder3.dec1.3", false, CONV_S1, c->u3, Nn, Nn, H1, W1, true, e); }
+      RUN(conv32_tpair(c, s, false, "depth_decoder3.dec1.1", c->s1_3, Nn, Nn, H2, W2, e_raw(c->u3), "depth_decoder3.dec1.3", Nn, e)); }
     CV("depth_decoder3.prdct.1", false, CONV_S1, c->s0_3, Nn, Nn, H1, W1, true, e_raw(c->v3));
     {
         const LOut& lo = c->lout["depth_decoder3.prdct.3"];
diff --git a/tta-depth-completion_amd/csrc/msgchn_step.hip b/tta-depth-completion_amd/csrc/msgchn_step.hip
--- a/tta-depth-completion_amd/csrc/msgchn_step.hip
+++ b/tta-depth-completion_amd/csrc/msgchn_step.hip
@@ -149,6 +149,7 @@
 static int step_body(ptta_handle c, const float* image, const float* loss_image, const float* sparse, const float* validity,
                      ptta_stream s_) {
     c->pair_fuse_count = 0;
+    c->tpair_fuse_count = 0;
     RUN(ensure_fused_heads(c, (hipStream_t)s_));
     c->thru_active = thru_ok(c, (hipStream_t)s_);
     c->cnt_sparse = c->thru_active ? sparse : nullptr; c->cnt_validity = validity;
diff --git a/tta-depth-completion_amd/csrc/ptta_api.hip b/tta-depth-completion_amd/csrc/ptta_api.hip
--- a/tta-depth-completion_amd/csrc/ptta_api.hip
+++ b/tta-depth-completion_amd/csrc/ptta_api.hip
@@ -409,6 +409,7 @@
     {"fuse_heads", &ptta_ctx::fuse_heads, 1, false},    {"heads_v2", &ptta_ctx::heads_v2, 1, false},
     {"cos_in_gemm", &ptta_ctx::cos_grad_fused, 1, false}, {"mask_bits", &ptta_ctx::mask_bits_on, 1, false},
     {"stamps", &ptta_ctx::stamps, 1, true},             {"pair_fuse", &ptta_ctx::pair_fuse, 1, true},
+    {"tpair_fuse", &ptta_ctx::tpair_fuse, 1, true},
 };
 static const Option* find_option(const std::string& k) {
     for (const Option& o : kOptions) if (k == o.key) return &o;
@@ -435,7 +436,7 @@
         return 0;
     }
     if (c->nl) return -38;
-    if (k == "pair_fuse_count") return c->fail("ptta_set_option: 'pair_fuse_count' is read-only", -22);
+    if (k == "pair_fuse_count" || k == "tpair_fuse_count") return c->fail("ptta_set_option: '" + k + "' is read-only", -22);
     const Option* o = find_option(k);
     if (!o) return c->fail("ptta_set_option: unknown key '" + k + "'", -22);
     int* f = &(c->*(o->member));
@@ -464,6 +465,7 @@
     if (c->nl) { if (k != "graph") return -38; *value = c->nl->use_graph; return 0; }
     if (k == "graph") { *value = c->use_graph; return 0; }
     if (k == "pair_fuse_count") { *value = c->pair_fuse_count; return 0; }
+    if (k == "tpair_fuse_count") { *value = c->tpair_fuse_count; return 0; }
     const Option* o = find_option(k);
     if (!o) return -22;
     *value = c->*(o->member);
@@ -533,6 +535,8 @@
     if (it == c->dbg.end()) return c->fail(std::string("no debug tensor ") + name, -2);
     if (numel_host) *numel_host = it->second.numel;
     if (!dst) return 0;
+    if (c->tpair_unwritten.count(it->second.p))
+        return c->fail(std::string("debug tensor ") + name + " is not written while option 'tpair_fuse' is 1 (the fused launch keeps it on chip): set it to 0", -38);
     if (capacity < it->second.numel) return c->fail("capacity too small", -22);
     hipStream_t s = (hipStream_t)s_;
     const long n = it->second.numel;
diff --git a/tta-depth-completion_amd/csrc/ptta_kernels.h b/tta-depth-completion_amd/csrc/ptta_kernels.h
--- a/tta-depth-completion_amd/csrc/ptta_kernels.h
+++ b/tta-depth-completion_amd/csrc/ptta_kernels.h
@@ -39,6 +39,9 @@
 int ptta_launch_conv32(const Conv32Args& a, hipStream_t s);
 bool ptta_conv32_pair_applies(const Conv32Args& first, const Conv32Args& second);
 int ptta_launch_conv32_pair(const Conv32Args& first, const Conv32Args& second, hipStream_t s);
+bool ptta_conv32_tpair_applies(const Conv32Args& first, const Conv32Args& second);
+bool ptta_conv32_tpair_pays(const Conv32Args& first, const Conv32Args& second);
+int ptta_launch_conv32_tpair(const Conv32Args& first, const Conv32Args& second, int form, int max_blocks, hipStream_t s);
 int ptta_launch_conv32_loop(const Conv32Args& a, void* buf_a, void* buf_b, int reps, unsigned* ctr, unsigned* base_io, int* err, int variant, hipStream_t s);
 
 struct Plane { const float* p = nullptr; int nb = 1; long bstride = 0;
diff --git a/tta-depth-completion_amd/csrc/ptta_ops.hip b/tta-depth-completion_amd/csrc/ptta_ops.hip
--- a/tta-depth-completion_amd/csrc/ptta_ops.hip
+++ b/tta-depth-completion_amd/csrc/ptta_ops.hip
@@ -97,11 +97,11 @@
     return rc;
 }
 
-int ptta_op_conv32_pair(const float* in, const float* weight1, const float* bias1, const float* weight2, const float* bias2, const float* up,
-                        const float* add0, const float* add1, const float* add2, const uint32_t* mask1_bits, const uint32_t* mask2_bits,
-                        float* out_raw, float* out_sum, float* mid_raw, float* mid_sum, uint32_t* mid_bits, int b, int in_nb,
-                        int hin, int win, int first_mode, int relu1, int relu2, int in_major, int flip, int dtype, int w2, int fused,
-                        int* fused_host, ptta_stream s_) {
+static int op_conv32_pair_body(const float* in, const float* weight1, const float* bias1, const float* weight2, const float* bias2, const float* up,
+                               const float* add0, const float* add1, const float* add2, const uint32_t* mask1_bits, const uint32_t* mask2_bits,
+                               float* out_raw, float* out_sum, float* mid_raw, float* mid_sum, uint32_t* mid_bits, int b, int in_nb,
+                               int hin, int win, int first_mode, int relu1, int relu2, int in_major, int flip, int dtype, int w2, int fused,
+                               int* fused_host, int tform, int max_blocks, ptta_stream s_) {
     hipStream_t s = (hipStream_t)s_;
     if (!in || !weight1 || !weight2 || (!out_raw && !out_sum) || b < 1 || in_nb < 1 || in_nb > b || hin < 1 || win < 1 ||
         (first_mode != CONV_S2 && first_mode != CONV_T2) || (add2 && !add1) || (add1 && !out_sum)) return -22;
@@ -140,8 +140,19 @@
         if (mask2_bits) { g.mask = mask2_bits; g.mask_nb = b; g.mask_bits = mask2_bits; }
         g.out_raw = t[7]; g.out_sum = t[8]; g.B = b; g.Hin = hm; g.Win = wm; g.mode = CONV_S1; g.relu_in = relu2; g.bf16 = nar ? 1 : 0; g.x3 = 1; g.w2 = w2;
         int did = 0;
-        rc = fused ? ptta_launch_conv32_pair(f, g, s) : 1;
+        if (!fused) rc = 1;
+        else if (tform < 0) rc = ptta_launch_conv32_pair(f, g, s);
+        else {
+            Conv32Args ff = f;
+            if (!mid_raw) ff.out_raw = nullptr;
+            rc = ptta_launch_conv32_tpair(ff, g, tform, max_blocks, s);
+        }
         if (rc == 0) did = 1;
+        if (rc == 0 && tform >= 0 && !mid_raw) {
+            std::vector<unsigned char> hb((size_t)nm * es);
+            if (hipStreamSynchronize(s) != hipSuccess || hipMemcpy(hb.data(), t[5], hb.size(), hipMemcpyDeviceToHost) != hipSuccess) rc = -5;
+            else for (unsigned char ch : hb) if (ch != 0xff) { rc = -14; break; }
+        }
         if (rc == 1) { rc = ptta_launch_conv32(f, s); if (!rc) rc = ptta_launch_conv32(g, s); }
         if (fused_host) *fused_host = did;
     }
@@ -156,6 +167,24 @@
     if (hipStreamSynchronize(s) != hipSuccess && !rc) rc = -5;
     for (int k = 0; k < 9; ++k) (void)hipFree(t[k]);
     return rc;
+}
+
+int ptta_op_conv32_pair(const float* in, const float* weight1, const float* bias1, const float* weight2, const float* bias2, const float* up,
+                        const float* add0, const float* add1, const float* add2, const uint32_t* mask1_bits, const uint32_t* mask2_bits,
+                        float* out_raw, float* out_sum, float* mid_raw, float* mid_sum, uint32_t* mid_bits, int b, int in_nb,
+                        int hin, int win, int first_mode, int relu1, int relu2, int in_major, int flip, int dtype, int w2, int fused,
+                        int* fused_host, ptta_stream s_) {
+    return op_conv32_pair_body(in, weight1, bias1, weight2, bias2, up, add0, add1, add2, mask1_bits, mask2_bits, out_raw, out_sum, mid_raw, mid_sum,
+                               mid_bits, b, in_nb, hin, win, first_mode, relu1, relu2, in_major, flip, dtype, w2, fused, fused_host, -1, 0, s_);
+}
+int ptta_op_conv32_tpair(const float* in, const float* weight1, const float* bias1, const float* weight2, const float* bias2, const float* up,
+                         const float* add0, const float* add1, const float* add2, const uint32_t* mask1_bits, const uint32_t* mask2_bits,
+                         float* out_raw, float* out_sum, float* mid_raw, float* mid_sum, uint32_t* mid_bits, int b, int in_nb,
+                         int hin, int win, int first_mode, int relu1, int relu2, int in_major, int flip, int dtype, int w2, int fused,
+                         int form, int max_blocks, int* fused_host, ptta_stream s_) {
+    if (form < 0 || form > 2 || max_blocks < 0) return -22;
+    return op_conv32_pair_body(in, weight1, bias1, weight2, bias2, up, add0, add1, add2, mask1_bits, mask2_bits, out_raw, out_sum, mid_raw, mid_sum,
+                               mid_bits, b, in_nb, hin, win, first_mode, relu1, relu2, in_major, flip, dtype, w2, fused, fused_host, form, max_blocks, s_);
 }
 
 int ptta_op_gwgrad(const float* x, const float* gy, float* gw, float* gb, int b, int h, int w, int ci, int co, int impl, int reps,
diff --git a/tta-depth-completion_amd/proxytta/_lib.py b/tta-depth-completion_amd/proxytta/_lib.py
--- a/tta-depth-completion_amd/proxytta/_lib.py
+++ b/tta-depth-completion_amd/proxytta/_lib.py
@@ -121,6 +121,7 @@
     ('ptta_op_conv32', c_int, [_P, _P, _P, _P, c_int, c_int, c_int, c_int, c_int, c_int, c_int, c_int, c_int, _P]),
     ('ptta_op_conv32_chain', c_int, [_P] * 6 + [c_int] * 7 + [POINTER(c_float), _P]),
     ('ptta_op_conv32_pair', c_int, [_P] * 16 + [c_int] * 12 + [POINTER(c_int), _P]),
+    ('ptta_op_conv32_tpair', c_int, [_P] * 16 + [c_int] * 14 + [POINTER(c_int), _P]),
     ('ptta_op_gwgrad', c_int, [_P, _P, _P, _P] + [c_int] * 7 + [POINTER(c_float), _P]),
     ('ptta_op_gconv', c_int, [_P, c_int, c_int, _P, c_int, c_int, _P, _P, _P] + [c_int] * 16 + [POINTER(ctypes.c_double), POINTER(c_int), _P]),
     ('ptta_op_gconv_affine', c_int, [_P, c_int, c_int, _P, c_int, c_int, _P, _P, _P] + [c_int] * 16 + [POINTER(ctypes.c_double), POINTER(c_int),
```

New measurement: 874.3 (median of 6 runs). 1.02x the previous value.
